# Danderson123/Amira

Measured on AMD Instinct MI355X. Metric: gene-mers/s to corrected GeneMerGraph, higher is better.
Workload: dtype int32; 1 GPU; synthetic 1M reads x 60 genes, k=5, 20k-gene vocab: build + error-correction sweep (build, filter(3,1), correct, build, clip(5), correct, build); reads_per_gpu=1000000, genes_per_read=60, k=5, vocab=20000, gene_mers_per_gpu=56000000, final_nodes=472478, final_edges=1054844, multi_gpu=n/a

## Files before the change

amira_amd/_ffi.py:

```python
import ctypes as C
import os

import numpy as np

_HERE = os.path.dirname(os.path.abspath(__file__))
LIB_PATH = os.path.join(_HERE, "libamg.so")


class AmgError(RuntimeError):
    def __init__(self, code, msg):
        super().__init__(f"libamg error {code}: {msg}")
        self.code = code


E_ARG = -2
E_PALINDROME = -4
E_NOMEM = -6
MAX_K = 16


class Counts(C.Structure):
    _fields_ = [(n, C.c_int64) for n in (
        "n_reads", "n_tokens", "n_windows", "n_short_reads", "n_nodes", "n_edges", "n_pairs",
        "n_components", "n_live_nodes", "n_live_edges", "n_reads_to_correct",
        "node_table_slots", "edge_table_slots", "build_retries")] + [("k", C.c_int32), ("two_v", C.c_int32),
                                                                 ("exact_keys", C.c_int32), ("derived", C.c_int32)]

    def as_dict(self):
        return {n: getattr(self, n) for n, _ in self._fields_}


class Xfer(C.Structure):
    _fields_ = [("kind", C.c_int32), ("elem_bytes", C.c_int32), ("send", C.c_void_p), ("recv", C.c_void_p),
                ("send_counts", C.POINTER(C.c_int64)), ("recv_counts", C.POINTER(C.c_int64)), ("count", C.c_int64)]


XFER_ALL_TO_ALL, XFER_ALL_GATHER = 1, 2
UNIQUE_ID_BYTES = 128


def _load():
    if not os.path.exists(LIB_PATH):
        raise ImportError(
            f"{LIB_PATH} is missing: build it with `python -c 'import __graft_entry__ as g; g.build()'` "
            "(make -C amira_amd/csrc).  amira_amd has no CPU fallback."
        )
    try:
        import torch
    except Exception:
        pass
    lib = C.CDLL(LIB_PATH)
    P, I32, I64, U32 = C.c_void_p, C.c_int32, C.c_int64, C.c_uint32
    sig = {
        "amg_create": (C.c_int, [C.c_int, C.POINTER(P)]),
        "amg_destroy": (C.c_int, [P]),
        "amg_last_error": (C.c_char_p, []),
        "amg_sync": (C.c_int, [P]),
        "amg_stream": (P, [P]),
        "amg_set_reads": (C.c_int, [P, P, P, I64, I32, C.c_int]),
        "amg_set_positions": (C.c_int, [P, P, P, P, C.c_int]),
        "amg_set_positions32": (C.c_int, [P, P, P, P, C.c_int]),
        "amg_set_read_lengths": (C.c_int, [P, P, C.c_int]),
        "amg_build": (C.c_int, [P, I32]),
        "amg_build_filtered": (C.c_int, [P, C.c_int32, C.c_uint32, C.c_uint32]),
        "amg_counts": (C.c_int, [P, C.POINTER(Counts)]),
        "amg_build_multi": (C.c_int, [C.POINTER(P), C.POINTER(I32), I32]),
        "amg_finalize": (C.c_int, [P]),
        "amg_sizes": (C.c_int, [P, C.POINTER(I64), C.POINTER(I64)]),
        "amg_graph_sizes": (C.c_int, [P, C.POINTER(I64), C.POINTER(I64), C.POINTER(I32)]),
        "amg_get_nodes": (C.c_int, [P, P, P, P, P, P, P]),
        "amg_get_edges": (C.c_int, [P, P, P, P, P, P, P]),
        "amg_get_read_nodes": (C.c_int, [P, P, P]),
        "amg_get_read_nodes_rows": (C.c_int, [P, P, P, I64, P]),
        "amg_get_node_adj": (C.c_int, [P, P, P]),
        "amg_get_node_reads": (C.c_int, [P, P, P]),
        "amg_filter": (C.c_int, [P, U32, U32]),
        "amg_remove_nodes": (C.c_int, [P, P, I64]),
        "amg_remove_edges": (C.c_int, [P, P, I64]),
        "amg_remove_short_linear_paths": (C.c_int, [P, I32, P, C.POINTER(I64), P]),
        "amg_remove_low_coverage_components": (C.c_int, [P, U32]),
        "amg_get_reads_to_correct": (C.c_int, [P, P]),
        "amg_correct_reads": (C.c_int, [P, C.POINTER(I64), C.POINTER(I64)]),
        "amg_get_corrected": (C.c_int, [P, P, P, P, P, P, P]),
        "amg_get_corrected32": (C.c_int, [P, P, P, P, P, P, P, P, C.POINTER(I64)]),
        "amg_get_corrected_positions32": (C.c_int, [P, P, P]),
        "amg_adopt_corrected": (C.c_int, [P]),
        "amg_set_reads_from_corrected": (C.c_int, [P, P]),
        "amg_match_patterns": (C.c_int, [P, C.c_int, P, P, I64, P, P, P]),
        "amg_minhash": (C.c_int, [P, P, P, P, I64, I32, C.c_uint64, P, P, I64, C.POINTER(I64)]),
        "amg_junction_paths": (C.c_int, [P, I32, C.POINTER(I64)]),
        "amg_get_junction_paths": (C.c_int, [P, P, P, P, P, P, P]),
        "amg_seqs_create": (C.c_int, [I32, P, P, I64, C.POINTER(P)]),
        "amg_seqs_destroy": (C.c_int, [P]),
        "amg_path_sketch_overlaps": (C.c_int, [P, P, P, I32, C.c_uint64, I64, P, P, I64, P, P, P, P]),
        "amg_kcount_create": (C.c_int, [P, P, I32, I32, C.POINTER(P)]),
        "amg_kcount_sizes": (C.c_int, [P, P]),
        "amg_kcount_histo": (C.c_int, [P, P, I64, P]),
        "amg_kcount_query": (C.c_int, [P, P, P, P, I64, I64, P]),
        "amg_kcount_medians": (C.c_int, [P, P, P, P, P, I64, I64, P, P, P, I64]),
        "amg_kcount_destroy": (C.c_int, [P]),
        "amg_nw_align": (C.c_int, [P, I32, P, I32, P, C.POINTER(I32)]),
        "amg_pop_rewrite": (C.c_int, [P, I32, I32, I64, P, P, P, P, P, I64, P, P, P, I64, P, P, P, P, P, P, P,
                                      C.POINTER(I64)]),
        "amg_dist_unique_id": (C.c_int, [P, I32]),
        "amg_dist_init": (C.c_int, [P, P, I32, I32]),
        "amg_dist_merge": (C.c_int, [P, I32, U32, U32]),
        "amg_dist_finalize": (C.c_int, [P]),
        "amg_dist_init_external": (C.c_int, [P, I32, I32]),
        "amg_dist_merge_begin": (C.c_int, [P, I32, U32, U32]),
        "amg_dist_merge_next": (C.c_int, [P, C.POINTER(Xfer)]),
        "amg_dist_merge_local": (C.c_int, [C.POINTER(P), I32, I32, U32, U32]),
        "amg_copy_d2h": (C.c_int, [P, P, P, I64]),
        "amg_copy_h2d": (C.c_int, [P, P, P, I64]),
        "amg_dist_stats": (C.c_int, [P, C.POINTER(I64), I32]),
        "amg_dist_phase_ms": (C.c_int, [P, I32, C.POINTER(C.c_char_p), C.POINTER(C.c_double), I32]),
        "amg_calls_load_json": (C.c_int, [C.c_char_p, C.POINTER(P)]),
        "amg_calls_counts": (C.c_int, [P, C.POINTER(I64), C.POINTER(I64), C.POINTER(I64), C.POINTER(I64),
                                       C.POINTER(I64)]),
        "amg_calls_get": (C.c_int, [P, P, P, P, P, P]),
        "amg_calls_load_positions_json": (C.c_int, [P, C.c_char_p, P, P]),
        "amg_calls_write_json": (C.c_int, [C.c_char_p, P, P, I64, P, I64, P]),
        "amg_calls_write_positions_json": (C.c_int, [C.c_char_p, P, P, P, I64, P]),
        "amg_calls_write_positions_json32": (C.c_int, [C.c_char_p, P, P, P, I64, P]),
        "amg_calls_first_use": (C.c_int, [P, I64, I32, P, I64, P]),
        "amg_calls_has_blanks": (C.c_int, [P, C.POINTER(I32)]),
        "amg_calls_free": (C.c_int, [P]),
        "amg_calls_trim": (C.c_int, [C.POINTER(I64)]),
        "amg_cluster_full_blocks": (C.c_int, [P, P, I64, P, P, I32, P, I64, I64, C.POINTER(P)]),
        "amg_cluster_anchor_stats": (C.c_int, [P, P, I64, P, P, I32, I64, P]),
        "amg_cluster_blocks_sizes": (C.c_int, [P, C.POINTER(I64), C.POINTER(I64)]),
        "amg_cluster_blocks_get": (C.c_int, [P, P, P]),
        "amg_cluster_blocks_free": (C.c_int, [P]),
        "amg_py_tuple_hash": (I64, [P, I64]),
        "amg_pyset_script": (C.c_int, [P, I64, P, I32, P, P]),
        "amg_last_timings": (C.c_int, [P, C.POINTER(C.c_char_p), C.POINTER(C.c_float), C.c_int]),
        "amg_set_timing": (C.c_int, [P, C.c_int]),
        "amg_scan_probe": (C.c_int, [P, C.c_int, P, I64, P, P]),
        "amg_count_probe": (C.c_int, [P, C.c_int, C.c_int, P, I64, I64, P, I64, C.c_int, C.c_int, P, P]),
        "amg_nw_probe": (C.c_int, [P, I64, P, P, P, P, P, P, P, P, C.c_int, P, P, P, P]),
        "amg_correct_routes": (C.c_int, [P, P, I32]),
    }
    for name, (res, args) in sig.items():
        fn = getattr(lib, name)
        fn.restype, fn.argtypes = res, args
    return lib, sorted(sig)


lib, SYMBOLS = _load()


def check(rc):
    if rc != 0:
        raise AmgError(rc, lib.amg_last_error().decode(errors="replace"))


def ptr(a):
    if a is None:
        return None
    assert isinstance(a, np.ndarray) and a.flags["C_CONTIGUOUS"]
    return a.ctypes.data_as(C.c_void_p)
```

amira_amd/csrc/amg_correct.h:

```cpp
#pragma once
#include "amg_device.h"

enum { RC_SKIP = 0, RC_COPY = 1, RC_DROP = 2, RC_TRIM = 3, RC_GAPPED = 4, RC_KEEP_ORIG = 5 };

struct CorrArgs {
  const int* tokens;
  const long long* read_off;
  const int* tok_node;
  const signed char* tok_dir;
  const unsigned char* read_fix;
  const long long* p0s;
  const long long* p0e;
  const long long* p1s;
  const long long* p1e;
  long long n0;
  const long long* pos_off;
  const long long* read_len;
  long long n_reads;
  int k, flip, have_pos;
  unsigned int* gflag;
  unsigned long long* max_bound;
  unsigned long long* lmask;
  unsigned long long* n_runs;
  unsigned char* cls;
  unsigned char* cls_final;
  int* r_start;
  int* r_end;
  unsigned int* bound;
  const long long* tmp_off;
  unsigned int* new_len;
  int* tmp_tok;
};

__device__ __forceinline__ void pos_base(const CorrArgs& a, long long off, const long long*& gs, const long long*& ge) {
  if (off < a.n0) {
    gs = a.p0s + off;
    ge = a.p0e + off;
  } else {
    gs = a.p1s + (off - a.n0);
    ge = a.p1e + (off - a.n0);
  }
}

__device__ __forceinline__ long long bcast_i64(long long v, int lane) {
  const unsigned int lo = (unsigned int)__builtin_amdgcn_readlane((int)(unsigned int)v, lane);
  const unsigned int hi = (unsigned int)__builtin_amdgcn_readlane((int)(unsigned int)((unsigned long long)v >> 32), lane);
  return (long long)(((unsigned long long)hi << 32) | lo);
}

__device__ __forceinline__ void wave_sync() {
  __builtin_amdgcn_fence(__ATOMIC_ACQ_REL, "wavefront");
  __builtin_amdgcn_wave_barrier();
}

struct __attribute__((aligned(16))) GapRec {
  int r, L0, start, end;
  long long t0, dst;
  unsigned long long mask;
  long long pad;
};

__device__ __forceinline__ unsigned long long gap_run_ends(unsigned long long lv, int start, int end) {
  const unsigned long long inside =
      (end >= 63 ? ~0ull : ((1ull << (end + 1)) - 1ull)) & ~((1ull << (start & 63)) - 1ull);
  return ~lv & inside & (lv >> 1);
}
__device__ __forceinline__ void gap_run_terminals(unsigned long long lv, int i, int& ps, int& pe) {
  ps = 63 - __clzll((long long)(lv & ((1ull << i) - 1ull)));
  pe = i + 1;
}

struct GapArgs {
  CorrArgs a;
  GView g;
  const GapRec* rec;
  const int* gapped_reads;
  long long n_gapped;
  int* pool;
  unsigned long long pool_cap;
  unsigned long long* pool_used;
  unsigned long long* status;
  int* cand;
  unsigned int cand_stride;
  unsigned char* final_cls;
  unsigned char* need_slow;
  const int* gq;
  const int4* qres;
  const int* qpool;
};

#define GF_MAXW 128
#define GF_MAXGAP 16
#define GF_POOL 384
#define GF_CAND 136
#define GF_MAXCOMBO 256
#define GM_INLINE 64
#define LEAN_CHUNK 32
#define CLS_READS 64
#define PACK_READS 64
enum {
  GS_NOT_TRIED = 1,
  GS_WINDOWS = 2,
  GS_RUNS = 3,
  GS_MEMO_UNFIT = 4,
  GS_RECORDS = 5,
  GS_COMBOS = 6,
  GS_CAND = 7,
  GS_CODES = 8
};
enum {
  GL_NO_SLOTS = 1,
  GL_ANSWERS = 2,
  GL_LONG = 3,
  GL_OTHER = 4,
  GL_CODES = 5
};

#define NWF_MAX_M 64
#define NWF_MAX_N 128
__device__ __forceinline__ bool nw_fast_ok(long long N, long long M) {
  return N <= NWF_MAX_N && M <= NWF_MAX_M && N > 0 && M > 0;
}

struct __attribute__((aligned(16))) NwRec {
  int r, M, N, pad;
  long long t0, dst;
  long long pdst;
  long long poff;
};

struct NwArgs {
  CorrArgs a;
  const NwRec* rec;
  long long* o_gs;
  long long* o_ge;
  const int* gapped_reads;
  long long n_gapped;
  const unsigned char* final_cls;
  const long long* big_off;
  unsigned char* big_buf;
  int allow_fast;
  int shortcuts;
  unsigned char* route;
};
enum { NW_ROUTE_NONE = 0, NW_ROUTE_EQUAL = 1, NW_ROUTE_CERT = 2, NW_ROUTE_FILL = 3, NW_ROUTE_LDS = 4, NW_ROUTE_GLOBAL = 5 };

struct PackArgs {
  CorrArgs a;
  const long long* new_idx;
  const long long* new_off;
  const unsigned char* final_cls;
  int* o_tok;
  long long* o_off;
  int* o_orig;
  unsigned char* o_changed;
  long long* o_src;
  const long long* pos_new;
  long long* o_posoff;
  long long* o_rl;
  long long out_reads, out_tokens;
  unsigned long long* dead_kept;
};

struct CorrSwitches {
  bool gap_memo;
  bool fast_gapped;
  bool lean_gapped;
  int fast_nw;
  int nw_shortcuts;
  const char* node_bound;
  bool routes;
  const char* gap_pool;
  const char* memo_spill;
};

struct CorrScratch {
  size_t per_read = 0;
  unsigned char *cls = nullptr, *final_cls = nullptr;
  int *r_start = nullptr, *r_end = nullptr;
  long long *nw_size = nullptr, *nw_off = nullptr;
  unsigned int *bound = nullptr, *new_len = nullptr, *flag = nullptr;
  long long *tmp_off = nullptr, *new_idx = nullptr, *new_off = nullptr;
  int* tmp_tok = nullptr;
  long long *plen = nullptr, *poffs = nullptr, *pos_new = nullptr;
  unsigned long long *max_bound = nullptr, *n_general = nullptr;
  unsigned long long* n_runs = nullptr;
  unsigned long long* dead_kept = nullptr;
  bool count_alive = false;
  DevBuf* glist = nullptr;
  DevBuf* cand = nullptr;
  DevBuf* pool = nullptr;
  DevBuf* need_slow = nullptr;
};

struct CorrCounts {
  long long tmp_total = 0, n_gapped = 0, total_runs = 0;
  unsigned long long max_bound = 0;
  bool carry = false;
  long long out_reads = 0, out_tokens = 0, big_total = 0, pos_total = 0;
  unsigned long long n_general = 0;
  long long n_queries = 0;
  int pool_retries = 0;
  bool lean_ran = false, fast_ran = false, memo = false;
};

static void fill_pos_args(amg_ctx* c, CorrArgs& a) {
  a.p0s = c->have_pos ? c->gene_start.as<long long>() : nullptr;
  a.p0e = c->have_pos ? c->gene_end.as<long long>() : nullptr;
  a.p1s = c->pos1_s.as<long long>();
  a.p1e = c->pos1_e.as<long long>();
  a.n0 = c->pos_n0;
  a.pos_off = (c->have_pos && !c->pos_identity) ? c->pos_off.as<long long>() : nullptr;
}

void corr_classify_launch(amg_ctx* c, const CorrArgs& a);
int corr_gapped(amg_ctx* c, const CorrSwitches& sw, const CorrScratch& S, const CorrArgs& a, CorrCounts& n);
int corr_nw_sizes(amg_ctx* c, const CorrSwitches& sw, const CorrScratch& S, const CorrArgs& a, long long n_gapped,
                  FetchList& shape);
int corr_grow_pos_pools(amg_ctx* c, const CorrCounts& n);
int corr_positions(amg_ctx* c, const CorrSwitches& sw, const CorrScratch& S, const CorrArgs& a, const CorrCounts& n,
                   unsigned char* route = nullptr);

int routes_begin(amg_ctx* c);
int routes_gapped(amg_ctx* c, const CorrScratch& S, const CorrCounts& n, const unsigned char* need_slow, const int* gq);
int routes_nw(amg_ctx* c, const CorrScratch& S, const CorrCounts& n);
int routes_end(amg_ctx* c, const CorrCounts& n);
```

amira_amd/csrc/amg_correct.hip:

```cpp
#include "amg_correct.h"

__global__ __launch_bounds__(256) void k_count_alive(const unsigned char* __restrict__ alive, long long n,
                                                     unsigned long long* out) {
  __shared__ unsigned int s_part[4];
  unsigned int c = 0;
  for (long long i = ((long long)blockIdx.x * blockDim.x + threadIdx.x) * 4; i < n; i += (long long)gridDim.x * blockDim.x * 4) {
    if (i + 4 <= n) {
      const unsigned int w = *reinterpret_cast<const unsigned int*>(alive + i);
      c += __popc(w & 0x01010101u);
    } else {
      for (long long j = i; j < n; ++j) c += alive[j] ? 1u : 0u;
    }
  }
  for (int d = 32; d > 0; d >>= 1) c += (unsigned int)__shfl_xor((int)c, d, 64);
  if ((threadIdx.x & 63) == 0) s_part[threadIdx.x >> 6] = c;
  __syncthreads();
  if (threadIdx.x == 0 && (s_part[0] | s_part[1] | s_part[2] | s_part[3]))
    atomicAdd(out, (unsigned long long)s_part[0] + s_part[1] + s_part[2] + s_part[3]);
}

__global__ __launch_bounds__(256) void k_corr_pack(PackArgs A) {
  const CorrArgs& a = A.a;
  const int lane = threadIdx.x & 63;
  const long long r = ((long long)blockIdx.x * 4 + (threadIdx.x >> 6)) * PACK_READS + lane;
  if (blockIdx.x == 0 && threadIdx.x == 0) A.o_off[A.out_reads] = A.out_tokens;
  long long dst = 0, src = 0;
  int n = 0;
  unsigned int dead = 0;
  if (r < a.n_reads && a.new_len[r] > 0) {
    dst = A.new_off[r];
    n = (int)a.new_len[r];
    const unsigned char fc = A.final_cls[r];
    if (fc == RC_KEEP_ORIG) {
      const long long nw = a.read_off[r + 1] - a.read_off[r] - a.k + 1;
      dead = nw <= 64 ? (unsigned int)(nw - __popcll(a.lmask[r])) : (unsigned int)nw;
    }
    long long poff = 0;
    if (fc == RC_GAPPED) {
      src = a.tmp_off[r] | (1ll << 62);
      if (a.have_pos) poff = A.pos_new[r];
    } else {
      const long long cut = fc == RC_TRIM ? a.r_start[r] : 0;
      src = a.read_off[r] + cut;
      if (a.have_pos) poff = (a.pos_off ? a.pos_off[r] : a.read_off[r]) + cut;
    }
    const long long q = A.new_idx[r];
    A.o_off[q] = dst;
    A.o_orig[q] = (int)r;
    A.o_changed[q] = (fc == RC_TRIM || fc == RC_GAPPED) ? 1 : 0;
    A.o_src[q] = fc == RC_GAPPED ? -1ll : src;
    if (a.have_pos) A.o_posoff[q] = poff;
    if (a.read_len) A.o_rl[q] = a.read_len[r];
  }
  if (__ballot(dead != 0u) != 0ull) {
    for (int d = 32; d > 0; d >>= 1) dead += (unsigned int)__shfl_xor((int)dead, d, 64);
    if (lane == 0) atomicAdd(A.dead_kept + 16 * (blockIdx.x & 15), (unsigned long long)dead);
  }
  if (__ballot(n > 0) == 0ull) return;
  for (int j0 = 0; j0 < PACK_READS; j0 += 4) {
    const int* sp[4];
    long long d[4];
    int nn[4], vt[4];
#pragma unroll
    for (int j = 0; j < 4; ++j) {
      nn[j] = __builtin_amdgcn_readlane(n, j0 + j);
      const long long sj = bcast_i64(src, j0 + j);
      d[j] = bcast_i64(dst, j0 + j);
      sp[j] = ((sj >> 62) & 1 ? a.tmp_tok : a.tokens) + (sj & ~(1ll << 62));
    }
#pragma unroll
    for (int j = 0; j < 4; ++j)
      if (lane < nn[j]) vt[j] = sp[j][lane];
#pragma unroll
    for (int j = 0; j < 4; ++j)
      if (lane < nn[j]) A.o_tok[d[j] + lane] = vt[j];
#pragma unroll
    for (int j = 0; j < 4; ++j)
      for (int i = 64 + lane; i < nn[j]; i += 64)
        A.o_tok[d[j] + i] = sp[j][i];
  }
}

static CorrSwitches read_switches() {
  auto is_one = [](const char* name) {
    const char* v = getenv(name);
    return v && v[0] == '1';
  };
  CorrSwitches sw;
  sw.gap_memo = !is_one("AMG_NO_GAP_MEMO");
  sw.fast_gapped = !is_one("AMG_NO_FAST_GAPPED");
  sw.lean_gapped = !is_one("AMG_NO_LEAN_GAPPED");
  sw.fast_nw = !is_one("AMG_NO_FAST_NW");
  sw.nw_shortcuts = !is_one("AMG_NW_NO_SHORTCUT");
  sw.node_bound = getenv("AMG_TEST_NODE_BOUND");
  sw.routes = is_one("AMG_CORR_ROUTES");
  sw.gap_pool = getenv("AMG_TEST_GAP_POOL");
  sw.memo_spill = getenv("AMG_TEST_MEMO_SPILL");
  return sw;
}

static int plan_per_read(amg_ctx* c, CorrScratch& S) {
  const size_t per_read = (size_t)(c->n_reads + 2);
  AMGCHK(c->s0.ensure(per_read * (1 + 1) + 64));
  AMGCHK(c->s1.ensure(per_read * sizeof(int) * 2 + per_read * sizeof(long long) * 2 + 64));
  AMGCHK(c->s2.ensure(per_read * sizeof(unsigned int) * 3));
  AMGCHK(c->s3.ensure(per_read * sizeof(long long) * 3));
  AMGCHK(c->gm_mask.ensure(per_read * sizeof(unsigned long long)));
  AMGCHK(c->gm_ctr.ensure((16 + 256 + 256 + 16) * sizeof(unsigned long long)));
  S.per_read = per_read;
  S.cls = c->s0.as<unsigned char>();
  S.final_cls = S.cls + per_read;
  S.r_start = c->s1.as<int>();
  S.r_end = S.r_start + per_read;
  S.nw_size = reinterpret_cast<long long*>(((uintptr_t)(S.r_end + per_read) + 15) & ~(uintptr_t)15);
  S.nw_off = S.nw_size + per_read;
  S.bound = c->s2.as<unsigned int>();
  S.new_len = S.bound + per_read;
  S.flag = S.new_len + per_read;
  S.tmp_off = c->s3.as<long long>();
  S.new_idx = S.tmp_off + per_read;
  S.new_off = S.new_idx + per_read;
  S.max_bound = S.n_general = c->status.as<unsigned long long>() + ST_MISC;
  S.n_runs = c->gm_ctr.as<unsigned long long>() + 16;
  S.dead_kept = S.n_runs + 256;
  S.count_alive = c->n_nodes >= (1ll << 20);
  S.glist = &c->c_orig;
  S.cand = &c->c_gstart;
  S.pool = &c->c_gend;
  S.need_slow = &c->c_changed;
  return AMG_OK;
}

static int plan_staging(amg_ctx* c, CorrScratch& S, long long tmp_total) {
  AMGCHK(c->c_tokens_buf.ensure((size_t)(tmp_total + 4) * sizeof(int)));
  AMGCHK(c->s4.ensure((size_t)(tmp_total + 4) * sizeof(int)));
  S.tmp_tok = c->s4.as<int>();
  return AMG_OK;
}

static int plan_positions(amg_ctx* c, CorrScratch& S, long long n_gapped) {
  AMGCHK(c->s5.ensure((size_t)(2 * (n_gapped + 2) + c->n_reads + 2) * sizeof(long long)));
  S.plen = c->s5.as<long long>();
  S.poffs = S.plen + (n_gapped + 2);
  S.pos_new = S.poffs + (n_gapped + 2);
  return AMG_OK;
}

static void corr_args(amg_ctx* c, const CorrScratch& S, CorrArgs& a) {
  a.tokens = c->tokens.as<int>();
  a.read_off = c->read_off.as<long long>();
  a.tok_node = c->tok_node.as<int>();
  a.tok_dir = c->tok_dir.as<signed char>();
  a.read_fix = c->read_fix.as<unsigned char>();
  fill_pos_args(c, a);
  a.read_len = c->have_read_len ? c->read_len.as<long long>() : nullptr;
  a.n_reads = c->n_reads;
  a.k = c->k;
  a.flip = c->two_v - 1;
  a.have_pos = c->have_pos ? 1 : 0;
  a.gflag = S.flag;
  a.max_bound = S.max_bound;
  a.lmask = c->gm_mask.as<unsigned long long>();
  a.n_runs = S.n_runs;
  a.cls = S.cls;
  a.cls_final = S.final_cls;
  a.r_start = S.r_start;
  a.r_end = S.r_end;
  a.bound = S.bound;
  a.tmp_off = S.tmp_off;
  a.new_len = S.new_len;
  a.tmp_tok = S.tmp_tok;
}

static int corr_classify(amg_ctx* c, const CorrScratch& S, const CorrArgs& a, CorrCounts& n) {
  hipStream_t st = c->stream;
  const long long R = c->n_reads;
  {
    ClearList cl;
    cl.add(S.bound, S.per_read * sizeof(unsigned int) * 3);
    cl.add(S.max_bound, sizeof(unsigned long long));
    cl.add(S.n_runs, (256 + 256 + 16) * sizeof(unsigned long long));
    AMGCHK(clear_many(c, cl));
  }
  if (R > 0) corr_classify_launch(c, a);
  if (S.count_alive)
    hipLaunchKernelGGL(k_count_alive, dim3(128), dim3(256), 0, st, c->node_alive.as<unsigned char>(), c->n_nodes,
                       S.dead_kept + 256);
  AMGCHK(prim_exscan_u32_pair(c, S.bound, S.tmp_off, S.flag, S.new_idx, (size_t)R));
  FetchList l;
  l.add(S.tmp_off + R);
  l.add(S.max_bound);
  l.add(S.new_idx + R);
  for (int i = 0; i < 16; ++i) l.add(S.n_runs + 16 * i);
  unsigned long long v[3 + 16];
  AMGCHK(fetch(c, l, v));
  n.tmp_total = (long long)v[0];
  n.max_bound = v[1];
  n.n_gapped = (long long)v[2];
  for (int i = 0; i < 16; ++i) n.total_runs += (long long)v[3 + i];
  n.carry = n.n_gapped > 0 && c->have_pos;
  return AMG_OK;
}

static int corr_shape(amg_ctx* c, const CorrSwitches& sw, CorrScratch& S, const CorrArgs& a, CorrCounts& n) {
  const long long R = c->n_reads;
  AMGCHK(prim_exscan_keep_and_len(c, S.new_len, S.new_idx, S.new_off, (size_t)R));
  FetchList shape;
  shape.add(S.new_idx + R);
  shape.add(S.new_off + R);
  if (n.carry) {
    AMGCHK(plan_positions(c, S, n.n_gapped));
    AMGCHK(corr_nw_sizes(c, sw, S, a, n.n_gapped, shape));
  }
  unsigned long long v[5] = {0, 0, 0, 0, 0};
  AMGCHK(fetch(c, shape, v));
  n.out_reads = (long long)v[0];
  n.out_tokens = (long long)v[1];
  n.big_total = (long long)v[2];
  n.pos_total = (long long)v[3];
  n.n_general = v[4];
  return AMG_OK;
}

static int ensure_outputs(amg_ctx* c, const CorrCounts& n) {
  AMGCHK(c->c_tokens_buf.ensure((size_t)(n.out_tokens + 64) * sizeof(int)));
  AMGCHK(c->c_read_off.ensure((size_t)(n.out_reads + 2) * sizeof(long long)));
  AMGCHK(c->c_orig.ensure((size_t)(n.out_reads + 2) * sizeof(int)));
  AMGCHK(c->c_changed.ensure((size_t)(n.out_reads + 2)));
  AMGCHK(c->c_src.ensure((size_t)(n.out_reads + 2) * sizeof(long long)));
  if (c->have_pos) AMGCHK(c->c_pos_off.ensure((size_t)(n.out_reads + 2) * sizeof(long long)));
  if (c->have_read_len) AMGCHK(c->c_read_len.ensure((size_t)(n.out_reads + 2) * sizeof(long long)));
  return AMG_OK;
}

static int corr_pack(amg_ctx* c, const CorrScratch& S, const CorrArgs& a, const CorrCounts& n) {
  PackArgs Pk;
  Pk.a = a;
  Pk.new_idx = S.new_idx;
  Pk.new_off = S.new_off;
  Pk.final_cls = S.final_cls;
  Pk.o_tok = c->c_tokens_buf.as<int>();
  Pk.o_off = c->c_read_off.as<long long>();
  Pk.o_orig = c->c_orig.as<int>();
  Pk.o_changed = c->c_changed.as<unsigned char>();
  Pk.o_src = c->c_src.as<long long>();
  Pk.pos_new = S.pos_new;
  Pk.o_posoff = c->have_pos ? c->c_pos_off.as<long long>() : nullptr;
  Pk.o_rl = c->have_read_len ? c->c_read_len.as<long long>() : nullptr;
  Pk.out_reads = n.out_reads;
  Pk.out_tokens = n.out_tokens;
  Pk.dead_kept = S.dead_kept;
  if (c->n_reads > 0)
    hipLaunchKernelGGL(k_corr_pack, dim3(nblk(c->n_reads, 4 * PACK_READS)), dim3(256), 0, c->stream, Pk);
  else
    HIPCHK(hipMemcpyAsync(c->c_read_off.as<long long>() + n.out_reads, &n.out_tokens, sizeof(long long),
                          hipMemcpyHostToDevice, c->stream));
  return AMG_OK;
}

static int corr_node_bound(amg_ctx* c, const CorrSwitches& sw, const CorrScratch& S, const CorrCounts& n) {
  FetchList l;
  for (int i = 0; i < 16; ++i) l.add(S.dead_kept + 16 * i);
  l.add(S.dead_kept + 256);
  unsigned long long v[17];
  AMGCHK(fetch(c, l, v));
  unsigned long long bound = S.count_alive ? v[16] : (unsigned long long)c->n_nodes;
  unsigned long long dead_kept = 0;
  for (int i = 0; i < 16; ++i) dead_kept += v[i];
  bound += dead_kept;
  c->c_derivable = n.n_gapped == 0 && dead_kept == 0 && !c->edge_own_deaths;
  c->c_node_bound = (int64_t)bound;
  if (sw.node_bound) c->c_node_bound = atoll(sw.node_bound);
  c->c_node_bound_k = c->k;
  return AMG_OK;
}

extern "C" int amg_correct_reads(amg_ctx* c, int64_t* n_out_reads, int64_t* n_out_tokens) {
  NEED_BUILT(c);
  const CorrSwitches sw = read_switches();
  stages_reset(c);
  c->have_corrected = false;
  CorrScratch S;
  CorrCounts n;
  CorrArgs a;
  AMGCHK(plan_per_read(c, S));
  corr_args(c, S, a);
  c->have_routes = false;
  if (sw.routes) AMGCHK(routes_begin(c));

  stage_begin(c, "correct_classify");
  AMGCHK(corr_classify(c, S, a, n));
  stage_end(c);
  AMGCHK(plan_staging(c, S, n.tmp_total));
  corr_args(c, S, a);

  if (n.n_gapped > 0) {
    stage_begin(c, "live_adjacency");
    AMGCHK(ensure_live_adj(c));
    stage_end(c);
    stage_begin(c, "correct_gapped");
    AMGCHK(corr_gapped(c, sw, S, a, n));
    stage_end(c);
  }

  stage_begin(c, "correct_pack");
  AMGCHK(corr_shape(c, sw, S, a, n));
  stage_end(c);
  AMGCHK(ensure_outputs(c, n));

  if (n.carry) {
    stage_begin(c, "correct_positions");
    AMGCHK(corr_grow_pos_pools(c, n));
    corr_args(c, S, a);
    AMGCHK(corr_positions(c, sw, S, a, n));
    if (sw.routes) AMGCHK(routes_nw(c, S, n));
    stage_end(c);
  }

  stage_begin(c, "correct_pack");
  AMGCHK(corr_pack(c, S, a, n));
  AMGCHK(corr_node_bound(c, sw, S, n));
  stage_end(c);
  if (sw.routes) AMGCHK(routes_end(c, n));
  c->c_reads = n.out_reads;
  c->c_tokens = n.out_tokens;
  c->c_pos1_used = c->pos1_used + (n.carry ? n.pos_total : 0);
  c->have_corrected = true;
  if (n_out_reads) *n_out_reads = n.out_reads;
  if (n_out_tokens) *n_out_tokens = n.out_tokens;
  return AMG_OK;
}
```

amira_amd/csrc/amg_correct_gapped.hip:

```cpp
#include "amg_correct.h"
#include "amg_wave_dfs.h"

__global__ __launch_bounds__(256) void k_corr_classify(CorrArgs a) {
  const long long rbase = ((long long)blockIdx.x * 4 + (threadIdx.x >> 6)) * CLS_READS;
  if (rbase >= a.n_reads) return;
  const int lane = threadIdx.x & 63;
  const long long r = rbase + lane;
  const bool have = r < a.n_reads;
  const long long t0 = have ? a.read_off[r] : 0;
  const long long n = have ? (a.read_off[r + 1] - t0) - a.k + 1 : 0;
  const bool look = have && n > 0 && a.read_fix[r] != 0;
  unsigned long long lv = 0;
  unsigned long long todo = __ballot(look && n <= 64);
  while (todo) {
    int who[4];
    long long tj[4];
    int nj[4], v[4];
#pragma unroll
    for (int q = 0; q < 4; ++q) {
      who[q] = todo ? __ffsll((long long)todo) - 1 : -1;
      if (todo) todo &= todo - 1ull;
      tj[q] = who[q] >= 0 ? bcast_i64(t0, who[q]) : 0;
      nj[q] = who[q] >= 0 ? __builtin_amdgcn_readlane((int)n, who[q]) : 0;
    }
// ... 562 lines not shown

__device__ __forceinline__ void gf_stage(const CorrArgs& a, const GapRec& rec, int nwin, int lane, GfLds& S) {
  for (int i = lane; i < nwin; i += 64) {
    S.node[i] = a.tok_node[rec.t0 + i];
    S.dir[i] = a.tok_dir[rec.t0 + i];
  }
  for (int i = lane; i < rec.L0; i += 64) S.tok[i] = a.tokens[rec.t0 + i];
  if (lane == 0) S.used = 0;
  wave_sync();
}

__device__ __forceinline__ int gf_list_runs(int start, int end, int lane, GfLds& S) {
  int n_gaps = 0;
  for (int c0 = start; c0 <= end; c0 += 64) {
    const int i = c0 + lane;
    const bool is_end = i <= end && S.node[i] < 0 && S.node[i + 1] >= 0;
    const unsigned long long m = __ballot(is_end);
    if (is_end) {
      int q = n_gaps + __popcll(m & ((1ull << lane) - 1ull));
      if (q < GF_MAXGAP) {
        int ps = i - 1;
        while (S.node[ps] < 0) --ps;
        S.gap[3 * q] = ps;
        S.gap[3 * q + 1] = i + 1;
        S.gap[3 * q + 2] = 0;
      }
    }
    n_gaps += __popcll(m);
  }
  return n_gaps;
}

__device__ __forceinline__ int gf_paths_from_memo(const GapArgs& A, int myslot, int n_gaps, int lane, GfLds& S) {
  int4 res = make_int4(0, 0, 0, 0);
  if (lane < n_gaps) res = A.qres[myslot];
  const int len = res.y > 0 ? res.y : 0;
  int at = len;
#pragma unroll
  for (int d = 1; d < GF_MAXGAP; d <<= 1) {
    const int o = __shfl_up(at, d, 64);
    if (lane >= d) at += o;
  }
  const int total = __shfl(at, n_gaps - 1, 64);
  at -= len;
  if (__any(res.y < 0)) return GS_MEMO_UNFIT;
  if (total > GF_POOL) return GS_RECORDS;
  for (int q = 0; q < n_gaps; ++q) {
    const int src = __shfl(res.x, q, 64), ln = __shfl(len, q, 64), dst0 = __shfl(at, q, 64);
    for (int i = lane; i < ln; i += 64) S.pool[dst0 + i] = A.qpool[src + i];
  }
  wave_sync();
  if (lane < n_gaps) {
    for (int o = at; o < at + len; o += 2 + 2 * S.pool[o + 1]) S.pool[o] = lane;
    S.gap[3 * lane + 2] = res.z;
  }
  if (lane == 0) S.used = total;
  wave_sync();
  return 0;
}

__device__ __forceinline__ int gf_paths_by_search(const GView& g, int n_gaps, int lane, GfLds& S) {
  for (int q = 0; q < n_gaps; ++q) {
    const int ps = S.gap[3 * q], pe = S.gap[3 * q + 1];
    const int np = dfs_paths_wave(g, S.node[ps], S.dir[ps], S.node[pe], 2 * g.k, q, S.pool, &S.used, lane);
    if (lane == 0) S.gap[3 * q + 2] = np < 0 ? 0 : np;
    if (np < 0) return GS_RECORDS;
  }
  return 0;
}

__device__ __forceinline__ unsigned long long gf_count_combos(const GfLds& S, int n_gaps, bool& dead_end) {
  unsigned long long n_combo = 1;
  dead_end = false;
  for (int q = 0; q < n_gaps; ++q) {
    const int np = S.gap[3 * q + 2];
    dead_end = dead_end || np == 0;
    n_combo *= (unsigned long long)np;
    if (n_combo > GF_MAXCOMBO) break;
  }
  return n_combo;
}

__device__ __forceinline__ void gf_copy_windows(GfLds& S, int n, int i, int cnt, int lane) {
  for (int j = lane; j < cnt; j += 64) {
    S.cnode[n + j] = S.node[i + j];
    S.cdir[n + j] = S.dir[i + j];
  }
}

__device__ __forceinline__ int gf_build_candidate(GfLds& S, int start, int end, int n_gaps, int used,
                                                  unsigned long long combo, int lane) {
  int n = 0, i = start, prev_pe = -1;
  for (int q = 0; q < n_gaps; ++q) {
    const int ps = S.gap[3 * q], pe = S.gap[3 * q + 1], np = S.gap[3 * q + 2];
    const int cnt = ps - i;
    if (cnt > 0) {
      if (n + cnt > GF_CAND) return -1;
      gf_copy_windows(S, n, i, cnt, lane);
      n += cnt;
    }
    unsigned long long div = 1;
    for (int j = q + 1; j < n_gaps; ++j) div *= (unsigned long long)S.gap[3 * j + 2];
    int pick = (int)((combo / div) % (unsigned long long)np);
    int off = 0;
    while (off < used) {
      if (S.pool[off] == q) {
        if (pick == 0) break;
        --pick;
      }
      off += 2 + 2 * S.pool[off + 1];
    }
    const int L = S.pool[off + 1];
    if (prev_pe == ps && n > 0) --n;
    if (n + L > GF_CAND) return -1;
    for (int j = lane; j < L; j += 64) {
      S.cnode[n + j] = S.pool[off + 2 + j];
      S.cdir[n + j] = (signed char)S.pool[off + 2 + L + j];
    }
    n += L;
    prev_pe = pe;
    i = (q + 1 < n_gaps && S.gap[3 * (q + 1)] == pe) ? pe : pe + 1;
  }
  const int cnt = end - i + 1;
  if (cnt > 0) {
    if (n + cnt > GF_CAND) return -1;
    gf_copy_windows(S, n, i, cnt, lane);
    n += cnt;
  }
  return n;
}

__device__ __forceinline__ void gf_spell_and_score(const GView& g, GfLds& S, int n, int L0, bool rank, int lane,
                                                   int& shared, unsigned long long& csum) {
  const int ng = n + g.k - 1;
  shared = 0;
  csum = 0;
  for (int q = lane; q < ng; q += 64) {
    const int idx = q < g.k - 1 ? 0 : q - (g.k - 1);
    const int j = q < g.k - 1 ? q : g.k - 1;
    S.gene[q] = oriented_tok(g, S.cnode[idx], S.cdir[idx], j);
  }
  if (rank) {
    for (int q = lane; q < n; q += 64) csum += g.n_cov[S.cnode[q]];
    for (int d = 32; d > 0; d >>= 1) csum += __shfl_xor(csum, d, 64);
  }
  wave_sync();
  if (rank) {
    for (int q = lane; q < ng; q += 64) {
      const int tk = S.gene[q];
      bool dup = false;
      for (int w = 0; w < q && !dup; ++w) dup = (S.gene[w] == tk);
      bool hit = false;
      if (!dup)
        for (int w = 0; w < L0 && !hit; ++w) hit = (S.tok[w] == tk);
      shared += hit ? 1 : 0;
    }
    for (int d = 32; d > 0; d >>= 1) shared += __shfl_xor(shared, d, 64);
  }
}

__device__ __forceinline__ void gf_hand_down(const GapArgs& A, long long gi, int lane, int why) {
  if (lane == 0) A.need_slow[gi] = (unsigned char)why;
}

__device__ __forceinline__ void gapped_fast_read(const GapArgs& A, long long gi, int lane, GfLds& S) {
  const CorrArgs& a = A.a;
  const GView& g = A.g;
  const GapRec rec = A.rec[gi];
  const int nwin = rec.L0 - g.k + 1;
  if (nwin > GF_MAXW) return gf_hand_down(A, gi, lane, GS_WINDOWS);
  const int myslot = (A.gq && lane < GF_MAXGAP) ? A.gq[gi * GF_MAXGAP + lane] : -1;
  gf_stage(a, rec, nwin, lane, S);
  const int n_gaps = gf_list_runs(rec.start, rec.end, lane, S);
  if (n_gaps > GF_MAXGAP) return gf_hand_down(A, gi, lane, GS_RUNS);
  wave_sync();
  const int unfit = __builtin_amdgcn_readfirstlane(myslot) >= 0 ? gf_paths_from_memo(A, myslot, n_gaps, lane, S)
                                                                : gf_paths_by_search(g, n_gaps, lane, S);
  if (unfit) return gf_hand_down(A, gi, lane, unfit);
  wave_sync();
  bool dead_end;
  const unsigned long long n_combo = gf_count_combos(S, n_gaps, dead_end);
  if (dead_end) {
    if (lane == 0) {
      a.new_len[rec.r] = (unsigned int)rec.L0;
      A.final_cls[rec.r] = RC_KEEP_ORIG;
    }
    return;
  }
  if (n_combo > GF_MAXCOMBO) return gf_hand_down(A, gi, lane, GS_COMBOS);
  const int used = S.used;
  int best_shared = 0, best_ng = -1;
  unsigned long long best_sum = 0, best_len = 1;
  for (unsigned long long combo = 0; combo < n_combo; ++combo) {
    const int n = gf_build_candidate(S, rec.start, rec.end, n_gaps, used, combo, lane);
    wave_sync();
    if (n < 0) return gf_hand_down(A, gi, lane, GS_CAND);
    int shared;
    unsigned long long csum;
    gf_spell_and_score(g, S, n, rec.L0, n_combo > 1, lane, shared, csum);
    if (n_combo == 1 || cand_better(shared, csum, n, best_shared, best_sum, best_len)) {
      best_shared = shared;
      best_sum = csum;
      best_len = (unsigned long long)n;
      best_ng = n + g.k - 1;
      for (int q = lane; q < best_ng; q += 64) S.best[q] = S.gene[q];
    }
    wave_sync();
  }
  for (int q = lane; q < best_ng; q += 64) a.tmp_tok[rec.dst + q] = S.best[q];
  if (lane == 0) a.new_len[rec.r] = (unsigned int)best_ng;
}

__global__ __launch_bounds__(64 * GF_WPB, 8) void k_corr_gapped_fast(GapArgs A, const unsigned char* __restrict__ left) {
  __shared__ GfLds s_lds;
  const int lane = (int)threadIdx.x;
  if (!left) {
    if ((long long)blockIdx.x < A.n_gapped) gapped_fast_read(A, (long long)blockIdx.x, lane, s_lds);
    return;
  }
  const long long base = (long long)blockIdx.x * LEAN_CHUNK;
  const bool mine = lane < LEAN_CHUNK && base + lane < A.n_gapped && left[base + lane] != 0;
  unsigned long long todo = __ballot(mine);
  while (todo) {
    const int b = __ffsll((long long)todo) - 1;
    todo &= todo - 1ull;
    gapped_fast_read(A, base + b, lane, s_lds);
    wave_sync();
  }
}

__global__ void k_scatter_gapped(const unsigned int* __restrict__ flag, const long long* __restrict__ pos,
                                 long long n_reads, int* __restrict__ out, const long long* __restrict__ read_off,
                                 const int* __restrict__ r_start, const int* __restrict__ r_end,
                                 const long long* __restrict__ tmp_off, const unsigned long long* __restrict__ lmask,
                                 GapRec* __restrict__ rec) {
  long long r = (long long)blockIdx.x * blockDim.x + threadIdx.x;
  if (r >= n_reads || !flag[r]) return;
  const long long gi = pos[r];
  out[gi] = (int)r;
  GapRec q;
  q.r = (int)r;
  q.t0 = read_off[r];
  const long long len = read_off[r + 1] - q.t0;
  q.L0 = (int)(len > 0x7fffffff ? 0x7fffffff : len);
  q.start = r_start[r];
  q.end = r_end[r];
  q.dst = tmp_off[r];
  q.mask = lmask[r];
  q.pad = 0;
  rec[gi] = q;
}

static int gap_memo(amg_ctx* c, const CorrSwitches& sw, const CorrArgs& a, CorrCounts& n, const int** gq) {
  hipStream_t st = c->stream;
  const long long n_gapped = n.n_gapped, total_runs = n.total_runs;
  *gq = nullptr;
  const uint64_t qslots = pow2_at_least((uint64_t)total_runs * 2 + 16);
  AMGCHK(c->gm_tab.ensure((size_t)qslots * sizeof(unsigned long long)));
  AMGCHK(c->gm_res.ensure((size_t)qslots * sizeof(int4)));
  AMGCHK(c->gm_list.ensure((size_t)(total_runs + 1) * sizeof(int)));
  AMGCHK(c->gm_q.ensure((size_t)(n_gapped + 1) * GF_MAXGAP * sizeof(int)));
  {
    ClearList cl;
    cl.add(c->gm_tab.p, (size_t)qslots * sizeof(unsigned long long));
    cl.add(c->gm_ctr.p, 16 * sizeof(unsigned long long));
    cl.add(c->status.as<unsigned long long>() + ST_OVERFLOW, sizeof(unsigned long long));
    AMGCHK(clear_many(c, cl));
  }
  hipLaunchKernelGGL(k_gap_queries, dim3(nblk(n_gapped, 256)), dim3(256), 0, st, c->gap_rec.as<GapRec>(), n_gapped,
                     c->k, a.tok_node, a.tok_dir, c->gm_tab.as<unsigned long long>(), (unsigned int)(qslots - 1),
                     c->gm_ctr.as<unsigned long long>(), c->gm_list.as<int>(), c->gm_q.as<int>(),
                     c->status.as<unsigned long long>());
  unsigned long long v[2] = {0, 0};
  {
    FetchList l;
    l.add(c->gm_ctr.p);
    l.add(c->status.as<unsigned long long>() + ST_OVERFLOW);
    AMGCHK(fetch(c, l, v));
  }
  if (v[1]) return amg_fail(AMG_E_HIP, "correct_reads: path memo table full");
  const long long n_queries = (long long)v[0];
  unsigned long long qcap = (unsigned long long)n_queries * (GM_INLINE + 32ull) + 4096ull;
  if (sw.memo_spill) {
    const unsigned long long lo = (unsigned long long)n_queries * GM_INLINE + strtoull(sw.memo_spill, nullptr, 10);
    qcap = lo < qcap ? lo : qcap;
  }
  if (qcap > 0x7fffffffull) return AMG_OK;
  AMGCHK(c->gm_pool.ensure((size_t)qcap * sizeof(int)));
  AMGCHK(c->gm_gene.ensure((size_t)qcap * sizeof(int)));
  if (n_queries > 0)
    hipLaunchKernelGGL(k_gap_dfs, dim3((unsigned int)n_queries), dim3(64), 0, st, make_view(c), c->gm_list.as<int>(),
                       n_queries, c->gm_tab.as<unsigned long long>(), c->gm_ctr.as<unsigned long long>() + 1, qcap,
                       c->gm_pool.as<int>(), c->gm_res.as<int4>(), c->gm_gene.as<int>());
  *gq = c->gm_q.as<int>();
  n.n_queries = n_queries;
  return AMG_OK;
}

int corr_gapped(amg_ctx* c, const CorrSwitches& sw, const CorrScratch& S, const CorrArgs& a, CorrCounts& n) {
  hipStream_t st = c->stream;
  const long long R = c->n_reads, n_gapped = n.n_gapped;
  AMGCHK(S.glist->ensure((size_t)(n_gapped + 1) * sizeof(int)));
  AMGCHK(c->gap_rec.ensure((size_t)(n_gapped + 1) * sizeof(GapRec)));
  hipLaunchKernelGGL(k_scatter_gapped, dim3(nblk(R, 256)), dim3(256), 0, st, S.flag, S.new_idx, R,
                     S.glist->as<int>(), a.read_off, S.r_start, S.r_end, S.tmp_off, a.lmask, c->gap_rec.as<GapRec>());
  const int* gq = nullptr;
  if (n.total_runs > 0 && sw.gap_memo) AMGCHK(gap_memo(c, sw, a, n, &gq));
  const unsigned int threads_total = 64u * 2048u;
  unsigned int cand_stride = (unsigned int)(2 * n.max_bound + (n.max_bound + 3) / 4 + c->k + 16);
  AMGCHK(S.cand->ensure((size_t)threads_total * cand_stride * sizeof(int)));
  unsigned long long pool_cap = 1ull << 22;
  if (sw.gap_pool) {
    const unsigned long long lo = strtoull(sw.gap_pool, nullptr, 10);
    pool_cap = lo < pool_cap ? lo : pool_cap;
  }
  AMGCHK(S.need_slow->ensure((size_t)n_gapped + 64));
  unsigned char* need_slow = S.need_slow->as<unsigned char>();
  for (int attempt = 0;; ++attempt) {
    AMGCHK(S.pool->ensure((size_t)pool_cap * sizeof(int)));
    unsigned long long* used = c->status.as<unsigned long long>() + ST_COMPACT_A;
    ClearList gcl;
    gcl.add(c->status.p, ST_WORDS * sizeof(unsigned long long));
    GapArgs G;
    G.a = a;
    G.g = make_view(c);
    G.rec = c->gap_rec.as<GapRec>();
    G.gapped_reads = S.glist->as<int>();
    G.n_gapped = n_gapped;
    G.pool = S.pool->as<int>();
    G.pool_cap = pool_cap;
    G.pool_used = used;
    G.status = c->status.as<unsigned long long>();
    G.cand = S.cand->as<int>();
    G.cand_stride = cand_stride;
    G.final_cls = S.final_cls;
    G.need_slow = need_slow;
    G.gq = gq;
    G.qres = c->gm_res.as<int4>();
    G.qpool = c->gm_pool.as<int>();
    if (attempt == 0) {
      gcl.add(need_slow, ((size_t)n_gapped + 4) & ~(size_t)3, sw.fast_gapped ? 0u : 0x01010101u);
      AMGCHK(clear_many(c, gcl));
      if (sw.fast_gapped && gq && sw.lean_gapped) {
        n.lean_ran = true;
        AMGCHK(c->gm_fail.ensure((size_t)n_gapped + 64));
        hipLaunchKernelGGL(k_corr_gapped_lean, dim3(nblk(n_gapped, GL_THREADS / GL_GROUP)), dim3(GL_THREADS), 0, st, G,
                           c->gm_gene.as<int>(), c->gm_fail.as<unsigned char>());
        hipLaunchKernelGGL(k_corr_gapped_fast, dim3(nblk(n_gapped, LEAN_CHUNK)), dim3(64 * GF_WPB), 0, st, G,
                           c->gm_fail.as<unsigned char>());
      } else if (sw.fast_gapped) {
        hipLaunchKernelGGL(k_corr_gapped_fast, dim3((unsigned int)n_gapped), dim3(64 * GF_WPB), 0, st, G,
                           (const unsigned char*)nullptr);
      }
    } else {
      AMGCHK(clear_many(c, gcl));
    }
    unsigned int blocks = (unsigned int)((n_gapped + 63) / 64);
    if (blocks > 2048u) blocks = 2048u;
    hipLaunchKernelGGL(k_corr_gapped, dim3(blocks), dim3(64), 0, st, G);
    unsigned long long hs[ST_WORDS];
    AMGCHK(fetch_status(c, hs));
    if (!hs[ST_OVERFLOW]) break;
    if (attempt >= 8) return amg_fail(AMG_E_OVERFLOW, "correct_reads: path pool overflow");
    pool_cap = hs[ST_COMPACT_A] * 2 + (1ull << 20);
    n.pool_retries = attempt + 1;
  }
  if (sw.routes) AMGCHK(routes_gapped(c, S, n, need_slow, gq));
  return AMG_OK;
}
```

amira_amd/csrc/amg_corrected.hip:

```cpp
#include "amg_correct.h"

__global__ __launch_bounds__(256) void k_gather_positions(CorrArgs a, const long long* __restrict__ c_off,
                                                          const long long* __restrict__ c_posoff, long long c_reads,
                                                          long long* __restrict__ o_gs, long long* __restrict__ o_ge) {
  const long long q = (long long)blockIdx.x * 4 + (threadIdx.x >> 6);
  if (q >= c_reads) return;
  const int lane = threadIdx.x & 63;
  const long long a0 = c_off[q], n = c_off[q + 1] - a0;
  const long long *gs, *ge;
  pos_base(a, c_posoff[q], gs, ge);
  for (long long i = lane; i < n; i += 64) {
    o_gs[a0 + i] = gs[i];
    o_ge[a0 + i] = ge[i];
  }
}

static CorrArgs pool_args(amg_ctx* c) {
  CorrArgs a;
  memset(&a, 0, sizeof(a));
  fill_pos_args(c, a);
  return a;
}

static int to_host(amg_ctx* c, void* dst, const DevBuf& src, size_t bytes) {
  if (!dst || !bytes) return AMG_OK;
  HIPCHK(hipMemcpyAsync(dst, src.p, bytes, hipMemcpyDeviceToHost, c->stream));
  return AMG_OK;
}

extern "C" int amg_get_corrected(amg_ctx* c, int32_t* tokens, int64_t* read_offsets, int32_t* orig_read,
                                 uint8_t* changed, int64_t* gene_start, int64_t* gene_end) {
  if (!c) return amg_fail(AMG_E_ARG, "null ctx");
  if (!c->have_corrected) return amg_fail(AMG_E_STATE, "amg_correct_reads first");
  HIPCHK(hipSetDevice(c->device));
  hipStream_t st = c->stream;
  AMGCHK(to_host(c, tokens, c->c_tokens_buf, (size_t)c->c_tokens * sizeof(int32_t)));
  AMGCHK(to_host(c, read_offsets, c->c_read_off, (size_t)(c->c_reads + 1) * sizeof(int64_t)));
  AMGCHK(to_host(c, orig_read, c->c_orig, (size_t)c->c_reads * sizeof(int32_t)));
  AMGCHK(to_host(c, changed, c->c_changed, (size_t)c->c_reads));
  if (c->have_pos && (gene_start || gene_end) && c->c_tokens > 0) {
    AMGCHK(c->c_gstart.ensure((size_t)(c->c_tokens + 64) * sizeof(long long)));
    AMGCHK(c->c_gend.ensure((size_t)(c->c_tokens + 64) * sizeof(long long)));
    const CorrArgs a = pool_args(c);
    hipLaunchKernelGGL(k_gather_positions, dim3(nblk(c->c_reads, 4)), dim3(256), 0, st, a,
                       c->c_read_off.as<long long>(), c->c_pos_off.as<long long>(), (long long)c->c_reads,
                       c->c_gstart.as<long long>(), c->c_gend.as<long long>());
    AMGCHK(to_host(c, gene_start, c->c_gstart, (size_t)c->c_tokens * sizeof(int64_t)));
    AMGCHK(to_host(c, gene_end, c->c_gend, (size_t)c->c_tokens * sizeof(int64_t)));
  }
  HIPCHK(hipStreamSynchronize(st));
  return AMG_OK;
}

__global__ void k_widen_pos(const int* __restrict__ s32, const int* __restrict__ e32, long long n,
                            long long* __restrict__ s64, long long* __restrict__ e64) {
  for (long long i = (long long)blockIdx.x * blockDim.x + threadIdx.x; i < n; i += (long long)gridDim.x * blockDim.x) {
    s64[i] = (long long)s32[i];
    e64[i] = (long long)e32[i];
  }
}

extern "C" int amg_set_positions32(amg_ctx* c, const int32_t* gene_start, const int32_t* gene_end,
                                   const int64_t* read_len, int on_device) {
  if (!c) return amg_fail(AMG_E_ARG, "null ctx");
  if (c->two_v <= 0) return amg_fail(AMG_E_STATE, "amg_set_reads first");
  if (!gene_start || !gene_end) return amg_fail(AMG_E_ARG, "null positions");
  if (on_device != 0 && on_device != 1) return amg_fail(AMG_E_ARG, "amg_set_positions32: on_device is 0 or 1 (the arrays are widened, never borrowed)");
  HIPCHK(hipSetDevice(c->device));
  hipStream_t st = c->stream;
  const long long T = c->n_tokens;
  const int* d_s = gene_start;
  const int* d_e = gene_end;
  if (!on_device) {
    AMGCHK(c->c_gstart.ensure((size_t)(T + 64) * sizeof(long long)));
    AMGCHK(c->c_gend.ensure((size_t)(T + 64) * sizeof(long long)));
    if (T > 0) {
      HIPCHK(hipMemcpyAsync(c->c_gstart.p, gene_start, (size_t)T * sizeof(int), hipMemcpyHostToDevice, st));
      HIPCHK(hipMemcpyAsync(c->c_gend.p, gene_end, (size_t)T * sizeof(int), hipMemcpyHostToDevice, st));
    }
    d_s = c->c_gstart.as<int>();
    d_e = c->c_gend.as<int>();
  }
  c->gene_start.unborrow();
  c->gene_end.unborrow();
  AMGCHK(c->gene_start.ensure((size_t)(T + 64) * sizeof(long long)));
  AMGCHK(c->gene_end.ensure((size_t)(T + 64) * sizeof(long long)));
  if (T > 0)
    hipLaunchKernelGGL(k_widen_pos, dim3(nblk(T, 1024) < 4096u ? nblk(T, 1024) : 4096u), dim3(256), 0, st, d_s, d_e, T,
                       c->gene_start.as<long long>(), c->gene_end.as<long long>());
  c->have_pos = true;
  c->pos_identity = true;
  c->pos0_own = false;
  c->pos_n0 = T;
  c->pos1_used = c->c_pos1_used = 0;
  c->have_corrected = false;
  c->have_read_len = false;
  if (read_len) {
    c->read_len.unborrow();
    AMGCHK(c->read_len.ensure((size_t)c->n_reads * sizeof(int64_t) + 64));
    if (c->n_reads > 0)
      HIPCHK(hipMemcpyAsync(c->read_len.p, read_len, (size_t)c->n_reads * sizeof(int64_t),
                            on_device ? hipMemcpyDeviceToDevice : hipMemcpyHostToDevice, st));
    c->have_read_len = true;
  }
  HIPCHK(hipStreamSynchronize(st));
  return AMG_OK;
}

__global__ void k_new_pos_len(const long long* __restrict__ c_off, const long long* __restrict__ c_posoff, long long own,
                              long long c_reads, long long* __restrict__ len) {
  const long long q = (long long)blockIdx.x * blockDim.x + threadIdx.x;
  if (q < c_reads) len[q] = c_posoff[q] >= own ? c_off[q + 1] - c_off[q] : 0;
}

__global__ __launch_bounds__(256) void k_gather_new_positions32(CorrArgs a, const long long* __restrict__ c_off,
                                                                const long long* __restrict__ c_posoff, long long c_reads,
                                                                const long long* __restrict__ new_off,
                                                                long long* __restrict__ pos_src, int* __restrict__ o_gs,
                                                                int* __restrict__ o_ge, unsigned long long* too_wide,
                                                                long long own) {
  const long long q = (long long)blockIdx.x * 4 + (threadIdx.x >> 6);
  if (q >= c_reads) return;
  const int lane = threadIdx.x & 63;
  const long long off = c_posoff[q];
  if (off < own) {
    if (lane == 0) pos_src[q] = off;
    return;
  }
  const long long n = c_off[q + 1] - c_off[q], at = new_off[q];
  if (lane == 0) pos_src[q] = -1 - at;
  const long long *gs, *ge;
  pos_base(a, off, gs, ge);
  bool wide = false;
  for (long long i = lane; i < n; i += 64) {
    const long long s = gs[i], e = ge[i];
    wide = wide || s != (long long)(int)s || e != (long long)(int)e;
    o_gs[at + i] = (int)s;
    o_ge[at + i] = (int)e;
  }
  if (wide) *too_wide = 1ull;
}

extern "C" int amg_get_corrected32(amg_ctx* c, int32_t* tokens, int64_t* read_offsets, int32_t* orig_read,
                                   uint8_t* changed, int64_t* pos_src, int32_t* new_start, int32_t* new_end,
                                   int64_t* n_new) {
  if (!c) return amg_fail(AMG_E_ARG, "null ctx");
  if (!c->have_corrected) return amg_fail(AMG_E_STATE, "amg_correct_reads first");
  if (!pos_src || !n_new) return amg_fail(AMG_E_ARG, "amg_get_corrected32: pos_src and n_new are required");
  HIPCHK(hipSetDevice(c->device));
  hipStream_t st = c->stream;
  const long long R = c->c_reads;
  *n_new = 0;
  AMGCHK(to_host(c, tokens, c->c_tokens_buf, (size_t)c->c_tokens * sizeof(int32_t)));
  AMGCHK(to_host(c, read_offsets, c->c_read_off, (size_t)(R + 1) * sizeof(int64_t)));
  AMGCHK(to_host(c, orig_read, c->c_orig, (size_t)R * sizeof(int32_t)));
  AMGCHK(to_host(c, changed, c->c_changed, (size_t)R));
  if (!c->have_pos || R == 0) {
    HIPCHK(hipStreamSynchronize(st));
    return c->have_pos ? AMG_OK : amg_fail(AMG_E_STATE, "amg_get_corrected32: no positions were set");
  }
  AMGCHK(c->s1.ensure((size_t)(2 * R + 4) * sizeof(long long)));
  AMGCHK(c->s2.ensure((size_t)(R + 2) * sizeof(long long)));
  AMGCHK(c->c_gstart.ensure((size_t)(c->c_tokens + 64) * sizeof(long long)));
  AMGCHK(c->c_gend.ensure((size_t)(c->c_tokens + 64) * sizeof(long long)));
  long long* len = c->s1.as<long long>();
  long long* off = len + (R + 2);
  const CorrArgs a = pool_args(c);
  unsigned long long* flag = c->status.as<unsigned long long>() + ST_MISC;
  HIPCHK(hipMemsetAsync(flag, 0, sizeof(unsigned long long), st));
  HIPCHK(hipMemsetAsync(len + R, 0, sizeof(long long), st));
  const long long own = c->pos0_own ? 0 : a.n0;
  hipLaunchKernelGGL(k_new_pos_len, dim3(nblk(R, 256)), dim3(256), 0, st, c->c_read_off.as<long long>(),
                     c->c_pos_off.as<long long>(), own, R, len);
  AMGCHK(prim_exscan_i64(c, len, off, (size_t)R + 1));
  hipLaunchKernelGGL(k_gather_new_positions32, dim3(nblk(R, 4)), dim3(256), 0, st, a, c->c_read_off.as<long long>(),
                     c->c_pos_off.as<long long>(), R, off, c->s2.as<long long>(), c->c_gstart.as<int>(),
                     c->c_gend.as<int>(), flag, own);
  unsigned long long h[2] = {0, 0};
  {
    FetchList l;
    l.add(off + R);
    l.add(flag);
    AMGCHK(fetch(c, l, h));
  }
  if (h[1]) return amg_fail(AMG_E_ARG, "amg_get_corrected32: a position does not fit 32 bits (amg_get_corrected returns 64-bit positions)");
  *n_new = (int64_t)h[0];
  AMGCHK(to_host(c, pos_src, c->s2, (size_t)R * sizeof(int64_t)));
  AMGCHK(to_host(c, new_start, c->c_gstart, (size_t)h[0] * sizeof(int32_t)));
  AMGCHK(to_host(c, new_end, c->c_gend, (size_t)h[0] * sizeof(int32_t)));
  HIPCHK(hipStreamSynchronize(st));
  return AMG_OK;
}

__global__ __launch_bounds__(256) void k_gather_positions32(CorrArgs a, const long long* __restrict__ c_off,
                                                            const long long* __restrict__ c_posoff, long long c_reads,
                                                            int* __restrict__ o_gs, int* __restrict__ o_ge,
                                                            unsigned long long* too_wide) {
  const long long q = (long long)blockIdx.x * 4 + (threadIdx.x >> 6);
  if (q >= c_reads) return;
  const int lane = threadIdx.x & 63;
  const long long a0 = c_off[q], n = c_off[q + 1] - a0;
  const long long *gs, *ge;
  pos_base(a, c_posoff[q], gs, ge);
  bool wide = false;
  for (long long i = lane; i < n; i += 64) {
    const long long s = gs[i], e = ge[i];
    wide = wide || s != (long long)(int)s || e != (long long)(int)e;
    o_gs[a0 + i] = (int)s;
    o_ge[a0 + i] = (int)e;
  }
  if (wide) *too_wide = 1ull;
}

extern "C" int amg_get_corrected_positions32(amg_ctx* c, int32_t* gene_start, int32_t* gene_end) {
  if (!c || !gene_start || !gene_end) return amg_fail(AMG_E_ARG, "null argument");
  if (!c->have_corrected) return amg_fail(AMG_E_STATE, "amg_correct_reads first");
  if (!c->have_pos) return amg_fail(AMG_E_STATE, "no gene positions were set");
  HIPCHK(hipSetDevice(c->device));
  hipStream_t st = c->stream;
  const long long R = c->c_reads, T = c->c_tokens;
  if (T == 0) return AMG_OK;
  AMGCHK(c->c_gstart.ensure((size_t)(T + 64) * sizeof(long long)));
  AMGCHK(c->c_gend.ensure((size_t)(T + 64) * sizeof(long long)));
  unsigned long long* flag = c->status.as<unsigned long long>() + ST_MISC;
  HIPCHK(hipMemsetAsync(flag, 0, sizeof(unsigned long long), st));
  const CorrArgs a = pool_args(c);
  hipLaunchKernelGGL(k_gather_positions32, dim3(nblk(R, 4)), dim3(256), 0, st, a, c->c_read_off.as<long long>(),
                     c->c_pos_off.as<long long>(), R, c->c_gstart.as<int>(), c->c_gend.as<int>(), flag);
  unsigned long long wide = 0;
  {
    FetchList l;
    l.add(flag);
    AMGCHK(fetch(c, l, &wide));
  }
  if (wide) return amg_fail(AMG_E_ARG, "amg_get_corrected_positions32: a position does not fit 32 bits (amg_get_corrected returns 64-bit positions)");
  HIPCHK(hipMemcpyAsync(gene_start, c->c_gstart.p, (size_t)T * sizeof(int32_t), hipMemcpyDeviceToHost, st));
  HIPCHK(hipMemcpyAsync(gene_end, c->c_gend.p, (size_t)T * sizeof(int32_t), hipMemcpyDeviceToHost, st));
  HIPCHK(hipStreamSynchronize(st));
  return AMG_OK;
}

extern "C" int amg_adopt_corrected(amg_ctx* c) {
  if (!c) return amg_fail(AMG_E_ARG, "null ctx");
  if (!c->have_corrected) return amg_fail(AMG_E_STATE, "amg_correct_reads first");
  bool compacted = false;
  if (c->have_pos && c->c_tokens > 0) {
    long long slack = 1ll << 20;
    if (const char* e = getenv("AMG_POS_COMPACT_MIN")) slack = atoll(e);
    if (c->c_pos1_used > 2 * c->c_tokens + slack) {
      HIPCHK(hipSetDevice(c->device));
      AMGCHK(c->c_gstart.ensure((size_t)(c->c_tokens + 64) * sizeof(long long)));
      AMGCHK(c->c_gend.ensure((size_t)(c->c_tokens + 64) * sizeof(long long)));
      const CorrArgs a = pool_args(c);
      hipLaunchKernelGGL(k_gather_positions, dim3(nblk(c->c_reads, 4)), dim3(256), 0, c->stream, a,
                         c->c_read_off.as<long long>(), c->c_pos_off.as<long long>(), (long long)c->c_reads,
                         c->c_gstart.as<long long>(), c->c_gend.as<long long>());
      HIPCHK(hipStreamSynchronize(c->stream));
      c->gene_start.unborrow();
      c->gene_end.unborrow();
      std::swap(c->gene_start, c->c_gstart);
      std::swap(c->gene_end, c->c_gend);
      compacted = true;
      c->pos0_own = true;
    }
  }
  for (DevBuf* b : {&c->tokens, &c->read_off, &c->read_len}) b->unborrow();
  std::swap(c->tokens, c->c_tokens_buf);
  std::swap(c->read_off, c->c_read_off);
  std::swap(c->rd_src, c->c_src);
  c->derive_ready = c->c_derivable;
  c->dist_candidate = c->dist_mode;
  c->c_derivable = false;
  if (c->have_pos && compacted) {
    c->pos_identity = true;
    c->pos_n0 = c->c_tokens;
    c->pos1_used = c->c_pos1_used = 0;
  } else if (c->have_pos) {
    std::swap(c->pos_off, c->c_pos_off);
    c->pos_identity = false;
    c->pos1_used = c->c_pos1_used;
  }
  if (c->have_read_len) std::swap(c->read_len, c->c_read_len);
  c->n_reads = c->c_reads;
  c->n_tokens = c->c_tokens;
  c->have_corrected = false;
  c->built = false;
  c->match_valid = false;
  if (c->c_node_bound > 0 && c->c_node_bound_k == c->k && (c->node_hint == 0 || c->c_node_bound < c->node_hint))
    c->node_hint = c->c_node_bound > 256 ? c->c_node_bound : 256;
  c->c_node_bound = 0;
  return AMG_OK;
}

extern "C" int amg_set_reads_from_corrected(amg_ctx* dst, amg_ctx* src) {
  if (!dst || !src) return amg_fail(AMG_E_ARG, "null ctx");
  if (!src->have_corrected) return amg_fail(AMG_E_STATE, "amg_correct_reads on the source ctx first");
  if (dst == src) return amg_adopt_corrected(src);
  if (dst->device != src->device) return amg_fail(AMG_E_ARG, "amg_set_reads_from_corrected: one device");
  HIPCHK(hipSetDevice(dst->device));
  HIPCHK(hipStreamSynchronize(src->stream));
  hipStream_t st = dst->stream;
  const long long R = src->c_reads, T = src->c_tokens;
  AMGCHK(dst->tokens.ensure((size_t)T * sizeof(int32_t) + 64));
  AMGCHK(dst->read_off.ensure((size_t)(R + 1) * sizeof(int64_t) + 64));
  if (T > 0) HIPCHK(hipMemcpyAsync(dst->tokens.p, src->c_tokens_buf.p, (size_t)T * sizeof(int32_t), hipMemcpyDeviceToDevice, st));
  HIPCHK(hipMemcpyAsync(dst->read_off.p, src->c_read_off.p, (size_t)(R + 1) * sizeof(int64_t), hipMemcpyDeviceToDevice, st));
  dst->n_reads = R;
  dst->n_tokens = T;
  dst->two_v = src->two_v;
  dst->have_pos = dst->have_read_len = false;
  if (src->have_pos) {
    AMGCHK(dst->gene_start.ensure((size_t)(T + 64) * sizeof(long long)));
    AMGCHK(dst->gene_end.ensure((size_t)(T + 64) * sizeof(long long)));
    if (R > 0 && T > 0) {
      const CorrArgs a = pool_args(src);
      hipLaunchKernelGGL(k_gather_positions, dim3(nblk(R, 4)), dim3(256), 0, st, a, src->c_read_off.as<long long>(),
                         src->c_pos_off.as<long long>(), R, dst->gene_start.as<long long>(),
                         dst->gene_end.as<long long>());
    }
    dst->have_pos = true;
    dst->pos0_own = true;
    dst->pos_identity = true;
    dst->pos_n0 = T;
    dst->pos1_used = dst->c_pos1_used = 0;
  }
  if (src->have_read_len) {
    AMGCHK(dst->read_len.ensure((size_t)(R + 1) * sizeof(long long) + 64));
    if (R > 0)
      HIPCHK(hipMemcpyAsync(dst->read_len.p, src->c_read_len.p, (size_t)R * sizeof(long long), hipMemcpyDeviceToDevice, st));
    dst->have_read_len = true;
  }
  HIPCHK(hipStreamSynchronize(st));
  dst->built = false;
  dst->derive_ready = false;
  dst->have_corrected = false;
  dst->match_valid = false;
  dst->node_hint = 0;
  dst->hint_bound = src->c_node_bound;
  dst->hint_bound_k = src->c_node_bound_k;
  dst->cnt_hint_reset = true;
  return AMG_OK;
}
```

amira_amd/csrc/amg_derive.hip:

```cpp
#include "amg_device.h"

__device__ __forceinline__ long long dv_new_token(long long t, const long long* __restrict__ src,
                                                  const long long* __restrict__ read_off, long long n_reads, int k,
                                                  bool* ok) {
  long long lo = 0, hi = n_reads;
  while (lo < hi) {
    const long long mid = (lo + hi) >> 1;
    if (src[mid] <= t) lo = mid + 1; else hi = mid;
  }
  const long long i = lo - 1;
  if (i < 0) {
    *ok = false;
    return 0;
  }
  const long long q = t - src[i], len = read_off[i + 1] - read_off[i];
  if (q + k > len) *ok = false;
  return read_off[i] + q;
}

#define DV_READS 64
__device__ __forceinline__ long long dv_bcast(long long v, int lane) {
  const unsigned int lo = (unsigned int)__builtin_amdgcn_readlane((int)(unsigned int)(unsigned long long)v, lane);
  const unsigned int hi = (unsigned int)__builtin_amdgcn_readlane((int)(unsigned int)((unsigned long long)v >> 32), lane);
  return (long long)(((unsigned long long)hi << 32) | lo);
}
__global__ __launch_bounds__(256) void k_dv_windows(const long long* __restrict__ read_off, const long long* __restrict__ src,
                                                    long long n_reads, int k, const int* __restrict__ old_node,
                                                    const signed char* __restrict__ old_dir,
                                                    const long long* __restrict__ new_id, int* __restrict__ tok_node,
                                                    signed char* __restrict__ tok_dir, unsigned long long* bad) {
  const int lane = threadIdx.x & 63;
  const long long r0 = ((long long)blockIdx.x * 4 + (threadIdx.x >> 6)) * DV_READS;
  if (r0 >= n_reads) return;
  long long o = 0, s = 0;
  int n = 0;
  if (r0 + lane < n_reads) {
    o = read_off[r0 + lane];
    n = (int)(read_off[r0 + lane + 1] - o);
    s = src[r0 + lane];
  }
  for (int j0 = 0; j0 < DV_READS; j0 += 4) {
    long long oo[4], ss[4];
    int nn[4], most = 0;
#pragma unroll
    for (int j = 0; j < 4; ++j) {
      nn[j] = __builtin_amdgcn_readlane(n, j0 + j);
      oo[j] = dv_bcast(o, j0 + j);
      ss[j] = dv_bcast(s, j0 + j);
      most = nn[j] > most ? nn[j] : most;
    }
    for (int q = lane; q < most; q += 64) {
      int old[4];
      signed char d[4];
#pragma unroll
      for (int j = 0; j < 4; ++j) {
        old[j] = -1;
        d[j] = 0;
        if (q + k <= nn[j]) {
          old[j] = old_node[ss[j] + q];
          d[j] = old_dir[ss[j] + q];
        }
      }
#pragma unroll
      for (int j = 0; j < 4; ++j) {
        if (q >= nn[j]) continue;
        int v = -1;
        if (q + k <= nn[j]) {
          if (old[j] >= 0) v = (int)new_id[old[j]];
          else *bad = 1ull;
        }
        tok_node[oo[j] + q] = v;
        tok_dir[oo[j] + q] = v >= 0 ? d[j] : (signed char)0;
      }
    }
  }
}

__global__ void k_dv_nodes(const unsigned char* __restrict__ alive, const long long* __restrict__ new_id, long long n_old, int k,
                           const int* __restrict__ tok_in, const unsigned int* __restrict__ cov_in,
                           const long long* __restrict__ first_in, const long long* __restrict__ src,
                           const long long* __restrict__ read_off, long long n_reads, long long own_lo, long long own_hi,
                           int* __restrict__ tok_out, unsigned int* __restrict__ cov_out, long long* __restrict__ first_out,
                           unsigned char* __restrict__ alive_out, unsigned long long* bad) {
  long long n = (long long)blockIdx.x * blockDim.x + threadIdx.x;
  if (n >= n_old || !alive[n]) return;
  const long long i = new_id[n];
  for (int x = 0; x < k; ++x) tok_out[i * k + x] = tok_in[n * k + x];
  cov_out[i] = cov_in[n];
  alive_out[i] = 1;
  const long long f = first_in[n], tg = f >> 1;
  if (tg < own_lo || tg >= own_hi) {
    first_out[i] = 0;
    return;
  }
  bool ok = true;
  const long long t = dv_new_token(tg - own_lo, src, read_off, n_reads, k, &ok);
  if (!ok) *bad = 2ull;
  first_out[i] = (t << 1) | (f & 1ll);
}

__global__ void k_dv_pair_keep(const unsigned long long* __restrict__ pkey, long long n_pairs,
                               const unsigned char* __restrict__ alive, unsigned int* __restrict__ keep) {
  long long p = (long long)blockIdx.x * blockDim.x + threadIdx.x;
  if (p >= n_pairs) return;
  const unsigned long long key = pkey[p];
  const unsigned int lo = (unsigned int)((key >> 32) & 0x7fffffffull), hi = (unsigned int)(key & 0xffffffffull) - 1u;
  keep[p] = (alive[lo] && alive[hi]) ? 1u : 0u;
}

__global__ void k_dv_pairs(const unsigned long long* __restrict__ pkey, const unsigned long long* __restrict__ pfirst,
                           const unsigned int* __restrict__ pcnt, long long n_pairs, const unsigned int* __restrict__ keep,
                           const long long* __restrict__ pos, const long long* __restrict__ new_id,
                           const long long* __restrict__ src, const long long* __restrict__ read_off, long long n_reads, int k,
                           long long own_lo, long long own_hi,
                           unsigned long long* __restrict__ okey, unsigned long long* __restrict__ ofirst,
                           unsigned int* __restrict__ ocnt, unsigned long long* bad) {
  long long p = (long long)blockIdx.x * blockDim.x + threadIdx.x;
  if (p >= n_pairs || !keep[p]) return;
  const unsigned long long key = pkey[p], f = pfirst[p];
  const unsigned int lo = (unsigned int)((key >> 32) & 0x7fffffffull), hi = (unsigned int)(key & 0xffffffffull) - 1u;
  const unsigned long long nlo = (unsigned long long)new_id[lo], nhi = (unsigned long long)new_id[hi];
  const long long q = pos[p];
  okey[q] = (key & (1ull << 63)) | (nlo << 32) | (nhi + 1ull);
  ocnt[q] = pcnt[p];
  const long long tg = (long long)(f >> 3);
  if (tg < own_lo || tg >= own_hi) {
    ofirst[q] = 0ull;
    return;
  }
  bool ok = true;
  const long long t = dv_new_token(tg - own_lo, src, read_off, n_reads, k, &ok);
  if (!ok) *bad = 3ull;
  ofirst[q] = ((unsigned long long)t << 3) | (f & 7ull);
}

__global__ void k_dv_bounds(const long long* __restrict__ base, int world, const long long* __restrict__ node_first,
                            long long n_nodes, const long long* __restrict__ new_id, const unsigned long long* __restrict__ pfirst,
                            long long n_pairs, const long long* __restrict__ ppos, long long* __restrict__ bounds) {
  const int r = blockIdx.x * blockDim.x + threadIdx.x;
  if (r > world) return;
  {
    long long lo = 0, hi = n_nodes;
    const long long want = r == world ? 0x7fffffffffffffffll : (base[r] << 1);
    while (lo < hi) {
      const long long mid = (lo + hi) >> 1;
      if (node_first[mid] < want) lo = mid + 1; else hi = mid;
    }
    bounds[r] = new_id[lo];
  }
  {
    long long lo = 0, hi = n_pairs;
    const unsigned long long want = r == world ? ~0ull : ((unsigned long long)base[r] << 3);
    while (lo < hi) {
      const long long mid = (lo + hi) >> 1;
      if (pfirst[mid] < want) lo = mid + 1; else hi = mid;
    }
    bounds[world + 1 + r] = ppos[lo];
  }
}

int derive_local(amg_ctx* c, int k, long long own_lo, long long own_tokens, const long long* d_bases, int world,
                 long long* bounds_host, long long* D2_out, long long* P2_out, bool* ok) {
  *ok = false;
  hipStream_t st = c->stream;
  const long long D = c->n_nodes, P = c->n_pairs, R = c->n_reads, T = c->n_tokens;
  stage_begin(c, "derive");
  unsigned long long* bad = c->status.as<unsigned long long>() + ST_MISC;
  AMGCHK(c->s2.ensure((size_t)(D + 2) * sizeof(long long)));
  AMGCHK(c->s3.ensure((size_t)(P + 2) * sizeof(unsigned int)));
  AMGCHK(c->s4.ensure((size_t)(P + 2) * sizeof(long long)));
  long long* new_id = c->s2.as<long long>();
  unsigned int* keep = c->s3.as<unsigned int>();
  long long* ppos = c->s4.as<long long>();
  {
    ClearList cl;
    cl.add(c->status.p, ST_WORDS * sizeof(unsigned long long));
    cl.add(keep + P, sizeof(unsigned int));
    AMGCHK(clear_many(c, cl));
  }
  AMGCHK(prim_exscan_bytes_set(c, c->node_alive.as<unsigned char>(), new_id, (size_t)D));
  if (P > 0)
    hipLaunchKernelGGL(k_dv_pair_keep, dim3(nblk(P, 256)), dim3(256), 0, st, c->pair_key.as<unsigned long long>(), P,
                       c->node_alive.as<unsigned char>(), keep);
  AMGCHK(prim_exscan_u32_to_i64(c, keep, ppos, (size_t)P + 1));
  AMGCHK(c->alt_tok_node.ensure((size_t)(T + 8) * sizeof(int)));
  AMGCHK(c->alt_tok_dir.ensure((size_t)(T + 8)));
  if (R > 0)
    hipLaunchKernelGGL(k_dv_windows, dim3(nblk(R, 4 * DV_READS)), dim3(256), 0, st, c->read_off.as<long long>(),
                       c->rd_src.as<long long>(), R, k, c->tok_node.as<int>(), c->tok_dir.as<signed char>(), new_id,
                       c->alt_tok_node.as<int>(), c->alt_tok_dir.as<signed char>(), bad);
  long long* d_bounds = nullptr;
  if (d_bases) {
    AMGCHK(c->s1.ensure((size_t)(2 * (world + 1)) * sizeof(long long)));
    d_bounds = c->s1.as<long long>();
    hipLaunchKernelGGL(k_dv_bounds, dim3(nblk(world + 1, 64)), dim3(64), 0, st, d_bases, world, c->node_first.as<long long>(), D,
                       new_id, c->pair_first.as<unsigned long long>(), P, ppos, d_bounds);
  }
  unsigned long long v[2 + FETCH_MAX - 2];
  {
    FetchList l;
    l.add(new_id + D);
    l.add(ppos + P);
    if (d_bounds) l.add_words(d_bounds, 2 * (world + 1));
    if (l.overflow) return amg_fail(AMG_E_ARG, "derive: world too large");
    AMGCHK(fetch(c, l, v));
  }
  const long long D2 = (long long)v[0], P2 = (long long)v[1];
  if (bounds_host)
    for (int i = 0; i < 2 * (world + 1); ++i) bounds_host[i] = (long long)v[2 + i];
  AMGCHK(c->alt_ntok.ensure((size_t)(D2 * k + 1) * sizeof(int)));
  AMGCHK(c->alt_ncov.ensure((size_t)(D2 + 1) * sizeof(unsigned int)));
  AMGCHK(c->alt_nfirst.ensure((size_t)(D2 + 1) * sizeof(long long)));
  AMGCHK(c->alt_nalive.ensure((size_t)(D2 + 1)));
  AMGCHK(c->alt_pkey.ensure((size_t)(P2 + 2) * sizeof(unsigned long long)));
  AMGCHK(c->alt_pfirst.ensure((size_t)(P2 + 2) * sizeof(unsigned long long)));
  AMGCHK(c->alt_pcnt.ensure((size_t)(P2 + 2) * sizeof(unsigned int)));
  if (D > 0)
    hipLaunchKernelGGL(k_dv_nodes, dim3(nblk(D, 256)), dim3(256), 0, st, c->node_alive.as<unsigned char>(), new_id, D, k,
                       c->node_tokens.as<int>(), c->node_cov.as<unsigned int>(), c->node_first.as<long long>(),
                       c->rd_src.as<long long>(), c->read_off.as<long long>(), R, own_lo, own_lo + own_tokens,
                       c->alt_ntok.as<int>(), c->alt_ncov.as<unsigned int>(), c->alt_nfirst.as<long long>(),
                       c->alt_nalive.as<unsigned char>(), bad);
  if (P > 0)
    hipLaunchKernelGGL(k_dv_pairs, dim3(nblk(P, 256)), dim3(256), 0, st, c->pair_key.as<unsigned long long>(),
                       c->pair_first.as<unsigned long long>(), c->pair_cnt.as<unsigned int>(), P, keep, ppos, new_id,
                       c->rd_src.as<long long>(), c->read_off.as<long long>(), R, k, own_lo, own_lo + own_tokens,
                       c->alt_pkey.as<unsigned long long>(), c->alt_pfirst.as<unsigned long long>(),
                       c->alt_pcnt.as<unsigned int>(), bad);
  stage_end(c);
  AMGCHK(bs_read_stats(c, k));
  unsigned long long hs[ST_WORDS];
  AMGCHK(fetch_status(c, hs));
  if (hs[ST_MISC] || hs[ST_BADINPUT]) return AMG_OK;
  c->n_windows = (int64_t)hs[ST_N_WINDOWS];
  c->n_short = (int64_t)hs[ST_N_SHORT];
  *D2_out = D2;
  *P2_out = P2;
  *ok = true;
  return AMG_OK;
}

int derive_commit(amg_ctx* c, long long D2, long long P2) {
  std::swap(c->tok_node, c->alt_tok_node);
  std::swap(c->tok_dir, c->alt_tok_dir);
  std::swap(c->node_tokens, c->alt_ntok);
  std::swap(c->node_cov, c->alt_ncov);
  std::swap(c->node_first, c->alt_nfirst);
  std::swap(c->node_alive, c->alt_nalive);
  std::swap(c->pair_key, c->alt_pkey);
  std::swap(c->pair_first, c->alt_pfirst);
  std::swap(c->pair_cnt, c->alt_pcnt);
  AMGCHK(c->node_comp.ensure((size_t)(D2 + 1) * sizeof(int)));
  c->n_nodes = c->n_local_nodes = D2;
  c->n_pairs = c->n_local_pairs = P2;
  c->comp_from_claims = false;
  c->filtered_build = false;
  AMGCHK(bs_finish_from_pairs(c));
  c->built = true;
  c->derived = true;
  c->node_hint = D2 > 256 ? D2 : 256;
  return AMG_OK;
}

int derive_from_previous(amg_ctx* c, int k, bool* done) {
  *done = false;
  if (c->n_nodes <= 0 || c->n_reads <= 0 || c->n_tokens <= 0) return AMG_OK;
  long long D2 = 0, P2 = 0;
  bool ok = false;
  AMGCHK(derive_local(c, k, 0, 0x3fffffffffffffffll, nullptr, 1, nullptr, &D2, &P2, &ok));
  if (!ok) return AMG_OK;
  AMGCHK(derive_commit(c, D2, P2));
  *done = true;
  return AMG_OK;
}
```

amira_amd/csrc/amg_device.h:

```cpp
#pragma once
#include "amg_internal.h"

#define AMG_WAVE 64
#define AMG_LAST_FLAG 0x80000000u
#define AMG_MADE_FLAG 0x40000000u
#define AMG_FLAG_MASK (AMG_LAST_FLAG | AMG_MADE_FLAG)
#define AMG_SINGLE_BIT 0x20000000u

__device__ __forceinline__ unsigned long long ld_u64(const unsigned long long* p) {
  return __hip_atomic_load(p, __ATOMIC_RELAXED, __HIP_MEMORY_SCOPE_AGENT);
}
__device__ __forceinline__ int ld_i32(const int* p) {
  return __hip_atomic_load(p, __ATOMIC_RELAXED, __HIP_MEMORY_SCOPE_AGENT);
}

__device__ __forceinline__ unsigned long long mix64(unsigned long long x) {
  x ^= x >> 32;
  x *= 0xD6E8FEB86659FD93ull;
  x ^= x >> 32;
  x *= 0xD6E8FEB86659FD93ull;
  x ^= x >> 32;
  return x;
}

template <class View>
__device__ __forceinline__ int canon_dir(const View& w, int k, int flip) {
  for (int j = 0; j < k; ++j) {
    int a = w[j];
    int b = flip - w[k - 1 - j];
    if (a != b) return a < b ? 1 : -1;
  }
  return 0;
}

template <class View>
__device__ __forceinline__ int canon_tok(const View& w, int k, int flip, int dir, int j) {
  return dir > 0 ? w[j] : flip - w[k - 1 - j];
}

template <class View>
__device__ __forceinline__ unsigned long long canon_fingerprint(const View& w, int k, int flip,
                                                                int dir, unsigned long long seed) {
  unsigned long long h = seed;
  for (int j = 0; j < k; ++j) {
    unsigned long long c = (unsigned long long)(unsigned int)canon_tok(w, k, flip, dir, j);
    h = (h ^ c) * 0x9E3779B97F4A7C15ull;
    h ^= h >> 29;
  }
  h = mix64(h);
  return h ? h : 1ull;
}

__device__ __forceinline__ long long table_upsert(Slot* tab, unsigned long long mask,
                                                  unsigned long long key,
                                                  unsigned long long start,
                                                  unsigned long long first, unsigned int limit,
                                                  bool count_inline = true,
                                                  const unsigned long long* abort_flag = nullptr) {
  unsigned long long idx = start & mask;
  for (unsigned int probes = 0;; ++probes) {
    if (abort_flag && (probes & 63u) == 63u && *reinterpret_cast<const volatile unsigned long long*>(abort_flag))
      return -1;
    Slot* s = tab + idx;
    unsigned long long cur = ld_u64(&s->key);
    if (cur == 0ull) {
      cur = atomicCAS(&s->key, 0ull, key);
      if (cur == 0ull) cur = key;
    }
    if (cur == key) {
      if (count_inline) atomicAdd(&s->count, 1u);
      unsigned long long fi = ~first;
      if (ld_u64(&s->first_inv) < fi) atomicMax(&s->first_inv, fi);
      return (long long)idx;
    }
    if (probes >= limit) return -1;
    idx = (idx + 1) & mask;
  }
}

#define AMG_PACK_MAX_K 14
__device__ __forceinline__ void slot_pack(Slot* s, int id, const int* tok, int k) {
  unsigned int w[8] = {0, 0, 0, 0, 0, 0, 0, 0};
  for (int j = 0; j < k; ++j) {
    const int word = j < 10 ? (j >> 1) : 6 + ((j - 10) >> 1);
    w[word] |= ((unsigned int)tok[j] & 0xffffu) << ((j & 1) * 16);
  }
  w[5] = (unsigned int)id;
  uint4* p = reinterpret_cast<uint4*>(s);
  p[0] = make_uint4(w[0], w[1], w[2], w[3]);
  p[1] = make_uint4(w[4], w[5], w[6], w[7]);
}
__device__ __forceinline__ unsigned int packed_tok(const uint4& lo, const uint4& hi, int j) {
  const int word = j < 10 ? (j >> 1) : 6 + ((j - 10) >> 1);
  unsigned int w = word == 0 ? lo.x : word == 1 ? lo.y : word == 2 ? lo.z : word == 3 ? lo.w
                 : word == 4 ? hi.x : word == 6 ? hi.z : hi.w;
  return (w >> ((j & 1) * 16)) & 0xffffu;
}

template <int WAVES>
__device__ __forceinline__ unsigned int block_exscan(unsigned int v, unsigned int* total,
                                                     unsigned int* s_wave ) {
  unsigned int lane = threadIdx.x & 63, wave = threadIdx.x >> 6;
  unsigned int x = v;
#pragma unroll
  for (int d = 1; d < 64; d <<= 1) {
    unsigned int y = __shfl_up(x, d, 64);
    if (lane >= (unsigned)d) x += y;
  }
  if (lane == 63) s_wave[wave] = x;
  __syncthreads();
  unsigned int base = 0, tot = 0;
#pragma unroll
  for (int w = 0; w < WAVES; ++w) {
    unsigned int c = s_wave[w];
    if ((unsigned)w < wave) base += c;
    tot += c;
  }
  __syncthreads();
  *total = tot;
  return base + x - v;
}
__device__ __forceinline__ unsigned int block_exscan_256(unsigned int v, unsigned int* total,
                                                         unsigned int* s_wave ) {
  return block_exscan<4>(v, total, s_wave);
}


struct ClearArgs {
  void* p[CLEAR_MAX];
  unsigned long long words[CLEAR_MAX];
  unsigned int fill[CLEAR_MAX];
  int n;
};
static inline ClearArgs clear_args(const ClearList& l) {
  ClearArgs a;
  a.n = l.n;
  for (int i = 0; i < l.n; ++i) {
    a.p[i] = l.p[i];
    a.words[i] = l.bytes[i] >> 2;
    a.fill[i] = l.fill[i];
  }
  return a;
}
__device__ __forceinline__ void clear_args_part(const ClearArgs& a, unsigned long long part, unsigned long long parts) {
  const unsigned long long bd = blockDim.x, stride = parts * bd;
  for (int r = 0; r < a.n; ++r) {
    unsigned int* p = reinterpret_cast<unsigned int*>(a.p[r]);
    const unsigned long long w = a.words[r];
    const unsigned int f = a.fill[r];
    const unsigned long long head = ((16u - ((unsigned long long)(uintptr_t)p & 15u)) & 15u) >> 2;
    const unsigned long long h = head < w ? head : w;
    const unsigned long long quads = (w - h) >> 2;
    uint4* q = reinterpret_cast<uint4*>(p + h);
    for (unsigned long long i = part * bd + threadIdx.x; i < quads; i += stride) q[i] = make_uint4(f, f, f, f);
    if (part == 0) {
      for (unsigned long long i = threadIdx.x; i < h; i += bd) p[i] = f;
      for (unsigned long long i = h + quads * 4 + threadIdx.x; i < w; i += bd) p[i] = f;
    }
  }
}

__device__ __forceinline__ int uf_ld(const int* p) {
  return __hip_atomic_load(p, __ATOMIC_RELAXED, __HIP_MEMORY_SCOPE_WAVEFRONT);
}
__device__ __forceinline__ int uf_find(int* parent, int x) {
  int p = uf_ld(parent + x);
  while (p != x) {
    const int g = uf_ld(parent + p);
    if (g != p) __hip_atomic_store(parent + x, g, __ATOMIC_RELAXED, __HIP_MEMORY_SCOPE_WAVEFRONT);
    x = p;
    p = g;
  }
  return x;
}
```

amira_amd/csrc/amg_filter.hip:

```cpp
#include "amg_rows.h"

__global__ void k_filter_nodes(const unsigned int* __restrict__ cov, unsigned char* __restrict__ alive,
                               long long n, unsigned int min_cov) {
  long long i = (long long)blockIdx.x * blockDim.x + threadIdx.x;
  if (i < n && alive[i] && cov[i] < min_cov) alive[i] = 0;
}

__global__ void k_filter_edges(const int* __restrict__ src, const int* __restrict__ tgt,
                               const unsigned int* __restrict__ cov,
                               const unsigned char* __restrict__ node_alive,
                               unsigned char* __restrict__ alive, long long n, unsigned int min_cov) {
  long long e = (long long)blockIdx.x * blockDim.x + threadIdx.x;
  if (e >= n || !alive[e]) return;
  if ((min_cov > 1 && cov[e] < min_cov) || !node_alive[src[e]] || !node_alive[tgt[e]]) alive[e] = 0;
}

#define READS_PER_WAVE 8
__global__ __launch_bounds__(256) void k_mask_reads(int* __restrict__ tok_node,
                                                    const long long* __restrict__ read_off,
                                                    long long n_reads,
                                                    const unsigned char* __restrict__ node_alive,
                                                    unsigned char* __restrict__ read_fix) {
  const long long rbase = ((long long)blockIdx.x * 4 + (threadIdx.x >> 6)) * READS_PER_WAVE;
  if (rbase >= n_reads) return;
  const int lane = threadIdx.x & 63;
  const long long off_l = (lane <= READS_PER_WAVE && rbase + lane <= n_reads) ? read_off[rbase + lane] : 0;
  long long a[READS_PER_WAVE], b[READS_PER_WAVE];
  int v[READS_PER_WAVE];
#pragma unroll
  for (int j = 0; j < READS_PER_WAVE; ++j) {
    a[j] = __shfl(off_l, j, 64);
    b[j] = rbase + j < n_reads ? __shfl(off_l, j + 1, 64) : a[j];
  }
#pragma unroll
  for (int j = 0; j < READS_PER_WAVE; ++j) v[j] = a[j] + lane < b[j] ? tok_node[a[j] + lane] : -1;
  bool dead[READS_PER_WAVE];
#pragma unroll
  for (int j = 0; j < READS_PER_WAVE; ++j) dead[j] = v[j] >= 0 && !node_alive[v[j]];
#pragma unroll
  for (int j = 0; j < READS_PER_WAVE; ++j) {
    if (dead[j]) tok_node[a[j] + lane] = -2;
    bool hit = dead[j];
    for (long long t = a[j] + 64 + lane; t < b[j]; t += 64) {
      const int n = tok_node[t];
      if (n >= 0 && !node_alive[n]) {
        tok_node[t] = -2;
        hit = true;
      }
    }
    if (__any(hit) && lane == 0) read_fix[rbase + j] = 1;
  }
}

static int apply_removals(amg_ctx* c, unsigned int min_edge_cov) {
  hipStream_t st = c->stream;
  if (min_edge_cov > 1) live_lists_after_edge_deaths(c);
  else live_lists_after_node_deaths(c);
  if (c->n_edges > 0)
    hipLaunchKernelGGL(k_filter_edges, dim3(nblk(c->n_edges, 256)), dim3(256), 0, st,
                       c->edge_src.as<int>(), c->edge_tgt.as<int>(), c->edge_cov.as<unsigned int>(),
                       c->node_alive.as<unsigned char>(), c->edge_alive.as<unsigned char>(),
                       c->n_edges, min_edge_cov);
  if (c->n_reads > 0)
    hipLaunchKernelGGL(k_mask_reads, dim3(nblk(c->n_reads, 4 * READS_PER_WAVE)), dim3(256), 0, st,
                       c->tok_node.as<int>(), c->read_off.as<long long>(), c->n_reads,
                       c->node_alive.as<unsigned char>(), c->read_fix.as<unsigned char>());
  return AMG_OK;
}

extern "C" int amg_filter(amg_ctx* c, uint32_t min_node_cov, uint32_t min_edge_cov) {
  NEED_BUILT(c);
  stages_reset(c);
  stage_begin(c, "filter");
  if (c->n_nodes > 0)
    hipLaunchKernelGGL(k_filter_nodes, dim3(nblk(c->n_nodes, 256)), dim3(256), 0, c->stream,
                       c->node_cov.as<unsigned int>(), c->node_alive.as<unsigned char>(),
                       c->n_nodes, min_node_cov);
  AMGCHK(apply_removals(c, min_edge_cov));
  stage_end(c);
  c->have_corrected = false;
  return AMG_OK;
}

__global__ void k_kill_listed(const int* __restrict__ ids, long long n, long long n_nodes,
                              unsigned char* __restrict__ alive) {
  long long i = (long long)blockIdx.x * blockDim.x + threadIdx.x;
  if (i >= n) return;
  int v = ids[i];
  if (v >= 0 && v < n_nodes) alive[v] = 0;
}

extern "C" int amg_remove_nodes(amg_ctx* c, const int32_t* node_ids, int64_t n) {
  NEED_BUILT(c);
  if (n < 0 || (n > 0 && !node_ids)) return amg_fail(AMG_E_ARG, "bad node list");
  if (n == 0) return AMG_OK;
  AMGCHK(c->s0.ensure((size_t)n * sizeof(int)));
  HIPCHK(hipMemcpyAsync(c->s0.p, node_ids, (size_t)n * sizeof(int), hipMemcpyHostToDevice, c->stream));
  hipLaunchKernelGGL(k_kill_listed, dim3(nblk(n, 256)), dim3(256), 0, c->stream, c->s0.as<int>(),
                     (long long)n, c->n_nodes, c->node_alive.as<unsigned char>());
  AMGCHK(apply_removals(c, 0));
  HIPCHK(hipStreamSynchronize(c->stream));
  c->have_corrected = false;
  return AMG_OK;
}

extern "C" int amg_remove_edges(amg_ctx* c, const int32_t* edge_ids, int64_t n) {
  NEED_BUILT(c);
  if (n < 0 || (n > 0 && !edge_ids)) return amg_fail(AMG_E_ARG, "bad edge list");
  if (n == 0) return AMG_OK;
  AMGCHK(c->s0.ensure((size_t)n * sizeof(int)));
  HIPCHK(hipMemcpyAsync(c->s0.p, edge_ids, (size_t)n * sizeof(int), hipMemcpyHostToDevice, c->stream));
  hipLaunchKernelGGL(k_kill_listed, dim3(nblk(n, 256)), dim3(256), 0, c->stream, c->s0.as<int>(), (long long)n,
                     c->n_edges, c->edge_alive.as<unsigned char>());
  live_lists_after_edge_deaths(c);
  HIPCHK(hipStreamSynchronize(c->stream));
  c->have_corrected = false;
  return AMG_OK;
}

#define CLIP_MAX 64
template <class View>
__global__ void k_clip_mark(View g, long long n_nodes, int min_length, const unsigned long long* __restrict__ acc,
                            const unsigned int* __restrict__ comp_live,
                            const unsigned char* __restrict__ protect,
                            unsigned char* __restrict__ kill) {
  long long i = (long long)blockIdx.x * blockDim.x + threadIdx.x;
  if (i >= n_nodes || !g.n_alive[i]) return;
  int n = (int)i;
  if (node_degree(g, n) != 1) return;
  int d0 = (g.n_first[n] & 1ll) ? -1 : 1;
  int path[CLIP_MAX];
  int len = 0;
  path[len++] = n;
  int tgt = -1, td = 0;
  int r = lin_step(g, n, d0 == -1, &tgt, &td);
  while (r == 2 && tgt != n) {
    if (len >= min_length) return;
    path[len++] = tgt;
    r = lin_step(g, tgt, td == 1, &tgt, &td);
  }
  r = lin_step(g, n, d0 == 1, &tgt, &td);
  while (r == 2 && tgt != n) {
    if (len >= min_length) return;
    path[len++] = tgt;
    r = lin_step(g, tgt, td == 1, &tgt, &td);
  }
  if (!(len > 0 && len < min_length)) return;
  const double thr = ((double)acc[0] / (double)acc[1]) * 1.5;
  bool all_high = true;
  for (int j = 0; j < len; ++j) all_high = all_high && ((double)g.n_cov[path[j]] > thr);
  if (all_high) return;
  if (comp_live) {
    int distinct = 0;
    for (int j = 0; j < len; ++j) {
      bool dup = false;
      for (int q = 0; q < j; ++q) dup = dup || (path[q] == path[j]);
      distinct += dup ? 0 : 1;
    }
    if ((unsigned int)distinct == comp_live[g.n_comp[n]]) return;
  } else {
    bool closed = true;
    for (int j = 0; j < len && closed; ++j)
      for (int side = 0; side < 2 && closed; ++side) {
        const long long row = 2ll * path[j] + side;
        const int cnt = row_count(g, row);
        for (int q = 0; q < cnt && closed; ++q) {
          const int t = row_target(g, row, q);
          bool in = false;
          for (int m = 0; m < len; ++m) in = in || (path[m] == t);
          closed = in;
        }
      }
    if (closed) return;
  }
  for (int j = 0; j < len; ++j)
    if (!protect || !protect[path[j]]) kill[path[j]] = 1;
}

__device__ __forceinline__ void block_add_cov(unsigned long long sum, unsigned long long n, unsigned long long* __restrict__ acc) {
  __shared__ unsigned long long s_part[2][4];
  for (int d = 32; d > 0; d >>= 1) {
    sum += __shfl_xor(sum, d, 64);
    n += __shfl_xor(n, d, 64);
  }
  if ((threadIdx.x & 63) == 0) {
    s_part[0][threadIdx.x >> 6] = sum;
    s_part[1][threadIdx.x >> 6] = n;
  }
  __syncthreads();
  if (threadIdx.x == 0) {
    const unsigned long long n_all = s_part[1][0] + s_part[1][1] + s_part[1][2] + s_part[1][3];
    if (n_all) {
      atomicAdd(&acc[0], s_part[0][0] + s_part[0][1] + s_part[0][2] + s_part[0][3]);
      atomicAdd(&acc[1], n_all);
    }
  }
}

__global__ void k_comp_hist(const int* __restrict__ comp, const unsigned char* __restrict__ alive,
                            const unsigned int* __restrict__ cov, long long n, unsigned int min_cov,
                            unsigned int* __restrict__ live_cnt, unsigned int* __restrict__ high_cnt,
                            unsigned long long* __restrict__ acc ) {
  int cid = -1;
  unsigned int n_live = 0, n_high = 0;
  unsigned long long s_cov = 0, s_n = 0;
  for (long long i = (long long)blockIdx.x * blockDim.x + threadIdx.x; i < n; i += (long long)gridDim.x * blockDim.x) {
    if (!alive[i]) continue;
    if (acc) {
      s_cov += cov[i];
      s_n += 1;
    }
    const int id = comp[i];
    if (id != cid) {
      if (cid >= 0) {
        atomicAdd(&live_cnt[cid], n_live);
        if (high_cnt && n_high) atomicAdd(&high_cnt[cid], n_high);
      }
      cid = id;
      n_live = n_high = 0;
    }
    ++n_live;
    n_high += (high_cnt && cov[i] >= min_cov) ? 1u : 0u;
  }
  const int lane = threadIdx.x & 63;
  if (acc) block_add_cov(s_cov, s_n, acc);
  bool active = cid >= 0;
  unsigned long long todo = __ballot(active);
  while (todo) {
    const int leader = __ffsll((long long)todo) - 1;
    const int lc = __shfl(cid, leader, 64);
    const bool same = active && cid == lc;
    const unsigned long long m = __ballot(same);
    unsigned int sl = same ? n_live : 0u, sh = same ? n_high : 0u;
    for (int d = 32; d > 0; d >>= 1) {
      sl += __shfl_xor(sl, d, 64);
      sh += __shfl_xor(sh, d, 64);
    }
    if (lane == leader) {
      atomicAdd(&live_cnt[lc], sl);
      if (high_cnt && sh) atomicAdd(&high_cnt[lc], sh);
    }
    active = active && !same;
    todo &= ~m;
  }
}

__global__ __launch_bounds__(256) void k_cov_acc(const unsigned char* __restrict__ alive, const unsigned int* __restrict__ cov,
                                                 long long n, unsigned long long* __restrict__ acc) {
  unsigned long long s_cov = 0, s_n = 0;
  for (long long i = (long long)blockIdx.x * blockDim.x + threadIdx.x; i < n; i += (long long)gridDim.x * blockDim.x)
    if (alive[i]) {
      s_cov += cov[i];
      s_n += 1;
    }
  block_add_cov(s_cov, s_n, acc);
}

__global__ void k_scatter_ids(const unsigned char* __restrict__ killed, const long long* __restrict__ pos,
                              long long n, int* __restrict__ out) {
  long long i = (long long)blockIdx.x * blockDim.x + threadIdx.x;
  if (i < n && killed[i]) out[pos[i]] = (int)i;
}

static int finish_kill(amg_ctx* c, int64_t* n_removed, int32_t* removed_ids) {
  hipStream_t st = c->stream;
  const long long D = c->n_nodes;
  AMGCHK(c->s2.ensure((size_t)(D + 2) * sizeof(long long)));
  AMGCHK(prim_exscan_apply_kill(c, c->s0.as<unsigned char>(), c->node_alive.as<unsigned char>(), c->s2.as<long long>(),
                                (size_t)D));
  long long total = 0;
  {
    FetchList l;
    l.add(c->s2.as<long long>() + D);
    AMGCHK(fetch(c, l, reinterpret_cast<unsigned long long*>(&total)));
  }
  if (n_removed) *n_removed = total;
  if (removed_ids && total > 0) {
    AMGCHK(c->s3.ensure((size_t)total * sizeof(int)));
    hipLaunchKernelGGL(k_scatter_ids, dim3(nblk(D, 256)), dim3(256), 0, st, c->s0.as<unsigned char>(),
                       c->s2.as<long long>(), D, c->s3.as<int>());
    HIPCHK(hipMemcpyAsync(removed_ids, c->s3.p, (size_t)total * sizeof(int), hipMemcpyDeviceToHost, st));
  }
  if (total > 0) AMGCHK(apply_removals(c, 0));
  if (removed_ids && total > 0) HIPCHK(hipStreamSynchronize(st));
  return AMG_OK;
}

extern "C" int amg_remove_short_linear_paths(amg_ctx* c, int32_t min_length, const uint8_t* protect,
                                             int64_t* n_removed, int32_t* removed_ids) {
  NEED_BUILT(c);
  if (min_length < 1 || min_length > CLIP_MAX)
    return amg_fail(AMG_E_ARG, "min_length must be in [1, %d]", CLIP_MAX);
  hipStream_t st = c->stream;
  const long long D = c->n_nodes;
  if (n_removed) *n_removed = 0;
  if (D == 0) return AMG_OK;
  stages_reset(c);
  const bool by_labels = !c->pristine || getenv("AMG_CLIP_COMPONENTS");
  if (by_labels) AMGCHK(ensure_components(c));
  const bool light = c->live_lists == LiveLists::Absent && !getenv("AMG_CLIP_LISTS");
  stage_begin(c, "clip");
  unsigned long long* acc = c->status.as<unsigned long long>() + ST_COV_SUM;
  AMGCHK(c->s0.ensure((size_t)D + 8));
  if (by_labels) AMGCHK(c->s4.ensure((size_t)(c->n_components + 2) * sizeof(unsigned int)));
  {
    ClearList cl;
    cl.add(acc, 2 * sizeof(unsigned long long));
    cl.add(c->s0.p, (size_t)D + 8);
    if (by_labels) cl.add(c->s4.p, (size_t)(c->n_components + 2) * sizeof(unsigned int));
    if (light) AMGCHK(row_summary_reserve(c, &cl));
    AMGCHK(clear_many(c, cl));
  }
  RView summary;
  if (light) summary = row_summary(c);
  if (by_labels)
    hipLaunchKernelGGL(k_comp_hist, dim3(nblk(D, 256) < 256u ? nblk(D, 256) : 256u), dim3(256), 0, st, c->node_comp.as<int>(),
                       c->node_alive.as<unsigned char>(), c->node_cov.as<unsigned int>(), D, 0u,
                       c->s4.as<unsigned int>(), (unsigned int*)nullptr, acc);
  else
    hipLaunchKernelGGL(k_cov_acc, dim3(nblk(D, 2048) < 256u ? nblk(D, 2048) : 256u), dim3(256), 0, st,
                       c->node_alive.as<unsigned char>(), c->node_cov.as<unsigned int>(), D, acc);
  unsigned char* d_protect = nullptr;
  if (protect) {
    AMGCHK(c->s5.ensure((size_t)D + 8));
    HIPCHK(hipMemcpyAsync(c->s5.p, protect, (size_t)D, hipMemcpyHostToDevice, st));
    d_protect = c->s5.as<unsigned char>();
  }
  const unsigned int* comp_live = by_labels ? c->s4.as<unsigned int>() : nullptr;
  if (light) {
    hipLaunchKernelGGL(k_clip_mark<RView>, dim3(nblk(D, 128)), dim3(128), 0, st, summary, D, (int)min_length, acc, comp_live,
                       d_protect, c->s0.as<unsigned char>());
  } else {
    AMGCHK(ensure_live_adj(c));
    hipLaunchKernelGGL(k_clip_mark<GView>, dim3(nblk(D, 128)), dim3(128), 0, st, make_view(c), D, (int)min_length, acc,
                       comp_live, d_protect, c->s0.as<unsigned char>());
  }
  int r = finish_kill(c, n_removed, removed_ids);
  stage_end(c);
  c->have_corrected = false;
  return r;
}

__global__ void k_kill_low_components(const int* __restrict__ comp, const unsigned char* __restrict__ alive,
                                      const unsigned int* __restrict__ high_cnt, long long n,
                                      unsigned char* __restrict__ kill) {
  long long i = (long long)blockIdx.x * blockDim.x + threadIdx.x;
  if (i < n && alive[i] && high_cnt[comp[i]] == 0) kill[i] = 1;
}

extern "C" int amg_remove_low_coverage_components(amg_ctx* c, uint32_t min_cov) {
  NEED_BUILT(c);
  hipStream_t st = c->stream;
  const long long D = c->n_nodes;
  if (D == 0) return AMG_OK;
  AMGCHK(ensure_components(c));
  size_t nc = (size_t)(c->n_components + 2);
  AMGCHK(c->s0.ensure((size_t)D + 8));
  AMGCHK(c->s4.ensure(2 * nc * sizeof(unsigned int)));
  {
    ClearList cl;
    cl.add(c->s0.p, (size_t)D + 8);
    cl.add(c->s4.p, 2 * nc * sizeof(unsigned int));
    AMGCHK(clear_many(c, cl));
  }
  unsigned int* live = c->s4.as<unsigned int>();
  unsigned int* high = live + nc;
  hipLaunchKernelGGL(k_comp_hist, dim3(nblk(D, 256) < 256u ? nblk(D, 256) : 256u), dim3(256), 0, st, c->node_comp.as<int>(),
                     c->node_alive.as<unsigned char>(), c->node_cov.as<unsigned int>(), D, min_cov, live, high,
                     (unsigned long long*)nullptr);
  hipLaunchKernelGGL(k_kill_low_components, dim3(nblk(D, 256)), dim3(256), 0, st, c->node_comp.as<int>(),
                     c->node_alive.as<unsigned char>(), high, D, c->s0.as<unsigned char>());
  c->have_corrected = false;
  return finish_kill(c, nullptr, nullptr);
}
```

amira_amd/csrc/amg_internal.h:

```cpp
#pragma once
#include <cstdint>
#include <cstdio>
#include <cstring>
#include <string>
#include <vector>

#include <hip/hip_runtime.h>

#include "../../include/amg.h"

extern thread_local std::string g_amg_err;
int amg_fail(int code, const char* fmt, ...);

#define HIPCHK(call)                                                                   \
  do {                                                                                 \
    hipError_t e_ = (call);                                                            \
    if (e_ != hipSuccess)                                                              \
      return amg_fail(AMG_E_HIP, "%s:%d %s -> %s", __FILE__, __LINE__, #call,          \
                      hipGetErrorString(e_));                                          \
  } while (0)
#define AMGCHK(call)                 \
  do {                               \
    int r_ = (call);                 \
    if (r_ != AMG_OK) return r_;     \
  } while (0)

struct DevBuf {
  void* p = nullptr;
  size_t cap = 0;
  void* own_p = nullptr;
  size_t own_cap = 0;
  bool borrowed = false;
  void borrow(const void* ptr, size_t bytes) {
    if (!borrowed) {
      own_p = p;
      own_cap = cap;
    }
    p = const_cast<void*>(ptr);
    cap = bytes;
    borrowed = true;
  }
  void unborrow() {
    if (!borrowed) return;
    p = own_p;
    cap = own_cap;
    own_p = nullptr;
    own_cap = 0;
    borrowed = false;
  }
  int ensure(size_t bytes) {
    unborrow();
    if (bytes <= cap) return AMG_OK;
    if (p) (void)hipFree(p);
    p = nullptr;
    cap = 0;
    size_t want = bytes + bytes / 8 + 256;
    hipError_t e = hipMalloc(&p, want);
    if (e != hipSuccess) {
      p = nullptr;
      return amg_fail(AMG_E_NOMEM, "hipMalloc(%zu) failed: %s", want, hipGetErrorString(e));
    }
    cap = want;
    return AMG_OK;
  }
  void release() {
    unborrow();
    if (p) (void)hipFree(p);
    p = nullptr;
    cap = 0;
  }
  template <class T>
  T* as() const {
    return reinterpret_cast<T*>(p);
  }
};

struct __attribute__((aligned(32))) Slot {
  unsigned long long key;
  unsigned long long first_inv;
  unsigned int count;
  int id;
  unsigned long long pad;
};
static_assert(sizeof(Slot) == 32, "slot must be one 32-byte sector");

enum {
  ST_NODE_INSERTS = 0,
  ST_PAIR_INSERTS = 1,
  ST_OVERFLOW = 2,
  ST_PALINDROME = 3,
  ST_COLLISION = 4,
  ST_N_WINDOWS = 5,
  ST_N_SHORT = 6,
  ST_COMPACT_A = 7,
  ST_COMPACT_B = 8,
  ST_MISC = 9,
  ST_BADINPUT = 10,
  ST_COV_SUM = 11,
  ST_WORDS = 16
};

struct StageTime {
  const char* name;
  hipEvent_t a, b;
  float ms;
};

static const uint64_t kAmgSeed0 = 0x9E3779B97F4A7C15ull;
static const unsigned int kProbeLimit = 1024;

struct BuildSwitches {
  bool head_tiles_set = false;
  long long head_tiles = 0;
  int claim_shards = -1;
  bool tight_bits = false;
  bool key_fp = false;
  bool node_buckets = true;
  bool generic_k = false;
  bool rank_sort = false;
  int edge_lone = -1;
  bool edge_home = true;
  bool no_derive = false;
  int weak_fp = 0;
  bool count_inline = false;
  int count_list_seg = 1 << 30;
  bool count_debug = false;
};
BuildSwitches read_build_switches();

enum Overflow { OV_NONE = 0, OV_NODE_TABLE = 1, OV_EDGE_TABLE = 2, OV_COLLISION = 3 };
static inline int overflowed(Overflow* which, Overflow cause) { return *which = cause, AMG_E_OVERFLOW; }

struct DistState;
struct BubbleState;
struct SketchState;
struct PopState;

enum class LiveLists {
  Absent,
  Current,
  BehindNodes,
};

struct amg_ctx {
  int device = 0;
  hipStream_t stream = nullptr;

  DevBuf tokens;
  DevBuf read_off;
  DevBuf gene_start;
  DevBuf gene_end;
  DevBuf read_len;
  bool have_pos = false, have_read_len = false;
  DevBuf pos_off, c_pos_off;
  DevBuf pos1_s, pos1_e;
  bool pos_identity = true;
  int64_t pos_n0 = 0, pos1_used = 0, c_pos1_used = 0;
  int64_t n_reads = 0, n_tokens = 0;
  int32_t two_v = 0;

  bool built = false;
  int32_t k = 0;
  uint64_t seed = kAmgSeed0;
  int64_t n_windows = 0, n_short = 0;
  int64_t n_nodes = 0, n_pairs = 0, n_edges = 0, n_components = 0;
  int64_t node_slots = 0, edge_slots = 0, retries = 0;
  int64_t node_hint = 0;
  int64_t c_node_bound = 0;
  int c_node_bound_k = 0;
  int64_t hint_bound = 0;
  int hint_bound_k = 0;
  bool filtered_build = false;
  int64_t n_local_nodes = 0, n_local_pairs = 0;
  int64_t tok_base = 0;
  int64_t tok_total = 0;

  DevBuf node_tab;
  DevBuf edge_tab;
  DevBuf tok_slot;
  DevBuf tok_node;
  DevBuf tok_dir;
  DevBuf tok_pair;
  bool packed_nodes = false;
  int weak_fp_builds = 0;
  bool dist_mode = false;
  bool count_inline = false;
  DevBuf node_tokens;
  DevBuf node_cov;
  DevBuf node_first;
  DevBuf node_comp;
  DevBuf node_alive;
  DevBuf edge_src, edge_tgt;
  DevBuf edge_sdir, edge_tdir;
  DevBuf edge_cov;
  DevBuf edge_alive;
  DevBuf pair_key, pair_first;
  DevBuf pair_cnt;
  DevBuf adj_off;
  DevBuf adj_edge;
  DevBuf ladj;
  DevBuf ladj_rows;
  DevBuf ladj_pos, ladj_keys;
  DevBuf hub_bits;
  LiveLists live_lists = LiveLists::Absent;
  bool comp_valid = false, adj_valid = false;
  bool pristine = false;
  DevBuf read_fix;

  bool have_corrected = false;
  bool pos0_own = false;
  int64_t c_reads = 0, c_tokens = 0;
  DevBuf c_tokens_buf, c_read_off, c_orig, c_changed, c_gstart, c_gend, c_read_len;

  DevBuf c_src, rd_src;
  bool c_derivable = false;
  bool derive_ready = false;
  bool derived = false;
  bool dist_candidate = false;
  bool edge_own_deaths = false;
  DevBuf alt_tok_node, alt_tok_dir, alt_ntok, alt_ncov, alt_nfirst, alt_nalive, alt_pkey, alt_pfirst, alt_pcnt;

  bool exact_keys = false;
  int x_bits = 0;
  bool x_fp = false;
  bool x_two = false;
  int x_kbits = 0;
  int64_t x_nspace = 0, x_espace = 0;
  int64_t x_max_claims = 0, x_max_eclaims = 0;
  bool dist_x = false;
  DevBuf x_first, x_slot;
  DevBuf x_final;
  DevBuf x_efirst, x_eslot;
  DevBuf x_ecnt;
  DevBuf x_ncnt;
  int64_t rank_flags_clean = 0;
  DevBuf x_ftag;
  DevBuf f_ctrs;
  DevBuf x_efinal;
  DevBuf x_first_all;
  bool comp_from_claims = false;

  int world = 1;
  uint32_t dist_min_node = 1, dist_min_edge = 1;
  DistState* dist = nullptr;
  BubbleState* bub = nullptr;
  SketchState* sk = nullptr;
  PopState* pop = nullptr;

  bool match_valid = false;
  int64_t match_total = 0, match_npat = 0;
  DevBuf match_read, match_pos, match_off, match_wave;

  DevBuf status;
  unsigned long long* mail_host = nullptr;
  unsigned long long* mail_dev = nullptr;
  unsigned long long mail_ticket = 0;
  DevBuf sort_tmp;
  DevBuf scan_state;
  unsigned long long scan_tickets = 0;
  unsigned int scan_epoch = 0;
  DevBuf s0, s1, s2, s3, s4, s5;
  DevBuf nw_big;
  DevBuf gap_rec;
  DevBuf gm_mask;
  DevBuf gm_tab;
  DevBuf gm_res;
  DevBuf gm_list;
  DevBuf gm_q;
  DevBuf gm_pool;
  DevBuf gm_gene;
  DevBuf gm_fail;
  DevBuf gm_ctr;
  DevBuf nw_rec;
  DevBuf routes_dev;
  bool have_routes = false;
  int64_t routes[AMG_ROUTE_WORDS] = {0};
  DevBuf bnd_bits;
  DevBuf cnt_state;
  bool cnt_hint_reset = false;
  DevBuf cnt_list;
  int cnt_sweeps[2] = {4, 4};
  int cnt_launched[2] = {0, 0};

  BuildSwitches sw;
  std::vector<StageTime> stages;
  bool timing = true;
};

struct amg_seqs {
  int device = 0;
  DevBuf bases, off;
  int64_t n = 0, total = 0;
};

int prim_sort_u64_u32(amg_ctx* c, const unsigned long long* kin, unsigned long long* kout,
                      const unsigned int* vin, unsigned int* vout, size_t n, int end_bit);
int prim_sort_u32_u32(amg_ctx* c, const unsigned int* kin, unsigned int* kout,
                      const unsigned int* vin, unsigned int* vout, size_t n, int end_bit);
struct ClearList;
int prim_exscan_i64(amg_ctx* c, const long long* in, long long* out, size_t n);
int prim_exscan_u32_to_i64(amg_ctx* c, const unsigned int* in, long long* out, size_t n);
int prim_exscan_u32_pair(amg_ctx* c, const unsigned int* in_a, long long* out_a, const unsigned int* in_b, long long* out_b,
                         size_t n);
int prim_exscan_i64_pair(amg_ctx* c, const long long* in_a, long long* out_a, const long long* in_b, long long* out_b,
                         size_t n);
int prim_exscan_bytes_set(amg_ctx* c, const unsigned char* in, long long* out, size_t n, const ClearList* side = nullptr);
int prim_exscan_apply_kill(amg_ctx* c, unsigned char* kill, unsigned char* alive, long long* out, size_t n);
int prim_exscan_keep_and_len(amg_ctx* c, const unsigned int* len, long long* out_keep, long long* out_off, size_t n);
int prim_exscan_flag_words(amg_ctx* c, const unsigned char* flags, unsigned int* bits, long long* out, size_t n_words);
int prim_exscan_bits_popc(amg_ctx* c, const unsigned int* bits, long long* out, size_t n_words);
int prim_exscan_pair_width(amg_ctx* c, const unsigned long long* pkey, long long* out, size_t n_pairs);
int prim_exscan_emit_edges(amg_ctx* c, const unsigned long long* pkey, const unsigned int* pcnt,
                           const unsigned long long* pfirst, size_t n_pairs, long long* total, int* e_src, int* e_tgt,
                           signed char* e_sdir, signed char* e_tdir, unsigned int* e_cov, unsigned char* e_alive,
                           const ClearList* side);

#define CLEAR_MAX 8
struct ClearList {
  void* p[CLEAR_MAX];
  unsigned long long bytes[CLEAR_MAX];
  int n = 0;
  bool overflow = false;
  unsigned int fill[CLEAR_MAX];
  void add(void* ptr, size_t b, unsigned int value = 0u) {
    if (b == 0) return;
    if (n >= CLEAR_MAX) {
      overflow = true;
      return;
    }
    p[n] = ptr;
    bytes[n] = (unsigned long long)((b + 3) & ~(size_t)3);
    fill[n] = value;
    ++n;
  }
};
int clear_many(amg_ctx* c, const ClearList& l);

#define FETCH_MAX 96
struct FetchList {
  const unsigned long long* p[FETCH_MAX];
  int n = 0;
  bool overflow = false;
  void add(const void* q) {
    if (n < FETCH_MAX)
      p[n++] = static_cast<const unsigned long long*>(q);
    else
      overflow = true;
  }
  void add_words(const void* q, int words) { for (int i = 0; i < words; ++i) add(static_cast<const unsigned long long*>(q) + i); }
};
int fetch(amg_ctx* c, const FetchList& l, unsigned long long* out, const ClearList* filler = nullptr);
static_assert(ST_WORDS <= FETCH_MAX, "fetch_status reads the status words in one list");
int fetch_status(amg_ctx* c, unsigned long long* out , const ClearList* filler = nullptr);
int stream_wait(amg_ctx* c);

void stage_begin(amg_ctx* c, const char* name);
void stage_end(amg_ctx* c);
void stages_reset(amg_ctx* c);

struct GView {
  const int2* lent;
  const int4* lrows;
  const unsigned char* n_alive;
  const unsigned int* n_cov;
  const int* n_tok;
  const long long* n_first;
  const int* n_comp;
  int k, flip;
};
int ensure_live_adj(amg_ctx* c);
GView make_view(amg_ctx* c);
void live_lists_after_node_deaths(amg_ctx* c);
void live_lists_after_edge_deaths(amg_ctx* c);
void live_lists_after_build(amg_ctx* c);
void bubbles_release(amg_ctx* c);
void sketch_release(amg_ctx* c);
void pop_release(amg_ctx* c);

void dist_release(amg_ctx* c);
int derive_from_previous(amg_ctx* c, int k, bool* done);
int derive_local(amg_ctx* c, int k, long long own_lo, long long own_tokens, const long long* d_bases, int world,
                 long long* bounds_host, long long* D2_out, long long* P2_out, bool* ok);
int derive_commit(amg_ctx* c, long long D2, long long P2);

uint64_t pow2_at_least(uint64_t x);
uint64_t slots_for(uint64_t n_keys);
void bs_size_tables(amg_ctx* c);
int grow_after_overflow(amg_ctx* c, Overflow cause);
int bs_read_stats(amg_ctx* c, int k, const ClearList* also = nullptr);
int bs_alloc_nodes(amg_ctx* c, long long D);
int bs_alloc_pairs(amg_ctx* c, long long P);
int bs_finish_from_pairs(amg_ctx* c);
int bs_nodes_pass(amg_ctx* c, int k, Overflow* which);
int bs_nodes_rank_local(amg_ctx* c);
int bs_edges_pass(amg_ctx* c, Overflow* which);
int bs_pairs_from_local(amg_ctx* c);
int ensure_components(amg_ctx* c);
int ensure_adjacency(amg_ctx* c);
enum CountKind { CountNodes = 0, CountEdgeClasses = 1 };
enum CountIds {
  IdsPlain,
  IdsClaimsMarked,
};
int count_ids(amg_ctx* c, CountKind what, CountIds form, int* ids, long long n, long long n_ids, unsigned int* out,
              const Slot* gather_tab = nullptr);
#define COUNT_LEARN_WORDS 8
bool count_learn_add(amg_ctx* c, FetchList* l);
void count_learn_take(amg_ctx* c, const unsigned long long* done );
bool bx_applicable(const amg_ctx* c, int k);
bool bx_fits(const amg_ctx* c, int k);
bool bx_tuple_fits(const amg_ctx* c, int k);
int bx_nodes(amg_ctx* c, int k, Overflow* which);
int bx_nodes_upsert(amg_ctx* c, int k, Overflow* which, bool sharded = false, bool rank_follows = true);
int bx_nodes_rank(amg_ctx* c);
int bx_edges(amg_ctx* c, Overflow* which, unsigned int min_edge_cov = 0);
int bx_nodes_filtered(amg_ctx* c, int k, unsigned int min_cov, Overflow* which);
int bx_flag_dead_reads(amg_ctx* c);
int bx_edges_upsert(amg_ctx* c, Overflow* which, bool lone = false, bool sharded = false, bool rank_follows = true);
int bx_edges_rank(amg_ctx* c, unsigned int min_edge_cov = 0, bool nodes_counted = false);
int bx_node_count(amg_ctx* c, bool tag);
int bx_bits(const amg_ctx* c, int k);
int bx_pairs_rank(amg_ctx* c, const int* final_of_claim, int* efinal);
int bx_components_from_claims(amg_ctx* c);
int bs_count_by_slot(amg_ctx* c, CountKind what, const int* slots, int* ids_scratch, long long n, Slot* tab,
                     const unsigned int* slot_sorted, long long n_ids, unsigned int* out);

#define NEED_BUILT(c)                                                     \
  do {                                                                    \
    if (!(c)) return amg_fail(AMG_E_ARG, "null ctx");                     \
    if (!(c)->built) return amg_fail(AMG_E_STATE, "amg_build first");     \
    HIPCHK(hipSetDevice((c)->device));                                    \
  } while (0)

static inline unsigned int nblk(long long n, int per) {
  long long b = (n + per - 1) / per;
  return (unsigned int)(b < 1 ? 1 : b);
}

static inline int ilog2_ceil(uint64_t x) {
  int b = 0;
  while ((1ull << b) < x && b < 63) ++b;
  return b;
}
```

amira_amd/csrc/amg_scan.hip:

```cpp
#include "amg_device.h"

#define SC_THREADS 512
#define SC_ROWS 16
#define SC_TILE (SC_THREADS * SC_ROWS)
#define SC_VAL_MASK ((1ull << 48) - 1ull)

__device__ __forceinline__ unsigned long long sc_word(unsigned int state, unsigned int epoch, unsigned long long v) {
  return ((unsigned long long)state << 62) | ((unsigned long long)(epoch & 0x3fffu) << 48) | (v & SC_VAL_MASK);
}

#define SC_NO_LIM 0x7fffffffffffffffll
template <class T>
struct LoadArr {
  const T* in;
  using Raw = T;
  __device__ __forceinline__ long long lim() const { return SC_NO_LIM; }
  __device__ __forceinline__ Raw raw(long long i) const { return in[i]; }
  __device__ __forceinline__ unsigned long long val(long long, Raw r) const { return (unsigned long long)r; }
};
template <class T>
struct LoadArrN {
  const T* in;
  long long n;
  using Raw = T;
  __device__ __forceinline__ long long lim() const { return n; }
  __device__ __forceinline__ Raw raw(long long i) const { return in[i]; }
  __device__ __forceinline__ unsigned long long val(long long, Raw r) const { return (unsigned long long)r; }
};
struct LoadNonzero {
  const unsigned int* in;
  long long n;
  using Raw = unsigned int;
  __device__ __forceinline__ long long lim() const { return n; }
  __device__ __forceinline__ Raw raw(long long i) const { return in[i]; }
  __device__ __forceinline__ unsigned long long val(long long, Raw r) const { return r != 0u ? 1ull : 0ull; }
};
struct LoadByteSet {
  const unsigned char* in;
  long long n;
  using Raw = unsigned char;
  __device__ __forceinline__ long long lim() const { return n; }
  __device__ __forceinline__ Raw raw(long long i) const { return in[i]; }
  __device__ __forceinline__ unsigned long long val(long long, Raw r) const { return r != 0 ? 1ull : 0ull; }
};
struct LoadApplyKill {
  unsigned char* kill;
  unsigned char* alive;
  long long n;
  struct Raw {
    unsigned int kill, alive;
  };
  __device__ __forceinline__ long long lim() const { return n; }
  __device__ __forceinline__ Raw raw(long long i) const { return Raw{kill[i], alive[i]}; }
  __device__ __forceinline__ unsigned long long val(long long i, Raw r) const {
    const bool f = r.kill != 0u && r.alive != 0u;
    if (f) alive[i] = 0;
    kill[i] = f ? 1 : 0;
    return f ? 1ull : 0ull;
  }
};
struct LoadFlagWords {
  const unsigned char* flags;
  unsigned int* bits;
  long long n_words;
  struct Raw {
    uint4 a, b;
  };
  __device__ __forceinline__ long long lim() const { return n_words; }
  __device__ __forceinline__ Raw raw(long long i) const {
    const uint4* p = reinterpret_cast<const uint4*>(flags + 32 * i);
    return Raw{p[0], p[1]};
  }
  __device__ __forceinline__ unsigned long long val(long long i, const Raw& r) const {
    auto nib = [](unsigned int x) { return (x & 1u) | ((x >> 7) & 2u) | ((x >> 14) & 4u) | ((x >> 21) & 8u); };
    const uint4 a = r.a, b = r.b;
    const unsigned int w = nib(a.x) | (nib(a.y) << 4) | (nib(a.z) << 8) | (nib(a.w) << 12) | (nib(b.x) << 16) |
                           (nib(b.y) << 20) | (nib(b.z) << 24) | (nib(b.w) << 28);
    bits[i] = w;
    return (unsigned long long)__popc(w);
  }
};
struct LoadBitsPopc {
  const unsigned int* bits;
  long long n_words;
  using Raw = unsigned int;
  __device__ __forceinline__ long long lim() const { return n_words; }
  __device__ __forceinline__ Raw raw(long long i) const { return bits[i]; }
  __device__ __forceinline__ unsigned long long val(long long, Raw r) const { return (unsigned long long)__popc(r); }
};
struct LoadPairWidth {
  const unsigned long long* pkey;
  long long n_pairs;
  using Raw = unsigned long long;
  __device__ __forceinline__ long long lim() const { return n_pairs; }
  __device__ __forceinline__ Raw raw(long long i) const { return pkey[i]; }
  __device__ __forceinline__ unsigned long long val(long long, Raw key) const {
    const unsigned int lo = (unsigned int)((key >> 32) & 0x7fffffffull);
    const unsigned int hi = (unsigned int)(key & 0xffffffffull) - 1u;
    return lo == hi ? 1ull : 2ull;
  }
};

struct LoadNone {
  using Raw = unsigned char;
  __device__ __forceinline__ long long lim() const { return 0; }
  __device__ __forceinline__ Raw raw(long long) const { return 0; }
  __device__ __forceinline__ unsigned long long val(long long, Raw) const { return 0ull; }
};

template <class L>
__device__ __forceinline__ void load_rows(const L& ld, long long w0, long long n, int lane, unsigned long long* x) {
  const long long lim = n < ld.lim() ? n : ld.lim();
  if (w0 >= lim) {
#pragma unroll
    for (int r = 0; r < SC_ROWS; ++r) x[r] = 0ull;
    return;
  }
  typename L::Raw raw[SC_ROWS];
#pragma unroll
  for (int r = 0; r < SC_ROWS; ++r) {
    const long long i = w0 + r * 64 + lane;
    raw[r] = ld.raw(i < lim ? i : lim - 1);
  }
  asm volatile("" ::: "memory");
#pragma unroll
  for (int r = 0; r < SC_ROWS; ++r) {
    const long long i = w0 + r * 64 + lane;
    x[r] = i < lim ? ld.val(i, raw[r]) : 0ull;
  }
}

struct EmitOut {
  long long* out;
  struct Pre {};
  __device__ __forceinline__ Pre pre(long long) const { return Pre{}; }
  __device__ __forceinline__ void operator()(long long i, unsigned long long excl, const Pre&) const {
    out[i] = (long long)excl;
  }
};
struct EmitEdges {
  const unsigned long long* pkey;
  const unsigned int* pcnt;
  const unsigned long long* pfirst;
  long long n_pairs;
  long long* total;
  int* e_src;
  int* e_tgt;
  signed char* e_sdir;
  signed char* e_tdir;
  unsigned int* e_cov;
  unsigned char* e_alive;
  struct Pre {
    unsigned long long key, first;
    unsigned int cnt;
  };
  __device__ __forceinline__ Pre pre(long long i) const {
    const long long j = i < n_pairs ? i : 0;
    return Pre{pkey[j], pfirst[j], pcnt[j]};
  }
  __device__ __forceinline__ void operator()(long long i, unsigned long long excl, const Pre& p) const {
    if (i >= n_pairs) {
      total[0] = (long long)excl;
      return;
    }
    const unsigned long long key = p.key, first = p.first;
    const int lo = (int)((key >> 32) & 0x7fffffffull);
    const int hi = (int)((key & 0xffffffffull) - 1ull);
    const int X = (first & 1ull) ? lo : hi, Y = (first & 1ull) ? hi : lo;
    const signed char dX = (first & 2ull) ? 1 : -1, dY = (first & 4ull) ? 1 : -1;
    const long long e = (long long)excl;
    const unsigned int cnt = p.cnt;
    e_src[e] = X; e_tgt[e] = Y; e_sdir[e] = dX; e_tdir[e] = dY; e_alive[e] = 1;
    if (lo == hi) {
      e_cov[e] = cnt * 2u;
    } else {
      e_cov[e] = cnt;
      e_src[e + 1] = Y; e_tgt[e + 1] = X; e_sdir[e + 1] = (signed char)-dY;
      e_tdir[e + 1] = (signed char)-dX; e_cov[e + 1] = cnt; e_alive[e + 1] = 1;
    }
  }
};
template <class Load, class LoadB, class Emit>
__global__ __launch_bounds__(SC_THREADS) void k_exscan(Load load, Emit emit_a, long long n_a, LoadB load_b,
                                                        long long* __restrict__ out_b, long long n_b, long long tiles_a,
                                                        unsigned long long* counter, unsigned long long ticket_base,
                                                        unsigned long long* status, unsigned int epoch, ClearArgs side) {
  __shared__ unsigned long long s_wave[SC_THREADS / 64];
  __shared__ unsigned long long s_excl;
  __shared__ unsigned int s_tile;
  const int lane = threadIdx.x & 63, wave = threadIdx.x >> 6;
  if (threadIdx.x == 0) s_tile = (unsigned int)(atomicAdd(counter, 1ull) - ticket_base);
  __syncthreads();
  const long long tile = s_tile;
  const bool second = tile >= tiles_a;
  const long long seg0 = second ? tiles_a : 0;
  const long long n = second ? n_b : n_a;
  const long long w0 = (tile - seg0) * SC_TILE + (long long)wave * (64 * SC_ROWS);
  unsigned long long x[SC_ROWS], inc[SC_ROWS];
  if (second)
    load_rows(load_b, w0, n, lane, x);
  else
    load_rows(load, w0, n, lane, x);
  unsigned long long row_off = 0;
#pragma unroll
  for (int r = 0; r < SC_ROWS; ++r) {
    unsigned long long v = x[r];
#pragma unroll
    for (int d = 1; d < 64; d <<= 1) {
      const unsigned long long o = __shfl_up(v, d, 64);
      if (lane >= d) v += o;
    }
    inc[r] = v + row_off;
    row_off += __shfl(v, 63, 64);
  }
  if (lane == 0) s_wave[wave] = row_off;
  __syncthreads();
  unsigned long long wave_excl = 0, tile_sum = 0;
#pragma unroll
  for (int w = 0; w < SC_THREADS / 64; ++w) {
    const unsigned long long s = s_wave[w];
    wave_excl += w < wave ? s : 0ull;
    tile_sum += s;
  }
  typename Emit::Pre pre[SC_ROWS];
  if (!second) {
#pragma unroll
    for (int r = 0; r < SC_ROWS; ++r) {
      const long long i = w0 + r * 64 + lane;
      pre[r] = emit_a.pre(i < n ? i : n - 1);
    }
  }
  if (wave == 0) {
    unsigned long long excl = 0;
    if (tile == seg0) {
      if (lane == 0)
        __hip_atomic_store(status + tile, sc_word(2u, epoch, tile_sum), __ATOMIC_RELAXED, __HIP_MEMORY_SCOPE_AGENT);
    } else {
      if (lane == 0)
        __hip_atomic_store(status + tile, sc_word(1u, epoch, tile_sum), __ATOMIC_RELAXED, __HIP_MEMORY_SCOPE_AGENT);
      for (long long look = tile - 1;; look -= 64) {
        const long long idx = look - lane;
        unsigned int state = 2u;
        unsigned long long val = 0;
        if (idx >= seg0) {
          unsigned long long w;
          do {
            w = __hip_atomic_load(status + idx, __ATOMIC_RELAXED, __HIP_MEMORY_SCOPE_AGENT);
          } while ((unsigned int)((w >> 48) & 0x3fffu) != (epoch & 0x3fffu) || (w >> 62) == 0ull);
          state = (unsigned int)(w >> 62);
          val = w & SC_VAL_MASK;
        }
        const unsigned long long full = __ballot(state == 2u);
        const int stop = full ? __ffsll((long long)full) - 1 : 63;
        unsigned long long part = lane <= stop ? val : 0ull;
#pragma unroll
        for (int d = 32; d > 0; d >>= 1) part += __shfl_xor(part, d, 64);
        excl += part;
        if (full) break;
      }
      if (lane == 0)
        __hip_atomic_store(status + tile, sc_word(2u, epoch, excl + tile_sum), __ATOMIC_RELAXED, __HIP_MEMORY_SCOPE_AGENT);
    }
    if (lane == 0) s_excl = excl;
  }
  __syncthreads();
  const unsigned long long base = s_excl + wave_excl;
#pragma unroll
  for (int r = 0; r < SC_ROWS; ++r) {
    const long long i = w0 + r * 64 + lane;
    if (i < n) {
      if (second)
        out_b[i] = (long long)(base + inc[r] - x[r]);
      else
        emit_a(i, base + inc[r] - x[r], pre[r]);
    }
  }
  if (side.n) clear_args_part(side, blockIdx.x, gridDim.x);
}

template <class Load, class Emit, class LoadB = LoadNone>
static int exscan_emit(amg_ctx* c, Load load, Emit emit, size_t n, LoadB load_b = LoadNone{}, long long* out_b = nullptr,
                       size_t n_b = 0, const ClearList* side = nullptr) {
  if (side && side->overflow) return amg_fail(AMG_E_ARG, "exscan: more than %d ranges in one list", CLEAR_MAX);
  if (n == 0 && n_b == 0) return side ? clear_many(c, *side) : AMG_OK;
  const unsigned long long tiles_a = (n + SC_TILE - 1) / SC_TILE;
  const unsigned long long tiles = tiles_a + (n_b + SC_TILE - 1) / SC_TILE;
  const size_t need = (size_t)(tiles + 8) * sizeof(unsigned long long);
  if (need > c->scan_state.cap || c->scan_epoch >= 0x3fffu) {
    if (need > c->scan_state.cap) {
      AMGCHK(c->scan_state.ensure(need * 2));
      c->scan_tickets = 0;
      HIPCHK(hipMemsetAsync(c->scan_state.p, 0, c->scan_state.cap, c->stream));
    } else {
      HIPCHK(hipMemsetAsync(c->scan_state.as<unsigned long long>() + 8, 0,
                            c->scan_state.cap - 8 * sizeof(unsigned long long), c->stream));
    }
    c->scan_epoch = 0;
  }
  const unsigned int epoch = ++c->scan_epoch;
  unsigned long long* st = c->scan_state.as<unsigned long long>();
  ClearArgs sa;
  sa.n = 0;
  if (side) sa = clear_args(*side);
  hipLaunchKernelGGL((k_exscan<Load, LoadB, Emit>), dim3((unsigned int)tiles), dim3(SC_THREADS), 0, c->stream, load, emit,
                     (long long)n, load_b, out_b, (long long)n_b, (long long)tiles_a, st, c->scan_tickets, st + 8, epoch, sa);
  c->scan_tickets += tiles;
  return AMG_OK;
}

template <class Load, class LoadB = LoadNone>
static int exscan(amg_ctx* c, Load load, long long* out, size_t n, LoadB load_b = LoadNone{}, long long* out_b = nullptr,
                  size_t n_b = 0) {
  return exscan_emit(c, load, EmitOut{out}, n, load_b, out_b, n_b);
}

int prim_exscan_u32_to_i64(amg_ctx* c, const unsigned int* in, long long* out, size_t n) {
  return exscan(c, LoadArr<unsigned int>{in}, out, n);
}

int prim_exscan_i64(amg_ctx* c, const long long* in, long long* out, size_t n) {
  return exscan(c, LoadArr<long long>{in}, out, n);
}

int prim_exscan_u32_pair(amg_ctx* c, const unsigned int* in_a, long long* out_a, const unsigned int* in_b, long long* out_b,
                         size_t n) {
  return exscan(c, LoadArrN<unsigned int>{in_a, (long long)n}, out_a, n + 1, LoadArrN<unsigned int>{in_b, (long long)n}, out_b,
                n + 1);
}

int prim_exscan_i64_pair(amg_ctx* c, const long long* in_a, long long* out_a, const long long* in_b, long long* out_b,
                         size_t n) {
  return exscan(c, LoadArrN<long long>{in_a, (long long)n}, out_a, n + 1, LoadArrN<long long>{in_b, (long long)n}, out_b,
                n + 1);
}

int prim_exscan_bytes_set(amg_ctx* c, const unsigned char* in, long long* out, size_t n, const ClearList* side) {
  return exscan_emit(c, LoadByteSet{in, (long long)n}, EmitOut{out}, n + 1, LoadNone{}, nullptr, 0, side);
}

int prim_exscan_apply_kill(amg_ctx* c, unsigned char* kill, unsigned char* alive, long long* out, size_t n) {
  return exscan(c, LoadApplyKill{kill, alive, (long long)n}, out, n + 1);
}

int prim_exscan_keep_and_len(amg_ctx* c, const unsigned int* len, long long* out_keep, long long* out_off, size_t n) {
  return exscan(c, LoadNonzero{len, (long long)n}, out_keep, n + 1, LoadArrN<unsigned int>{len, (long long)n}, out_off, n + 1);
}

int prim_exscan_flag_words(amg_ctx* c, const unsigned char* flags, unsigned int* bits, long long* out, size_t n_words) {
  return exscan(c, LoadFlagWords{flags, bits, (long long)n_words}, out, n_words + 1);
}

int prim_exscan_bits_popc(amg_ctx* c, const unsigned int* bits, long long* out, size_t n_words) {
  return exscan(c, LoadBitsPopc{bits, (long long)n_words}, out, n_words + 1);
}

int prim_exscan_pair_width(amg_ctx* c, const unsigned long long* pkey, long long* out, size_t n_pairs) {
  return exscan(c, LoadPairWidth{pkey, (long long)n_pairs}, out, n_pairs + 1);
}

int prim_exscan_emit_edges(amg_ctx* c, const unsigned long long* pkey, const unsigned int* pcnt,
                           const unsigned long long* pfirst, size_t n_pairs, long long* total, int* e_src, int* e_tgt,
                           signed char* e_sdir, signed char* e_tdir, unsigned int* e_cov, unsigned char* e_alive,
                           const ClearList* side) {
  return exscan_emit(c, LoadPairWidth{pkey, (long long)n_pairs},
                     EmitEdges{pkey, pcnt, pfirst, (long long)n_pairs, total, e_src, e_tgt, e_sdir, e_tdir, e_cov, e_alive},
                     n_pairs + 1, LoadNone{}, nullptr, 0, side);
}

extern "C" int amg_scan_probe(amg_ctx* c, int kind, const void* in, int64_t n, int64_t* out, void* aux) {
  if (!c || n < 0 || (n > 0 && !in) || !out) return amg_fail(AMG_E_ARG, "scan_probe: bad arguments");
  size_t in_bytes = 0, out_words = (size_t)n + 1, aux_bytes = 0;
  switch (kind) {
    case 0: in_bytes = (size_t)n; aux_bytes = (size_t)n; break;
    case 1: in_bytes = 8 * (size_t)n; break;
    case 2: in_bytes = 32 * (size_t)n; aux_bytes = 4 * (size_t)n; break;
    case 3: in_bytes = 2 * (size_t)n; aux_bytes = 2 * (size_t)n; break;
    case 4: in_bytes = 4 * (size_t)n; out_words = 2 * ((size_t)n + 1); break;
    case 5: in_bytes = 20 * (size_t)n; out_words = 1; aux_bytes = 30 * (size_t)n; break;
    default: return amg_fail(AMG_E_ARG, "scan_probe: unknown kind %d", kind);
  }
  char* d = nullptr;
  const size_t in_cap = (in_bytes + 255) & ~(size_t)255, out_cap = (out_words * 8 + 255) & ~(size_t)255;
  const size_t aux_cap = (aux_bytes + 256) & ~(size_t)255;
  HIPCHK(hipMalloc(reinterpret_cast<void**>(&d), in_cap + out_cap + aux_cap));
  char* din = d;
  long long* dout = reinterpret_cast<long long*>(d + in_cap);
  char* daux = d + in_cap + out_cap;
  int rc = AMG_OK;
  do {
    if (in_bytes && hipMemcpy(din, in, in_bytes, hipMemcpyHostToDevice) != hipSuccess) { rc = amg_fail(AMG_E_HIP, "h2d"); break; }
    if (hipMemset(daux, 0xff, aux_cap) != hipSuccess || hipDeviceSynchronize() != hipSuccess) {
      rc = amg_fail(AMG_E_HIP, "memset");
      break;
    }
    switch (kind) {
      case 0: {
        ClearList side;
        side.add(daux, (size_t)n);
        rc = prim_exscan_bytes_set(c, reinterpret_cast<unsigned char*>(din), dout, (size_t)n, &side);
        break;
      }
      case 1: rc = prim_exscan_pair_width(c, reinterpret_cast<unsigned long long*>(din), dout, (size_t)n); break;
      case 2:
        rc = prim_exscan_flag_words(c, reinterpret_cast<unsigned char*>(din), reinterpret_cast<unsigned int*>(daux), dout,
                                    (size_t)n);
        break;
      case 3:
        if (n && (hipMemcpy(daux, din, 2 * (size_t)n, hipMemcpyDeviceToDevice) != hipSuccess ||
                  hipDeviceSynchronize() != hipSuccess)) {
          rc = amg_fail(AMG_E_HIP, "d2d");
          break;
        }
        rc = prim_exscan_apply_kill(c, reinterpret_cast<unsigned char*>(daux), reinterpret_cast<unsigned char*>(daux) + n,
                                    dout, (size_t)n);
        break;
      case 4:
        rc = prim_exscan_keep_and_len(c, reinterpret_cast<unsigned int*>(din), dout, dout + n + 1, (size_t)n);
        break;
      case 5: {
        const size_t E = 2 * (size_t)n;
        int* src = reinterpret_cast<int*>(daux);
        int* tgt = src + E;
        unsigned int* cov = reinterpret_cast<unsigned int*>(tgt + E);
        signed char* sdir = reinterpret_cast<signed char*>(cov + E);
        signed char* tdir = sdir + E;
        unsigned char* alive = reinterpret_cast<unsigned char*>(tdir + E);
        rc = prim_exscan_emit_edges(c, reinterpret_cast<unsigned long long*>(din),
                                    reinterpret_cast<unsigned int*>(din + 16 * (size_t)n),
                                    reinterpret_cast<unsigned long long*>(din + 8 * (size_t)n), (size_t)n, dout, src, tgt,
                                    sdir, tdir, cov, alive, nullptr);
        break;
      }
    }
    if (rc != AMG_OK) break;
    if (hipStreamSynchronize(c->stream) != hipSuccess) { rc = amg_fail(AMG_E_HIP, "scan_probe: stream"); break; }
    if (hipMemcpy(out, dout, out_words * 8, hipMemcpyDeviceToHost) != hipSuccess) { rc = amg_fail(AMG_E_HIP, "d2h"); break; }
    if (aux && aux_bytes && hipMemcpy(aux, daux, aux_bytes, hipMemcpyDeviceToHost) != hipSuccess) { rc = amg_fail(AMG_E_HIP, "d2h"); break; }
  } while (false);
  (void)hipFree(d);
  return rc;
}
```

amira_amd/engine.py:

```python
import ctypes as C
import weakref

import numpy as np

from . import _ffi
from ._ffi import check, ptr


class Engine:
    def __init__(self, device=0):
        self._h = C.c_void_p()
        check(_ffi.lib.amg_create(int(device), C.byref(self._h)))
        self.device = device
        self._leases = weakref.WeakSet()
        self._pool_when_free = False
        self.pop_rewrite_stats = {"calls": 0, "reads": 0, "rewritten": 0, "declined": 0}

    def close(self):
        if self._h:
            _ffi.lib.amg_destroy(self._h)
            self._h = C.c_void_p()

    def __del__(self):
        try:
            self.close()
        except Exception:
            pass

    def set_reads(self, tokens, read_offsets, two_v):
        tokens = np.ascontiguousarray(tokens, dtype=np.int32)
        read_offsets = np.ascontiguousarray(read_offsets, dtype=np.int64)
        check(_ffi.lib.amg_set_reads(self._h, ptr(tokens), ptr(read_offsets),
                                     len(read_offsets) - 1, int(two_v), 0))

    def set_reads_device(self, tokens_ptr, read_offsets_ptr, n_reads, two_v, borrow=False):
        check(_ffi.lib.amg_set_reads(self._h, C.c_void_p(tokens_ptr), C.c_void_p(read_offsets_ptr),
                                     int(n_reads), int(two_v), 2 if borrow else 1))

    def set_positions(self, gene_start, gene_end, read_len=None):
        rl = None if read_len is None else np.ascontiguousarray(read_len, dtype=np.int64)
        if getattr(gene_start, "dtype", None) == np.int32 and getattr(gene_end, "dtype", None) == np.int32:
            gs, ge = np.ascontiguousarray(gene_start), np.ascontiguousarray(gene_end)
            check(_ffi.lib.amg_set_positions32(self._h, ptr(gs), ptr(ge), ptr(rl), 0))
            return
        gs = np.ascontiguousarray(gene_start, dtype=np.int64)
        ge = np.ascontiguousarray(gene_end, dtype=np.int64)
        check(_ffi.lib.amg_set_positions(self._h, ptr(gs), ptr(ge), ptr(rl), 0))

    def set_positions32_device(self, gs_ptr, ge_ptr, rl_ptr):
        check(_ffi.lib.amg_set_positions32(self._h, C.c_void_p(gs_ptr), C.c_void_p(ge_ptr),
                                           C.c_void_p(rl_ptr) if rl_ptr else None, 1))

    def set_read_lengths(self, read_len):
        rl = np.ascontiguousarray(read_len, dtype=np.int64)
        check(_ffi.lib.amg_set_read_lengths(self._h, ptr(rl), 0))

    def set_positions_device(self, gs_ptr, ge_ptr, rl_ptr, borrow=False):
        check(_ffi.lib.amg_set_positions(self._h, C.c_void_p(gs_ptr), C.c_void_p(ge_ptr),
                                         C.c_void_p(rl_ptr) if rl_ptr else None, 2 if borrow else 1))

    def build(self, k):
        check(_ffi.lib.amg_build(self._h, int(k)))

    def build_filtered(self, k, min_node_cov, min_edge_cov):
        check(_ffi.lib.amg_build_filtered(self._h, int(k), max(int(min_node_cov), 0), max(int(min_edge_cov), 0)))

    @staticmethod
    def build_multi(engines, ks):
        n = len(engines)
        assert n == len(ks) and n >= 1
        handles = (C.c_void_p * n)(*[e._h for e in engines])
        arr = (C.c_int32 * n)(*[int(k) for k in ks])
        check(_ffi.lib.amg_build_multi(handles, arr, n))

    def finalize(self):
        check(_ffi.lib.amg_finalize(self._h))

    def sizes(self):
        nr, nt = C.c_int64(0), C.c_int64(0)
        check(_ffi.lib.amg_sizes(self._h, C.byref(nr), C.byref(nt)))
        return nr.value, nt.value

    def graph_sizes(self):
        nn, ne, k = C.c_int64(0), C.c_int64(0), C.c_int32(0)
        check(_ffi.lib.amg_graph_sizes(self._h, C.byref(nn), C.byref(ne), C.byref(k)))
        return nn.value, ne.value, k.value

    def counts(self):
        c = _ffi.Counts()
        check(_ffi.lib.amg_counts(self._h, C.byref(c)))
        return c.as_dict()

    def sync(self):
        check(_ffi.lib.amg_sync(self._h))

    def stream(self):
        return _ffi.lib.amg_stream(self._h)

    def set_timing(self, on):
        check(_ffi.lib.amg_set_timing(self._h, 1 if on else 0))

    def timings(self):
        names = (C.c_char_p * 64)()
        ms = (C.c_float * 64)()
        n = _ffi.lib.amg_last_timings(self._h, names, ms, 64)
        return [(names[i].decode(), float(ms[i])) for i in range(max(n, 0))]

    @staticmethod
    def _take(buf, key, shape, dtype):
        n = int(np.prod(shape))
        if buf is not None and key in buf:
            a = buf[key]
            assert a.dtype == dtype and a.size >= n and a.flags["C_CONTIGUOUS"], key
            return a.reshape(-1)[:n].reshape(shape)
        return np.empty(shape, dtype)

    def nodes(self, buf=None):
        D, _, k = self.graph_sizes()
        out = {
            "tokens": self._take(buf, "tokens", (D, k), np.int32), "coverage": self._take(buf, "coverage", (D,), np.uint32),
            "first_token": self._take(buf, "first_token", (D,), np.int64), "first_dir": self._take(buf, "first_dir", (D,), np.int8),
            "component": self._take(buf, "component", (D,), np.int32), "alive": self._take(buf, "alive", (D,), np.uint8),
        }
        check(_ffi.lib.amg_get_nodes(self._h, ptr(out["tokens"]), ptr(out["coverage"]),
                                     ptr(out["first_token"]), ptr(out["first_dir"]),
                                     ptr(out["component"]), ptr(out["alive"])))
        return out

    def edges(self, buf=None):
        E = self.graph_sizes()[1]
        out = {"src": self._take(buf, "src", (E,), np.int32), "tgt": self._take(buf, "tgt", (E,), np.int32),
               "sdir": self._take(buf, "sdir", (E,), np.int8), "tdir": self._take(buf, "tdir", (E,), np.int8),
               "coverage": self._take(buf, "ecoverage", (E,), np.uint32), "alive": self._take(buf, "ealive", (E,), np.uint8)}
        check(_ffi.lib.amg_get_edges(self._h, ptr(out["src"]), ptr(out["tgt"]), ptr(out["sdir"]),
                                     ptr(out["tdir"]), ptr(out["coverage"]), ptr(out["alive"])))
        return out

    def read_nodes(self, buf=None):
        T = self.sizes()[1]
        node, d = self._take(buf, "tok_node", (T,), np.int32), self._take(buf, "tok_dir", (T,), np.int8)
        check(_ffi.lib.amg_get_read_nodes(self._h, ptr(node), ptr(d)))
        return node, d

    def read_node_ids(self, buf=None):
        T = self.sizes()[1]
        node = self._take(buf, "tok_node", (T,), np.int32)
        check(_ffi.lib.amg_get_read_nodes(self._h, ptr(node), None))
        return node

    def read_node_ids_of(self, first_token, n_windows):
        first_token = np.ascontiguousarray(first_token, np.int64)
        starts = np.zeros(len(first_token) + 1, np.int64)
        np.cumsum(n_windows, out=starts[1:])
        out = np.empty(int(starts[-1]), np.int32)
        check(_ffi.lib.amg_get_read_nodes_rows(self._h, ptr(first_token), ptr(starts), len(first_token), ptr(out)))
        return out, starts

    def read_dirs(self, buf=None):
        T = self.sizes()[1]
        d = self._take(buf, "tok_dir", (T,), np.int8)
        check(_ffi.lib.amg_get_read_nodes(self._h, None, ptr(d)))
        return d

    def node_adj(self):
        D, E, _ = self.graph_sizes()
        off, ids = np.empty(2 * D + 1, np.int64), np.empty(E, np.int32)
        check(_ffi.lib.amg_get_node_adj(self._h, ptr(off), ptr(ids)))
        return off, ids

    def node_reads(self):
        D = self.graph_sizes()[0]
        off = np.empty(D + 1, np.int64)
        idx = np.empty(max(self.sizes()[1], 1), np.int32)
        check(_ffi.lib.amg_get_node_reads(self._h, ptr(off), ptr(idx)))
        return off, idx[:int(off[-1]) if D else 0]

    def reads_to_correct(self):
        f = np.empty(self.sizes()[0], np.uint8)
        check(_ffi.lib.amg_get_reads_to_correct(self._h, ptr(f)))
        return f

    def filter(self, min_node_cov, min_edge_cov):
        check(_ffi.lib.amg_filter(self._h, int(min_node_cov), int(min_edge_cov)))

    def remove_nodes(self, ids):
        ids = np.ascontiguousarray(ids, dtype=np.int32)
        check(_ffi.lib.amg_remove_nodes(self._h, ptr(ids), len(ids)))

    def remove_edges(self, ids):
        ids = np.ascontiguousarray(ids, dtype=np.int32)
        check(_ffi.lib.amg_remove_edges(self._h, ptr(ids), len(ids)))

    def remove_short_linear_paths(self, min_length, protect=None, want_ids=True):
        n = C.c_int64(0)
        pr = None if protect is None else np.ascontiguousarray(protect, dtype=np.uint8)
        if not want_ids:
            check(_ffi.lib.amg_remove_short_linear_paths(self._h, int(min_length), ptr(pr), C.byref(n), None))
            return n.value
        ids = np.empty(self.graph_sizes()[0], np.int32)
        check(_ffi.lib.amg_remove_short_linear_paths(self._h, int(min_length), ptr(pr),
                                                     C.byref(n), ptr(ids)))
        return ids[: n.value].copy()

    def remove_low_coverage_components(self, min_cov):
        check(_ffi.lib.amg_remove_low_coverage_components(self._h, int(min_cov)))

    def correct_reads(self):
        nr, nt = C.c_int64(0), C.c_int64(0)
        check(_ffi.lib.amg_correct_reads(self._h, C.byref(nr), C.byref(nt)))
        return nr.value, nt.value

    ROUTES = ("gapped", "by_lean", "by_fast", "by_general", "on_not_tried", "on_windows", "on_runs", "on_memo_unfit",
              "on_records", "on_combos", "on_cand", "lean_no_slots", "lean_answers", "lean_long", "lean_other",
              "no_memo_slots", "memo_questions", "memo_spilled", "memo_unfit", "pool_retries", "keep_orig",
              "nw_fast", "nw_lds", "nw_global")

    def correct_routes(self):
        out = np.zeros(len(self.ROUTES), np.int64)
        check(_ffi.lib.amg_correct_routes(self._h, _ffi.ptr(out), len(out)))
        return dict(zip(self.ROUTES, out.tolist()))

    NW_ROUTES = ("none", "equal_length", "certificate", "fill", "general_lds", "general_global")

    def nw_probe(self, x, y, pos, read_len=None, keep_orig=None, flags=0):
        (xt, xo), (yt, yo) = ((np.ascontiguousarray(t, np.int32), np.ascontiguousarray(o, np.int64)) for t, o in (x, y))
        ps, pe = (np.ascontiguousarray(p, np.int64) for p in pos)
        n = len(xo) - 1
        assert len(yo) == n + 1 and len(ps) == len(pe) == len(yt)
        rl = None if read_len is None else np.ascontiguousarray(read_len, np.int64)
        keep = None if keep_orig is None else np.ascontiguousarray(keep_orig, np.uint8)
        lens = np.diff(xo)
        total = int(lens.sum() if keep is None else lens[keep == 0].sum())
        gs, ge = np.zeros(max(total, 1), np.int64), np.zeros(max(total, 1), np.int64)
        route, state = np.zeros(max(n, 1), np.uint8), np.zeros(8, np.int64)
        check(_ffi.lib.amg_nw_probe(self._h, n, _ffi.ptr(xt) if xt.size else None, _ffi.ptr(xo), _ffi.ptr(yt),
                                    _ffi.ptr(yo), _ffi.ptr(ps), _ffi.ptr(pe), _ffi.ptr(rl), _ffi.ptr(keep), int(flags),
                                    _ffi.ptr(gs), _ffi.ptr(ge), _ffi.ptr(route), _ffi.ptr(state)))
        return gs[:total], ge[:total], route[:n], state

    def corrected(self, n_reads, n_tokens, with_positions, buf=None, pos32=False):
        out = {"tokens": self._take(buf, "c_tokens", (n_tokens,), np.int32),
               "read_offsets": self._take(buf, "c_read_offsets", (n_reads + 1,), np.int64),
               "orig_read": self._take(buf, "c_orig_read", (n_reads,), np.int32),
               "changed": self._take(buf, "c_changed", (n_reads,), np.uint8)}
        gs = ge = None
        if with_positions and pos32:
            gs = self._take(buf, "c_gene_start32", (n_tokens,), np.int32)
            ge = self._take(buf, "c_gene_end32", (n_tokens,), np.int32)
            check(_ffi.lib.amg_get_corrected(self._h, ptr(out["tokens"]), ptr(out["read_offsets"]),
                                             ptr(out["orig_read"]), ptr(out["changed"]), None, None))
            rc = _ffi.lib.amg_get_corrected_positions32(self._h, ptr(gs), ptr(ge))
            if rc == 0:
                out["gene_start"], out["gene_end"] = gs, ge
                return out
            if rc != -2:
                check(rc)
        if with_positions:
            gs = self._take(buf, "c_gene_start", (n_tokens,), np.int64)
            ge = self._take(buf, "c_gene_end", (n_tokens,), np.int64)
        check(_ffi.lib.amg_get_corrected(self._h, ptr(out["tokens"]), ptr(out["read_offsets"]),
                                         ptr(out["orig_read"]), ptr(out["changed"]), ptr(gs), ptr(ge)))
        out["gene_start"], out["gene_end"] = gs, ge
        return out

    def corrected32(self, n_reads, n_tokens, buf=None):
        out = {"tokens": self._take(buf, "c_tokens", (n_tokens,), np.int32),
               "read_offsets": self._take(buf, "c_read_offsets", (n_reads + 1,), np.int64),
               "orig_read": self._take(buf, "c_orig_read", (n_reads,), np.int32),
               "changed": self._take(buf, "c_changed", (n_reads,), np.uint8),
               "pos_src": self._take(buf, "c_pos_src", (n_reads,), np.int64)}
        ns = self._take(buf, "c_new_start", (n_tokens,), np.int32)
        ne = self._take(buf, "c_new_end", (n_tokens,), np.int32)
        n = C.c_int64(0)
        check(_ffi.lib.amg_get_corrected32(self._h, ptr(out["tokens"]), ptr(out["read_offsets"]), ptr(out["orig_read"]),
                                           ptr(out["changed"]), ptr(out["pos_src"]), ptr(ns), ptr(ne), C.byref(n)))
        out["new_start"], out["new_end"] = ns[: n.value], ne[: n.value]
        return out

    def corrected_index(self, n_reads):
        out = {"read_offsets": np.empty(n_reads + 1, np.int64), "orig_read": np.empty(n_reads, np.int32),
               "changed": np.empty(n_reads, np.uint8)}
        check(_ffi.lib.amg_get_corrected(self._h, None, ptr(out["read_offsets"]), ptr(out["orig_read"]),
                                         ptr(out["changed"]), None, None))
        return out

    def adopt_corrected(self):
        check(_ffi.lib.amg_adopt_corrected(self._h))

    def set_reads_from_corrected(self, src):
        check(_ffi.lib.amg_set_reads_from_corrected(self._h, src._h))

    def match_patterns(self, which, patterns):
        n = len(patterns)
        offs = np.zeros(n + 1, np.int64)
        np.cumsum([len(p) for p in patterns], out=offs[1:])
        flat = np.fromiter((x for p in patterns for x in p), dtype=np.int32, count=int(offs[-1]))
        hit_off = np.zeros(n + 1, np.int64)
        check(_ffi.lib.amg_match_patterns(self._h, int(which), ptr(flat) if len(flat) else None,
                                          ptr(offs), n, ptr(hit_off), None, None))
        total = int(hit_off[-1])
        hr, hp = np.empty(total, np.int32), np.empty(total, np.int32)
        if total:
            check(_ffi.lib.amg_match_patterns(self._h, int(which), ptr(flat) if len(flat) else None,
                                              ptr(offs), n, ptr(hit_off), ptr(hr), ptr(hp)))
        return hit_off, hr, hp

    def minhash(self, segments, set_ids, ksize, scaled):
        out = {int(s): set() for s in set_ids}
        if not segments:
            return out
        blobs = [s.encode() if isinstance(s, str) else bytes(s) for s in segments]
        offs = np.zeros(len(blobs) + 1, np.int64)
        np.cumsum([len(b) for b in blobs], out=offs[1:])
        bases = np.frombuffer(b"".join(blobs), dtype=np.uint8)
        if len(bases) == 0:
            return out
        sets = np.ascontiguousarray(set_ids, dtype=np.int32)
        n = C.c_int64(0)
        cap = len(bases) if int(scaled) <= 1 else min(len(bases), 4 * len(bases) // int(scaled) + 1024)
        while True:
            o_set, o_hash = np.empty(cap, np.int32), np.empty(cap, np.uint64)
            check(_ffi.lib.amg_minhash(self._h, ptr(bases), ptr(offs), ptr(sets), len(blobs), int(ksize), int(scaled),
                                       ptr(o_set), ptr(o_hash), cap, C.byref(n)))
            if n.value <= cap:
                break
            cap = n.value
        if n.value == 0:
            return out
        o_set, o_hash = o_set[: n.value], o_hash[: n.value]
        order = np.lexsort((o_hash, o_set))
        o_set, o_hash = o_set[order], o_hash[order]
        cuts = np.flatnonzero(np.diff(o_set)) + 1
        for ids, hs in zip(np.split(o_set, cuts), np.split(o_hash, cuts)):
            out[int(ids[0])] = set(np.unique(hs).tolist())
        return out

    def junction_paths(self, max_distance):
        sizes = (C.c_int64 * 4)()
        check(_ffi.lib.amg_junction_paths(self._h, int(max_distance), sizes))
        J, P, N, flags = (int(x) for x in sizes)
        out = {"junction_node": np.empty(J, np.int32), "junction_dir": np.empty(J, np.int8),
               "path_start": np.empty(P, np.int32), "path_off": np.zeros(P + 1, np.int64),
               "path_node": np.empty(N, np.int32), "path_dir": np.empty(N, np.int8), "flags": flags}
        check(_ffi.lib.amg_get_junction_paths(self._h, ptr(out["junction_node"]), ptr(out["junction_dir"]),
                                              ptr(out["path_start"]), ptr(out["path_off"]), ptr(out["path_node"]),
                                              ptr(out["path_dir"])))
        return out

    def path_sketch_overlaps(self, seqs, row_to_seq, ksize, scaled, path_off, path_node, pair_a, pair_b):
        path_off = np.ascontiguousarray(path_off, np.int64)
        path_node = np.ascontiguousarray(path_node, np.int32)
        pair_a, pair_b = np.ascontiguousarray(pair_a, np.int32), np.ascontiguousarray(pair_b, np.int32)
        rts = None if row_to_seq is None else np.ascontiguousarray(row_to_seq, np.int32)
        n_paths, n_pairs = len(path_off) - 1, len(pair_a)
        size, common = np.zeros(max(n_paths, 1), np.int64), np.zeros(max(n_pairs, 1), np.int64)
        check(_ffi.lib.amg_path_sketch_overlaps(self._h, seqs._h, ptr(rts), int(ksize), int(scaled), n_paths, ptr(path_off),
                                                ptr(path_node), n_pairs, ptr(pair_a), ptr(pair_b), ptr(size), ptr(common)))
        return size[:n_paths], common[:n_pairs]

    POP_MAX_LIST, POP_MAX_ITEMS, POP_MAX_READ = 128, 1 << 20, 1 << 24

    @classmethod
    def pop_rewrite_declines(cls, k, better, worse, reads):
        return (not 1 <= k <= 16 or not 1 <= len(better) <= cls.POP_MAX_ITEMS or not 1 <= len(reads) <= cls.POP_MAX_ITEMS
                or any(not k <= len(x) <= cls.POP_MAX_LIST for lists in (better, worse) for x in lists)
                or any(len(x) > cls.POP_MAX_READ for x in reads))

    def pop_rewrite(self, k, two_v, better_tok, better_off, worse_tok, worse_off, interest, read_tok, read_off, read_op):
        better_tok, worse_tok = np.ascontiguousarray(better_tok, np.int32), np.ascontiguousarray(worse_tok, np.int32)
        better_off, worse_off = np.ascontiguousarray(better_off, np.int64), np.ascontiguousarray(worse_off, np.int64)
        read_tok, read_off = np.ascontiguousarray(read_tok, np.int32), np.ascontiguousarray(read_off, np.int64)
        read_op = np.ascontiguousarray(read_op, np.int32)
        flags = None if interest is None else np.ascontiguousarray(interest, np.uint8)
        assert flags is None or len(flags) == two_v
        n_ops, n_reads = len(better_off) - 1, len(read_off) - 1
        assert len(worse_off) == n_ops + 1 and len(read_op) == n_reads
        cap = int(read_off[-1])
        if n_ops > 0 and n_reads > 0 and 0 <= int(read_op.min()) and int(read_op.max()) < n_ops:
            cap += int(np.diff(better_off)[read_op].sum())
        out = {"op_veto": np.zeros(max(n_ops, 1), np.uint8), "status": np.zeros(max(n_reads, 1), np.uint8),
               "first_shared": np.zeros(max(n_reads, 1), np.int32), "last_shared": np.zeros(max(n_reads, 1), np.int32),
               "out_off": np.zeros(max(n_reads, 0) + 1, np.int64), "out_tok": np.empty(max(cap, 1), np.int32),
               "out_src": np.empty(max(cap, 1), np.int32)}
        n_out = C.c_int64(0)
        check(_ffi.lib.amg_pop_rewrite(self._h, int(k), int(two_v), n_ops, ptr(better_tok), ptr(better_off), ptr(worse_tok),
                                       ptr(worse_off), ptr(flags), n_reads, ptr(read_tok), ptr(read_off), ptr(read_op), cap,
                                       ptr(out["op_veto"]), ptr(out["status"]), ptr(out["first_shared"]),
                                       ptr(out["last_shared"]), ptr(out["out_off"]), ptr(out["out_tok"]),
                                       ptr(out["out_src"]), C.byref(n_out)))
        for key, n in (("op_veto", n_ops), ("status", n_reads), ("first_shared", n_reads), ("last_shared", n_reads),
                       ("out_tok", n_out.value), ("out_src", n_out.value)):
            out[key] = out[key][:n]
        stats = self.pop_rewrite_stats
        stats["calls"] += 1
        stats["reads"] += n_reads
        stats["rewritten"] += int((out["status"] == 2).sum())
        return out

    @staticmethod
    def dist_unique_id():
        buf = C.create_string_buffer(_ffi.UNIQUE_ID_BYTES)
        check(_ffi.lib.amg_dist_unique_id(buf, _ffi.UNIQUE_ID_BYTES))
        return buf.raw

    def dist_init(self, unique_id, rank, world):
        assert len(unique_id) == _ffi.UNIQUE_ID_BYTES
        check(_ffi.lib.amg_dist_init(self._h, C.c_char_p(unique_id), int(rank), int(world)))

    def dist_init_external(self, rank, world):
        check(_ffi.lib.amg_dist_init_external(self._h, int(rank), int(world)))

    def dist_merge(self, k, min_node_cov=1, min_edge_cov=1):
        check(_ffi.lib.amg_dist_merge(self._h, int(k), max(int(min_node_cov), 1), max(int(min_edge_cov), 1)))

    def dist_merge_begin(self, k, min_node_cov=1, min_edge_cov=1):
        check(_ffi.lib.amg_dist_merge_begin(self._h, int(k), max(int(min_node_cov), 1), max(int(min_edge_cov), 1)))

    def dist_merge_next(self):
        x = _ffi.Xfer()
        rc = _ffi.lib.amg_dist_merge_next(self._h, C.byref(x))
        if rc < 0:
            check(rc)
        return x if rc == 1 else None

    @staticmethod
    def dist_merge_local(engines, k, min_node_cov=1, min_edge_cov=1):
        n = len(engines)
        handles = (C.c_void_p * n)(*[e._h for e in engines])
        check(_ffi.lib.amg_dist_merge_local(handles, n, int(k), max(int(min_node_cov), 1), max(int(min_edge_cov), 1)))

    def dist_finalize(self):
        check(_ffi.lib.amg_dist_finalize(self._h))

    def copy_d2h(self, dev_ptr, host_array):
        check(_ffi.lib.amg_copy_d2h(self._h, C.c_void_p(dev_ptr), ptr(host_array), host_array.nbytes))

    def copy_h2d(self, dev_ptr, host_array):
        check(_ffi.lib.amg_copy_h2d(self._h, C.c_void_p(dev_ptr), ptr(host_array), host_array.nbytes))

    def dist_stats(self, reset=True):
        out = (C.c_int64 * 8)()
        check(_ffi.lib.amg_dist_stats(self._h, out, 1 if reset else 0))
        return {"host_waits": out[0], "exchanges": out[1], "a2a_bytes_per_peer": out[2], "back_bytes_per_peer": out[3],
                "ag_bytes_contributed": out[4], "repeated_builds": out[5], "a2a_bytes_sent": out[6],
                "derived_builds": out[7]}

    def dist_phase_ms(self, on=True):
        names = (C.c_char_p * 32)()
        ms = (C.c_double * 32)()
        n = _ffi.lib.amg_dist_phase_ms(self._h, 1 if on else 0, names, ms, 32)
        return {names[i].decode(): float(ms[i]) for i in range(max(n, 0))}


_ENGINE_POOL = {}


def acquire_engine(device):
    free = _ENGINE_POOL.setdefault(device, [])
    while free:
        engine = free.pop()
        if engine._h:
            return engine
    return Engine(device)


def release_engine(engine):
    if engine is None or not engine._h:
        return
    if len(engine._leases) > 0:
        engine._pool_when_free = True
        return
    engine._pool_when_free = False
    _ENGINE_POOL.setdefault(engine.device, []).append(engine)


def lease_done(engine, lease):
    engine._leases.discard(lease)
    if engine._pool_when_free and len(engine._leases) == 0:
        release_engine(engine)


class Sequences:

    def __init__(self, sequences, device=0):
        n = len(sequences)
        ptrs = (C.c_void_p * max(n, 1))()
        lens = np.zeros(max(n, 1), np.int64)
        as_utf8 = C.pythonapi.PyUnicode_AsUTF8AndSize
        as_utf8.restype, as_utf8.argtypes = C.c_void_p, [C.py_object, C.POINTER(C.c_ssize_t)]
        size = C.c_ssize_t(0)
        keep = []
        for i, s in enumerate(sequences):
            if isinstance(s, str):
                ptrs[i] = as_utf8(s, C.byref(size))
                lens[i] = size.value
                if size.value != len(s):
                    raise TypeError("a read's sequence holds characters outside ASCII")
            else:
                b = bytes(s)
                keep.append(b)
                ptrs[i] = C.cast(C.c_char_p(b), C.c_void_p).value
                lens[i] = len(b)
        self._h = C.c_void_p()
        self.device, self.n = int(device), n
        check(_ffi.lib.amg_seqs_create(int(device), ptrs, ptr(lens), n, C.byref(self._h)))
        del keep

    def close(self):
# ... 79 lines not shown
```

include/amg.h:

```cpp
#ifndef AMG_H
#define AMG_H

#include <stdint.h>

#ifdef __cplusplus
extern "C" {
#endif

typedef struct amg_ctx amg_ctx;

enum {
  AMG_OK = 0,
  AMG_E_HIP = -1,
  AMG_E_ARG = -2,
  AMG_E_STATE = -3,
  AMG_E_PALINDROME = -4,
  AMG_E_OVERFLOW = -5,
  AMG_E_NOMEM = -6,
  AMG_E_DIST = -7,
  AMG_E_COLLISION = -8
};

#define AMG_MAX_K 16

typedef struct amg_counts_t {
  int64_t n_reads;
  int64_t n_tokens;
  int64_t n_windows;
  int64_t n_short_reads;
  int64_t n_nodes;
  int64_t n_edges;
  int64_t n_pairs;
  int64_t n_components;
  int64_t n_live_nodes;
  int64_t n_live_edges;
  int64_t n_reads_to_correct;
  int64_t node_table_slots;
  int64_t edge_table_slots;
  int64_t build_retries;
  int32_t k;
  int32_t two_v;
  int32_t exact_keys;
  int32_t derived;
} amg_counts_t;

int amg_create(int device, amg_ctx** out);
int amg_destroy(amg_ctx* ctx);
const char* amg_last_error(void);
int amg_sync(amg_ctx* ctx);
void* amg_stream(amg_ctx* ctx);

int amg_set_reads(amg_ctx* ctx, const int32_t* tokens, const int64_t* read_offsets,
                  int64_t n_reads, int32_t two_v, int on_device);
int amg_set_positions(amg_ctx* ctx, const int64_t* gene_start, const int64_t* gene_end,
                      const int64_t* read_len, int on_device);
int amg_set_positions32(amg_ctx* ctx, const int32_t* gene_start, const int32_t* gene_end,
                        const int64_t* read_len, int on_device);

int amg_set_read_lengths(amg_ctx* ctx, const int64_t* read_len, int on_device);

int amg_build(amg_ctx* ctx, int32_t k);
int amg_build_filtered(amg_ctx* ctx, int32_t k, uint32_t min_node_cov, uint32_t min_edge_cov);
int amg_build_multi(amg_ctx* const* ctxs, const int32_t* ks, int32_t n);
int amg_counts(amg_ctx* ctx, amg_counts_t* out);
int amg_finalize(amg_ctx* ctx);
int amg_sizes(amg_ctx* ctx, int64_t* n_reads, int64_t* n_tokens);
int amg_graph_sizes(amg_ctx* ctx, int64_t* n_nodes, int64_t* n_edges, int32_t* k);

int amg_get_nodes(amg_ctx* ctx, int32_t* canon_tokens, uint32_t* coverage,
                  int64_t* first_token, int8_t* first_dir, int32_t* component,
                  uint8_t* alive);
int amg_get_edges(amg_ctx* ctx, int32_t* src, int32_t* tgt, int8_t* sdir, int8_t* tdir,
                  uint32_t* coverage, uint8_t* alive);
int amg_get_read_nodes(amg_ctx* ctx, int32_t* tok_node, int8_t* tok_dir);
int amg_get_read_nodes_rows(amg_ctx* ctx, const int64_t* first_token, const int64_t* out_start, int64_t n_rows,
                            int32_t* node_ids);
int amg_get_node_adj(amg_ctx* ctx, int64_t* offsets, int32_t* edge_ids);
int amg_get_node_reads(amg_ctx* ctx, int64_t* offsets, int32_t* read_idx);

int amg_filter(amg_ctx* ctx, uint32_t min_node_cov, uint32_t min_edge_cov);
int amg_remove_nodes(amg_ctx* ctx, const int32_t* node_ids, int64_t n);
int amg_remove_edges(amg_ctx* ctx, const int32_t* edge_ids, int64_t n);
int amg_remove_short_linear_paths(amg_ctx* ctx, int32_t min_length, const uint8_t* protect,
                                  int64_t* n_removed, int32_t* removed_ids);
int amg_remove_low_coverage_components(amg_ctx* ctx, uint32_t min_component_coverage);
int amg_get_reads_to_correct(amg_ctx* ctx, uint8_t* flags);

int amg_correct_reads(amg_ctx* ctx, int64_t* n_out_reads, int64_t* n_out_tokens);
int amg_get_corrected(amg_ctx* ctx, int32_t* tokens, int64_t* read_offsets,
                      int32_t* orig_read, uint8_t* changed, int64_t* gene_start,
                      int64_t* gene_end);
int amg_get_corrected32(amg_ctx* ctx, int32_t* tokens, int64_t* read_offsets, int32_t* orig_read,
                        uint8_t* changed, int64_t* pos_src, int32_t* new_start, int32_t* new_end,
                        int64_t* n_new);
int amg_get_corrected_positions32(amg_ctx* ctx, int32_t* gene_start, int32_t* gene_end);
int amg_adopt_corrected(amg_ctx* ctx);
int amg_set_reads_from_corrected(amg_ctx* dst, amg_ctx* src);

int amg_match_patterns(amg_ctx* ctx, int which, const int32_t* pat, const int64_t* pat_offsets,
                       int64_t n_pat, int64_t* hit_offsets, int32_t* hit_read,
                       int32_t* hit_pos);

int amg_minhash(amg_ctx* ctx, const uint8_t* bases, const int64_t* seg_off, const int32_t* seg_set,
                int64_t n_seg, int32_t ksize, uint64_t scaled, int32_t* out_set, uint64_t* out_hash,
                int64_t cap, int64_t* n_out);

int amg_junction_paths(amg_ctx* ctx, int32_t max_distance, int64_t* sizes );
int amg_get_junction_paths(amg_ctx* ctx, int32_t* junction_node, int8_t* junction_dir, int32_t* path_start,
                           int64_t* path_off, int32_t* path_node, int8_t* path_dir);
typedef struct amg_seqs amg_seqs;
int amg_seqs_create(int32_t device, const char* const* seq, const int64_t* len, int64_t n, amg_seqs** out);
int amg_seqs_destroy(amg_seqs* seqs);
int amg_path_sketch_overlaps(amg_ctx* ctx, const amg_seqs* seqs, const int32_t* row_to_seq, int32_t ksize,
                             uint64_t scaled, int64_t n_paths, const int64_t* path_off, const int32_t* path_node,
                             int64_t n_pairs, const int32_t* pair_a, const int32_t* pair_b, int64_t* sketch_size,
                             int64_t* common);

typedef struct amg_kcount amg_kcount;
int amg_kcount_create(amg_ctx* ctx, const amg_seqs* seqs, int32_t k, int32_t slots_log2, amg_kcount** out);
int amg_kcount_sizes(const amg_kcount* counts, int64_t sizes[4]);
int amg_kcount_histo(amg_ctx* ctx, const amg_kcount* counts, int64_t min_count, int64_t histo[10002]);
int amg_kcount_query(amg_ctx* ctx, const amg_kcount* counts, const uint8_t* bases, const int64_t* seg_off,
                     int64_t n_seg, int64_t min_count, int64_t* out_count);
int amg_kcount_medians(amg_ctx* ctx, const amg_kcount* counts, const amg_seqs* seqs, const int64_t* set_off,
                       const int64_t* set_row, int64_t n_sets, int64_t min_count, int64_t* n, int64_t* mid_lo,
                       int64_t* mid_hi, int64_t max_pairs);
int amg_kcount_destroy(amg_kcount* counts);

int amg_nw_align(const int32_t* x, int32_t n, const int32_t* y, int32_t m, int8_t* ops, int32_t* n_ops);
int amg_pop_rewrite(amg_ctx* ctx, int32_t k, int32_t two_v, int64_t n_ops, const int32_t* better_tok,
                    const int64_t* better_off, const int32_t* worse_tok, const int64_t* worse_off, const uint8_t* interest,
                    int64_t n_reads, const int32_t* read_tok, const int64_t* read_off, const int32_t* read_op, int64_t cap,
                    uint8_t* op_veto, uint8_t* status, int32_t* first_shared, int32_t* last_shared, int64_t* out_off,
                    int32_t* out_tok, int32_t* out_src, int64_t* n_out);

int amg_dist_unique_id(void* out, int32_t bytes);
int amg_dist_init(amg_ctx* ctx, const void* unique_id, int32_t rank, int32_t world);
int amg_dist_merge(amg_ctx* ctx, int32_t k, uint32_t min_node_cov, uint32_t min_edge_cov);
int amg_dist_finalize(amg_ctx* ctx);

enum { AMG_XFER_ALL_TO_ALL = 1, AMG_XFER_ALL_GATHER = 2 };
typedef struct amg_xfer {
  int32_t kind;
  int32_t elem_bytes;
  const void* send;
  void* recv;
  const int64_t* send_counts;
  const int64_t* recv_counts;
  int64_t count;
} amg_xfer;
int amg_dist_init_external(amg_ctx* ctx, int32_t rank, int32_t world);
int amg_dist_merge_begin(amg_ctx* ctx, int32_t k, uint32_t min_node_cov, uint32_t min_edge_cov);
int amg_dist_merge_next(amg_ctx* ctx, amg_xfer* out);
int amg_dist_merge_local(amg_ctx* const* ctxs, int32_t world, int32_t k, uint32_t min_node_cov, uint32_t min_edge_cov);
int amg_copy_d2h(amg_ctx* ctx, const void* device_ptr, void* host_ptr, int64_t bytes);
int amg_copy_h2d(amg_ctx* ctx, void* device_ptr, const void* host_ptr, int64_t bytes);
int amg_dist_stats(amg_ctx* ctx, int64_t* out, int32_t reset);
int amg_dist_phase_ms(amg_ctx* ctx, int32_t on, const char** names, double* ms, int32_t cap);

typedef struct amg_calls amg_calls;
int amg_calls_load_json(const char* path, amg_calls** out);
int amg_calls_counts(amg_calls* calls, int64_t* n_reads, int64_t* n_tokens, int64_t* n_genes,
                     int64_t* names_bytes, int64_t* ids_bytes);
int amg_calls_get(amg_calls* calls, int32_t* tokens, int64_t* read_offsets, char* gene_names,
                  char* read_ids, uint8_t* gene_hashes);
int amg_calls_has_blanks(amg_calls* calls, int32_t* out);
int amg_calls_load_positions_json(amg_calls* calls, const char* path, int64_t* gene_start,
                                  int64_t* gene_end);
int amg_calls_write_json(const char* path, const int32_t* tokens, const int64_t* read_offsets,
                         int64_t n_reads, const char* gene_names, int64_t n_genes,
                         const char* read_ids);
int amg_calls_write_positions_json(const char* path, const int64_t* gene_start, const int64_t* gene_end,
                                   const int64_t* read_offsets, int64_t n_reads, const char* read_ids);
int amg_calls_write_positions_json32(const char* path, const int32_t* gene_start, const int32_t* gene_end,
                                     const int64_t* read_offsets, int64_t n_reads, const char* read_ids);
int amg_calls_first_use(const int32_t* tokens, int64_t n_tokens, int32_t two_v, const int32_t* wanted_ranks,
                        int64_t n_wanted, int64_t* first_index);
int amg_calls_free(amg_calls* calls);
int amg_calls_trim(int64_t* released_bytes);

typedef struct amg_blocks amg_blocks;
int amg_cluster_full_blocks(const int32_t* seq, const int64_t* seq_off, int64_t n_reads,
                            const int32_t* anchors, const int32_t* anchor_rank, int32_t n_anchors,
                            const int64_t* py_hash, int64_t n_nodes, int64_t none_hash, amg_blocks** out);
int amg_cluster_anchor_stats(const int32_t* seq, const int64_t* seq_off, int64_t n_reads, const int64_t* read_order,
                             const int32_t* amr_ids, int32_t n_amr, int64_t n_nodes, int32_t* out);
int amg_cluster_blocks_sizes(const amg_blocks* blocks, int64_t* n_blocks, int64_t* n_ids);
int amg_cluster_blocks_get(const amg_blocks* blocks, int64_t* block_off, int32_t* block_ids);
int amg_cluster_blocks_free(amg_blocks* blocks);
int64_t amg_py_tuple_hash(const int64_t* item_hashes, int64_t n);
int amg_pyset_script(const int32_t* ops, int64_t n_ops, const int64_t* key_hash, int32_t n_sets,
                     int32_t* out_keys, int64_t* out_off);

int amg_last_timings(amg_ctx* ctx, const char** names, float* ms, int cap);
int amg_set_timing(amg_ctx* ctx, int on);

int amg_scan_probe(amg_ctx* ctx, int kind, const void* in, int64_t n, int64_t* out, void* aux);

int amg_count_probe(amg_ctx* ctx, int kind, int form, int32_t* ids, int64_t n, int64_t n_ids, const int32_t* tab_ids,
                    int64_t n_slots, int misalign, int flags, uint32_t* counts, int64_t* state);

int amg_nw_probe(amg_ctx* ctx, int64_t n_pairs, const int32_t* x_tok, const int64_t* x_off, const int32_t* y_tok,
                 const int64_t* y_off, const int64_t* y_start, const int64_t* y_end, const int64_t* read_len,
                 const uint8_t* keep_orig, int flags, int64_t* out_start, int64_t* out_end, uint8_t* route,
                 int64_t* state);

enum {
  AMG_ROUTE_GAPPED = 0,
  AMG_ROUTE_BY_LEAN = 1,
  AMG_ROUTE_BY_FAST = 2,
  AMG_ROUTE_BY_GENERAL = 3,
  AMG_ROUTE_ON_NOT_TRIED = 4,
  AMG_ROUTE_ON_WINDOWS = 5,
  AMG_ROUTE_ON_RUNS = 6,
  AMG_ROUTE_ON_MEMO_UNFIT = 7,
  AMG_ROUTE_ON_RECORDS = 8,
  AMG_ROUTE_ON_COMBOS = 9,
  AMG_ROUTE_ON_CAND = 10,
  AMG_ROUTE_LEAN_NO_SLOTS = 11,
  AMG_ROUTE_LEAN_ANSWERS = 12,
  AMG_ROUTE_LEAN_LONG = 13,
  AMG_ROUTE_LEAN_OTHER = 14,
  AMG_ROUTE_NO_MEMO_SLOTS = 15,
  AMG_ROUTE_MEMO_QUESTIONS = 16,
  AMG_ROUTE_MEMO_SPILLED = 17,
  AMG_ROUTE_MEMO_UNFIT = 18,
  AMG_ROUTE_POOL_RETRIES = 19,
  AMG_ROUTE_KEEP_ORIG = 20,
  AMG_ROUTE_NW_FAST = 21,
  AMG_ROUTE_NW_LDS = 22,
  AMG_ROUTE_NW_GLOBAL = 23,
  AMG_ROUTE_WORDS = 24
};
int amg_correct_routes(amg_ctx* ctx, int64_t* out, int32_t cap);

#ifdef __cplusplus
}
#endif
#endif
```

Baseline: 10.22 billion gene-mers/s.

## Cut host round-trips in correction, derive and clip; rework read masking kernel

Result: no change. 10.30 billion gene-mers/s, median of 6 (+0.8%).

```diff
diff --git a/amira_amd/_ffi.py b/amira_amd/_ffi.py
--- a/amira_amd/_ffi.py
+++ b/amira_amd/_ffi.py
@@ -139,6 +139,7 @@
         "amg_count_probe": (C.c_int, [P, C.c_int, C.c_int, P, I64, I64, P, I64, C.c_int, C.c_int, P, P]),
         "amg_nw_probe": (C.c_int, [P, I64, P, P, P, P, P, P, P, P, C.c_int, P, P, P, P]),
         "amg_correct_routes": (C.c_int, [P, P, I32]),
+        "amg_cov_acc": (C.c_int, [P, P]),
     }
     for name, (res, args) in sig.items():
         fn = getattr(lib, name)
diff --git a/amira_amd/csrc/amg_correct.h b/amira_amd/csrc/amg_correct.h
--- a/amira_amd/csrc/amg_correct.h
+++ b/amira_amd/csrc/amg_correct.h
@@ -42,12 +42,6 @@
   }
 }
 
-__device__ __forceinline__ long long bcast_i64(long long v, int lane) {
-  const unsigned int lo = (unsigned int)__builtin_amdgcn_readlane((int)(unsigned int)v, lane);
-  const unsigned int hi = (unsigned int)__builtin_amdgcn_readlane((int)(unsigned int)((unsigned long long)v >> 32), lane);
-  return (long long)(((unsigned long long)hi << 32) | lo);
-}
-
 __device__ __forceinline__ void wave_sync() {
   __builtin_amdgcn_fence(__ATOMIC_ACQ_REL, "wavefront");
   __builtin_amdgcn_wave_barrier();
@@ -181,6 +175,7 @@
   long long *nw_size = nullptr, *nw_off = nullptr;
   unsigned int *bound = nullptr, *new_len = nullptr, *flag = nullptr;
   long long *tmp_off = nullptr, *new_idx = nullptr, *new_off = nullptr;
+  long long* glist_pos = nullptr;
   int* tmp_tok = nullptr;
   long long *plen = nullptr, *poffs = nullptr, *pos_new = nullptr;
   unsigned long long *max_bound = nullptr, *n_general = nullptr;
@@ -196,6 +191,7 @@
 struct CorrCounts {
   long long tmp_total = 0, n_gapped = 0, total_runs = 0;
   unsigned long long max_bound = 0;
+  unsigned long long alive_nodes = 0;
   bool carry = false;
   long long out_reads = 0, out_tokens = 0, big_total = 0, pos_total = 0;
   unsigned long long n_general = 0;
diff --git a/amira_amd/csrc/amg_correct.hip b/amira_amd/csrc/amg_correct.hip
--- a/amira_amd/csrc/amg_correct.hip
+++ b/amira_amd/csrc/amg_correct.hip
@@ -104,7 +104,7 @@
   AMGCHK(c->s0.ensure(per_read * (1 + 1) + 64));
   AMGCHK(c->s1.ensure(per_read * sizeof(int) * 2 + per_read * sizeof(long long) * 2 + 64));
   AMGCHK(c->s2.ensure(per_read * sizeof(unsigned int) * 3));
-  AMGCHK(c->s3.ensure(per_read * sizeof(long long) * 3));
+  AMGCHK(c->s3.ensure(per_read * sizeof(long long) * 4));
   AMGCHK(c->gm_mask.ensure(per_read * sizeof(unsigned long long)));
   AMGCHK(c->gm_ctr.ensure((16 + 256 + 256 + 16) * sizeof(unsigned long long)));
   S.per_read = per_read;
@@ -120,6 +120,7 @@
   S.tmp_off = c->s3.as<long long>();
   S.new_idx = S.tmp_off + per_read;
   S.new_off = S.new_idx + per_read;
+  S.glist_pos = S.new_off + per_read;
   S.max_bound = S.n_general = c->status.as<unsigned long long>() + ST_MISC;
   S.n_runs = c->gm_ctr.as<unsigned long long>() + 16;
   S.dead_kept = S.n_runs + 256;
@@ -186,19 +187,27 @@
   if (S.count_alive)
     hipLaunchKernelGGL(k_count_alive, dim3(128), dim3(256), 0, st, c->node_alive.as<unsigned char>(), c->n_nodes,
                        S.dead_kept + 256);
-  AMGCHK(prim_exscan_u32_pair(c, S.bound, S.tmp_off, S.flag, S.new_idx, (size_t)R));
+  AMGCHK(prim_exscan_classify(c, S.bound, S.tmp_off, S.flag, S.glist_pos, S.new_len, S.new_idx, S.new_off, (size_t)R));
   FetchList l;
   l.add(S.tmp_off + R);
   l.add(S.max_bound);
+  l.add(S.glist_pos + R);
+  for (int i = 0; i < 16; ++i) l.add(S.n_runs + 16 * i);
   l.add(S.new_idx + R);
-  for (int i = 0; i < 16; ++i) l.add(S.n_runs + 16 * i);
-  unsigned long long v[3 + 16];
+  l.add(S.new_off + R);
+  l.add(S.dead_kept + 256);
+  unsigned long long v[3 + 16 + 3];
   AMGCHK(fetch(c, l, v));
   n.tmp_total = (long long)v[0];
   n.max_bound = v[1];
   n.n_gapped = (long long)v[2];
   for (int i = 0; i < 16; ++i) n.total_runs += (long long)v[3 + i];
   n.carry = n.n_gapped > 0 && c->have_pos;
+  if (n.n_gapped == 0) {
+    n.out_reads = (long long)v[19];
+    n.out_tokens = (long long)v[20];
+  }
+  n.alive_nodes = v[21];
   return AMG_OK;
 }
 
@@ -259,14 +268,15 @@
 }
 
 static int corr_node_bound(amg_ctx* c, const CorrSwitches& sw, const CorrScratch& S, const CorrCounts& n) {
-  FetchList l;
-  for (int i = 0; i < 16; ++i) l.add(S.dead_kept + 16 * i);
-  l.add(S.dead_kept + 256);
-  unsigned long long v[17];
-  AMGCHK(fetch(c, l, v));
-  unsigned long long bound = S.count_alive ? v[16] : (unsigned long long)c->n_nodes;
   unsigned long long dead_kept = 0;
-  for (int i = 0; i < 16; ++i) dead_kept += v[i];
+  if (n.n_gapped > 0) {
+    FetchList l;
+    for (int i = 0; i < 16; ++i) l.add(S.dead_kept + 16 * i);
+    unsigned long long v[16];
+    AMGCHK(fetch(c, l, v));
+    for (int i = 0; i < 16; ++i) dead_kept += v[i];
+  }
+  unsigned long long bound = S.count_alive ? n.alive_nodes : (unsigned long long)c->n_nodes;
   bound += dead_kept;
   c->c_derivable = n.n_gapped == 0 && dead_kept == 0 && !c->edge_own_deaths;
   c->c_node_bound = (int64_t)bound;
@@ -304,7 +314,7 @@
   }
 
   stage_begin(c, "correct_pack");
-  AMGCHK(corr_shape(c, sw, S, a, n));
+  if (n.n_gapped > 0) AMGCHK(corr_shape(c, sw, S, a, n));
   stage_end(c);
   AMGCHK(ensure_outputs(c, n));
 
@@ -322,6 +332,7 @@
   AMGCHK(corr_node_bound(c, sw, S, n));
   stage_end(c);
   if (sw.routes) AMGCHK(routes_end(c, n));
+  c->c_pack_in_flight = n.n_gapped == 0;
   c->c_reads = n.out_reads;
   c->c_tokens = n.out_tokens;
   c->c_pos1_used = c->pos1_used + (n.carry ? n.pos_total : 0);
diff --git a/amira_amd/csrc/amg_correct_gapped.hip b/amira_amd/csrc/amg_correct_gapped.hip
--- a/amira_amd/csrc/amg_correct_gapped.hip
+++ b/amira_amd/csrc/amg_correct_gapped.hip
@@ -888,7 +888,7 @@
   const long long R = c->n_reads, n_gapped = n.n_gapped;
   AMGCHK(S.glist->ensure((size_t)(n_gapped + 1) * sizeof(int)));
   AMGCHK(c->gap_rec.ensure((size_t)(n_gapped + 1) * sizeof(GapRec)));
-  hipLaunchKernelGGL(k_scatter_gapped, dim3(nblk(R, 256)), dim3(256), 0, st, S.flag, S.new_idx, R,
+  hipLaunchKernelGGL(k_scatter_gapped, dim3(nblk(R, 256)), dim3(256), 0, st, S.flag, S.glist_pos, R,
                      S.glist->as<int>(), a.read_off, S.r_start, S.r_end, S.tmp_off, a.lmask, c->gap_rec.as<GapRec>());
   const int* gq = nullptr;
   if (n.total_runs > 0 && sw.gap_memo) AMGCHK(gap_memo(c, sw, a, n, &gq));
diff --git a/amira_amd/csrc/amg_corrected.hip b/amira_amd/csrc/amg_corrected.hip
--- a/amira_amd/csrc/amg_corrected.hip
+++ b/amira_amd/csrc/amg_corrected.hip
@@ -264,6 +264,11 @@
       c->pos0_own = true;
     }
   }
+  if (c->c_pack_in_flight && (c->tokens.borrowed || c->read_off.borrowed || c->read_len.borrowed)) {
+    HIPCHK(hipSetDevice(c->device));
+    AMGCHK(stream_wait(c));
+  }
+  c->c_pack_in_flight = false;
   for (DevBuf* b : {&c->tokens, &c->read_off, &c->read_len}) b->unborrow();
   std::swap(c->tokens, c->c_tokens_buf);
   std::swap(c->read_off, c->c_read_off);
diff --git a/amira_amd/csrc/amg_derive.hip b/amira_amd/csrc/amg_derive.hip
--- a/amira_amd/csrc/amg_derive.hip
+++ b/amira_amd/csrc/amg_derive.hip
@@ -196,25 +196,13 @@
     hipLaunchKernelGGL(k_dv_bounds, dim3(nblk(world + 1, 64)), dim3(64), 0, st, d_bases, world, c->node_first.as<long long>(), D,
                        new_id, c->pair_first.as<unsigned long long>(), P, ppos, d_bounds);
   }
-  unsigned long long v[2 + FETCH_MAX - 2];
-  {
-    FetchList l;
-    l.add(new_id + D);
-    l.add(ppos + P);
-    if (d_bounds) l.add_words(d_bounds, 2 * (world + 1));
-    if (l.overflow) return amg_fail(AMG_E_ARG, "derive: world too large");
-    AMGCHK(fetch(c, l, v));
-  }
-  const long long D2 = (long long)v[0], P2 = (long long)v[1];
-  if (bounds_host)
-    for (int i = 0; i < 2 * (world + 1); ++i) bounds_host[i] = (long long)v[2 + i];
-  AMGCHK(c->alt_ntok.ensure((size_t)(D2 * k + 1) * sizeof(int)));
-  AMGCHK(c->alt_ncov.ensure((size_t)(D2 + 1) * sizeof(unsigned int)));
-  AMGCHK(c->alt_nfirst.ensure((size_t)(D2 + 1) * sizeof(long long)));
-  AMGCHK(c->alt_nalive.ensure((size_t)(D2 + 1)));
-  AMGCHK(c->alt_pkey.ensure((size_t)(P2 + 2) * sizeof(unsigned long long)));
-  AMGCHK(c->alt_pfirst.ensure((size_t)(P2 + 2) * sizeof(unsigned long long)));
-  AMGCHK(c->alt_pcnt.ensure((size_t)(P2 + 2) * sizeof(unsigned int)));
+  AMGCHK(c->alt_ntok.ensure((size_t)(D * k + 1) * sizeof(int)));
+  AMGCHK(c->alt_ncov.ensure((size_t)(D + 1) * sizeof(unsigned int)));
+  AMGCHK(c->alt_nfirst.ensure((size_t)(D + 1) * sizeof(long long)));
+  AMGCHK(c->alt_nalive.ensure((size_t)(D + 1)));
+  AMGCHK(c->alt_pkey.ensure((size_t)(P + 2) * sizeof(unsigned long long)));
+  AMGCHK(c->alt_pfirst.ensure((size_t)(P + 2) * sizeof(unsigned long long)));
+  AMGCHK(c->alt_pcnt.ensure((size_t)(P + 2) * sizeof(unsigned int)));
   if (D > 0)
     hipLaunchKernelGGL(k_dv_nodes, dim3(nblk(D, 256)), dim3(256), 0, st, c->node_alive.as<unsigned char>(), new_id, D, k,
                        c->node_tokens.as<int>(), c->node_cov.as<unsigned int>(), c->node_first.as<long long>(),
@@ -229,8 +217,21 @@
                        c->alt_pcnt.as<unsigned int>(), bad);
   stage_end(c);
   AMGCHK(bs_read_stats(c, k));
-  unsigned long long hs[ST_WORDS];
-  AMGCHK(fetch_status(c, hs));
+  unsigned long long v[FETCH_MAX];
+  const int n_bounds = d_bounds ? 2 * (world + 1) : 0;
+  {
+    FetchList l;
+    l.add(new_id + D);
+    l.add(ppos + P);
+    if (d_bounds) l.add_words(d_bounds, n_bounds);
+    l.add_words(c->status.p, ST_WORDS);
+    if (l.overflow) return amg_fail(AMG_E_ARG, "derive: world too large");
+    AMGCHK(fetch(c, l, v));
+  }
+  const long long D2 = (long long)v[0], P2 = (long long)v[1];
+  if (bounds_host)
+    for (int i = 0; i < n_bounds; ++i) bounds_host[i] = (long long)v[2 + i];
+  const unsigned long long* hs = v + 2 + n_bounds;
   if (hs[ST_MISC] || hs[ST_BADINPUT]) return AMG_OK;
   c->n_windows = (int64_t)hs[ST_N_WINDOWS];
   c->n_short = (int64_t)hs[ST_N_SHORT];
diff --git a/amira_amd/csrc/amg_device.h b/amira_amd/csrc/amg_device.h
--- a/amira_amd/csrc/amg_device.h
+++ b/amira_amd/csrc/amg_device.h
@@ -12,6 +12,12 @@
 }
 __device__ __forceinline__ int ld_i32(const int* p) {
   return __hip_atomic_load(p, __ATOMIC_RELAXED, __HIP_MEMORY_SCOPE_AGENT);
+}
+
+__device__ __forceinline__ long long bcast_i64(long long v, int lane) {
+  const unsigned int lo = (unsigned int)__builtin_amdgcn_readlane((int)(unsigned int)v, lane);
+  const unsigned int hi = (unsigned int)__builtin_amdgcn_readlane((int)(unsigned int)((unsigned long long)v >> 32), lane);
+  return (long long)(((unsigned long long)hi << 32) | lo);
 }
 
 __device__ __forceinline__ unsigned long long mix64(unsigned long long x) {
diff --git a/amira_amd/csrc/amg_filter.hip b/amira_amd/csrc/amg_filter.hip
--- a/amira_amd/csrc/amg_filter.hip
+++ b/amira_amd/csrc/amg_filter.hip
@@ -15,41 +15,58 @@
   if ((min_cov > 1 && cov[e] < min_cov) || !node_alive[src[e]] || !node_alive[tgt[e]]) alive[e] = 0;
 }
 
-#define READS_PER_WAVE 8
+#define MASK_READS 64
+#define MASK_FLIGHT 8
 __global__ __launch_bounds__(256) void k_mask_reads(int* __restrict__ tok_node,
                                                     const long long* __restrict__ read_off,
                                                     long long n_reads,
                                                     const unsigned char* __restrict__ node_alive,
                                                     unsigned char* __restrict__ read_fix) {
-  const long long rbase = ((long long)blockIdx.x * 4 + (threadIdx.x >> 6)) * READS_PER_WAVE;
-  if (rbase >= n_reads) return;
   const int lane = threadIdx.x & 63;
-  const long long off_l = (lane <= READS_PER_WAVE && rbase + lane <= n_reads) ? read_off[rbase + lane] : 0;
-  long long a[READS_PER_WAVE], b[READS_PER_WAVE];
-  int v[READS_PER_WAVE];
+  const long long r0 = ((long long)blockIdx.x * 4 + (threadIdx.x >> 6)) * MASK_READS;
+  if (r0 >= n_reads) return;
+  long long o = 0;
+  int n = 0;
+  if (r0 + lane < n_reads) {
+    o = read_off[r0 + lane];
+    n = (int)(read_off[r0 + lane + 1] - o);
+  }
+  bool hit = false;
+  for (int j0 = 0; j0 < MASK_READS; j0 += MASK_FLIGHT) {
+    long long oo[MASK_FLIGHT];
+    int nn[MASK_FLIGHT], v[MASK_FLIGHT];
+    bool dead[MASK_FLIGHT];
+    int most = 0;
 #pragma unroll
-  for (int j = 0; j < READS_PER_WAVE; ++j) {
-    a[j] = __shfl(off_l, j, 64);
-    b[j] = rbase + j < n_reads ? __shfl(off_l, j + 1, 64) : a[j];
-  }
+    for (int j = 0; j < MASK_FLIGHT; ++j) {
+      nn[j] = __builtin_amdgcn_readlane(n, j0 + j);
+      oo[j] = bcast_i64(o, j0 + j);
+      most = nn[j] > most ? nn[j] : most;
+    }
+    if (most == 0) continue;
 #pragma unroll
-  for (int j = 0; j < READS_PER_WAVE; ++j) v[j] = a[j] + lane < b[j] ? tok_node[a[j] + lane] : -1;
-  bool dead[READS_PER_WAVE];
+    for (int j = 0; j < MASK_FLIGHT; ++j) v[j] = lane < nn[j] ? tok_node[oo[j] + lane] : -1;
 #pragma unroll
-  for (int j = 0; j < READS_PER_WAVE; ++j) dead[j] = v[j] >= 0 && !node_alive[v[j]];
+    for (int j = 0; j < MASK_FLIGHT; ++j) dead[j] = v[j] >= 0 && !node_alive[v[j]];
 #pragma unroll
-  for (int j = 0; j < READS_PER_WAVE; ++j) {
-    if (dead[j]) tok_node[a[j] + lane] = -2;
-    bool hit = dead[j];
-    for (long long t = a[j] + 64 + lane; t < b[j]; t += 64) {
-      const int n = tok_node[t];
-      if (n >= 0 && !node_alive[n]) {
-        tok_node[t] = -2;
-        hit = true;
+    for (int j = 0; j < MASK_FLIGHT; ++j) {
+      if (dead[j]) tok_node[oo[j] + lane] = -2;
+      bool any = __ballot(dead[j]) != 0ull;
+      if (nn[j] > 64) {
+        bool more = false;
+        for (int q = 64 + lane; q < nn[j]; q += 64) {
+          const int w = tok_node[oo[j] + q];
+          if (w >= 0 && !node_alive[w]) {
+            tok_node[oo[j] + q] = -2;
+            more = true;
+          }
+        }
+        any = any || __ballot(more) != 0ull;
       }
-    }
-    if (__any(hit) && lane == 0) read_fix[rbase + j] = 1;
-  }
+      hit = hit || (any && lane == j0 + j);
+    }
+  }
+  if (hit) read_fix[r0 + lane] = 1;
 }
 
 static int apply_removals(amg_ctx* c, unsigned int min_edge_cov) {
@@ -62,7 +79,7 @@
                        c->node_alive.as<unsigned char>(), c->edge_alive.as<unsigned char>(),
                        c->n_edges, min_edge_cov);
   if (c->n_reads > 0)
-    hipLaunchKernelGGL(k_mask_reads, dim3(nblk(c->n_reads, 4 * READS_PER_WAVE)), dim3(256), 0, st,
+    hipLaunchKernelGGL(k_mask_reads, dim3(nblk(c->n_reads, 4 * MASK_READS)), dim3(256), 0, st,
                        c->tok_node.as<int>(), c->read_off.as<long long>(), c->n_reads,
                        c->node_alive.as<unsigned char>(), c->read_fix.as<unsigned char>());
   return AMG_OK;
@@ -121,6 +138,7 @@
 #define CLIP_MAX 64
 template <class View>
 __global__ void k_clip_mark(View g, long long n_nodes, int min_length, const unsigned long long* __restrict__ acc,
+                            unsigned long long known_sum, unsigned long long known_n,
                             const unsigned int* __restrict__ comp_live,
                             const unsigned char* __restrict__ protect,
                             unsigned char* __restrict__ kill) {
@@ -146,7 +164,7 @@
     r = lin_step(g, tgt, td == 1, &tgt, &td);
   }
   if (!(len > 0 && len < min_length)) return;
-  const double thr = ((double)acc[0] / (double)acc[1]) * 1.5;
+  const double thr = ((double)(acc ? acc[0] : known_sum) / (double)(acc ? acc[1] : known_n)) * 1.5;
   bool all_high = true;
   for (int j = 0; j < len; ++j) all_high = all_high && ((double)g.n_cov[path[j]] > thr);
   if (all_high) return;
@@ -256,6 +274,27 @@
   block_add_cov(s_cov, s_n, acc);
 }
 
+extern "C" int amg_cov_acc(amg_ctx* c, uint64_t* out ) {
+  NEED_BUILT(c);
+  if (!out) return amg_fail(AMG_E_ARG, "null out");
+  unsigned long long* acc = c->status.as<unsigned long long>() + ST_COV_SUM;
+  ClearList cl;
+  cl.add(acc, 2 * sizeof(unsigned long long));
+  AMGCHK(clear_many(c, cl));
+  const long long D = c->n_nodes;
+  if (D > 0)
+    hipLaunchKernelGGL(k_cov_acc, dim3(nblk(D, 2048) < 256u ? nblk(D, 2048) : 256u), dim3(256), 0, c->stream,
+                       c->node_alive.as<unsigned char>(), c->node_cov.as<unsigned int>(), D, acc);
+  FetchList l;
+  l.add(acc);
+  l.add(acc + 1);
+  unsigned long long v[2];
+  AMGCHK(fetch(c, l, v));
+  out[0] = v[0];
+  out[1] = v[1];
+  return AMG_OK;
+}
+
 __global__ void k_scatter_ids(const unsigned char* __restrict__ killed, const long long* __restrict__ pos,
                               long long n, int* __restrict__ out) {
   long long i = (long long)blockIdx.x * blockDim.x + threadIdx.x;
@@ -300,12 +339,15 @@
   if (by_labels) AMGCHK(ensure_components(c));
   const bool light = c->live_lists == LiveLists::Absent && !getenv("AMG_CLIP_LISTS");
   stage_begin(c, "clip");
-  unsigned long long* acc = c->status.as<unsigned long long>() + ST_COV_SUM;
+  const bool known = c->pristine && !c->dist_mode && !by_labels;
+  const unsigned long long known_sum = (unsigned long long)c->n_windows, known_n = (unsigned long long)D;
+  unsigned long long* acc =
+      known ? nullptr : c->status.as<unsigned long long>() + ST_COV_SUM;
   AMGCHK(c->s0.ensure((size_t)D + 8));
   if (by_labels) AMGCHK(c->s4.ensure((size_t)(c->n_components + 2) * sizeof(unsigned int)));
   {
     ClearList cl;
-    cl.add(acc, 2 * sizeof(unsigned long long));
+    if (acc) cl.add(acc, 2 * sizeof(unsigned long long));
     cl.add(c->s0.p, (size_t)D + 8);
     if (by_labels) cl.add(c->s4.p, (size_t)(c->n_components + 2) * sizeof(unsigned int));
     if (light) AMGCHK(row_summary_reserve(c, &cl));
@@ -317,7 +359,7 @@
     hipLaunchKernelGGL(k_comp_hist, dim3(nblk(D, 256) < 256u ? nblk(D, 256) : 256u), dim3(256), 0, st, c->node_comp.as<int>(),
                        c->node_alive.as<unsigned char>(), c->node_cov.as<unsigned int>(), D, 0u,
                        c->s4.as<unsigned int>(), (unsigned int*)nullptr, acc);
-  else
+  else if (acc)
     hipLaunchKernelGGL(k_cov_acc, dim3(nblk(D, 2048) < 256u ? nblk(D, 2048) : 256u), dim3(256), 0, st,
                        c->node_alive.as<unsigned char>(), c->node_cov.as<unsigned int>(), D, acc);
   unsigned char* d_protect = nullptr;
@@ -328,12 +370,12 @@
   }
   const unsigned int* comp_live = by_labels ? c->s4.as<unsigned int>() : nullptr;
   if (light) {
-    hipLaunchKernelGGL(k_clip_mark<RView>, dim3(nblk(D, 128)), dim3(128), 0, st, summary, D, (int)min_length, acc, comp_live,
-                       d_protect, c->s0.as<unsigned char>());
+    hipLaunchKernelGGL(k_clip_mark<RView>, dim3(nblk(D, 128)), dim3(128), 0, st, summary, D, (int)min_length, acc, known_sum,
+                       known_n, comp_live, d_protect, c->s0.as<unsigned char>());
   } else {
     AMGCHK(ensure_live_adj(c));
     hipLaunchKernelGGL(k_clip_mark<GView>, dim3(nblk(D, 128)), dim3(128), 0, st, make_view(c), D, (int)min_length, acc,
-                       comp_live, d_protect, c->s0.as<unsigned char>());
+                       known_sum, known_n, comp_live, d_protect, c->s0.as<unsigned char>());
   }
   int r = finish_kill(c, n_removed, removed_ids);
   stage_end(c);
diff --git a/amira_amd/csrc/amg_internal.h b/amira_amd/csrc/amg_internal.h
--- a/amira_amd/csrc/amg_internal.h
+++ b/amira_amd/csrc/amg_internal.h
@@ -208,6 +208,7 @@
   DevBuf read_fix;
 
   bool have_corrected = false;
+  bool c_pack_in_flight = false;
   bool pos0_own = false;
   int64_t c_reads = 0, c_tokens = 0;
   DevBuf c_tokens_buf, c_read_off, c_orig, c_changed, c_gstart, c_gend, c_read_len;
@@ -300,8 +301,8 @@
 struct ClearList;
 int prim_exscan_i64(amg_ctx* c, const long long* in, long long* out, size_t n);
 int prim_exscan_u32_to_i64(amg_ctx* c, const unsigned int* in, long long* out, size_t n);
-int prim_exscan_u32_pair(amg_ctx* c, const unsigned int* in_a, long long* out_a, const unsigned int* in_b, long long* out_b,
-                         size_t n);
+int prim_exscan_classify(amg_ctx* c, const unsigned int* in_a, long long* out_a, const unsigned int* flag, long long* out_flag,
+                         const unsigned int* len, long long* out_keep, long long* out_len, size_t n);
 int prim_exscan_i64_pair(amg_ctx* c, const long long* in_a, long long* out_a, const long long* in_b, long long* out_b,
                          size_t n);
 int prim_exscan_bytes_set(amg_ctx* c, const unsigned char* in, long long* out, size_t n, const ClearList* side = nullptr);
diff --git a/amira_amd/csrc/amg_scan.hip b/amira_amd/csrc/amg_scan.hip
--- a/amira_amd/csrc/amg_scan.hip
+++ b/amira_amd/csrc/amg_scan.hip
@@ -1,4 +1,6 @@
 #include "amg_device.h"
+
+#include <type_traits>
 
 #define SC_THREADS 512
 #define SC_ROWS 16
@@ -99,6 +101,37 @@
     const unsigned int hi = (unsigned int)(key & 0xffffffffull) - 1u;
     return lo == hi ? 1ull : 2ull;
   }
+};
+
+struct LoadCorrTrio {
+  const unsigned int* flag;
+  const unsigned int* len;
+  long long n;
+  long long* out_flag;
+  long long* out_keep;
+  long long* out_len;
+  static constexpr int parts = 3;
+  struct Part {
+    const unsigned int* in;
+    long long n;
+    bool nonzero;
+    using Raw = unsigned int;
+    __device__ __forceinline__ long long lim() const { return n; }
+    __device__ __forceinline__ Raw raw(long long i) const { return in[i]; }
+    __device__ __forceinline__ unsigned long long val(long long, Raw r) const {
+      return nonzero ? (r != 0u ? 1ull : 0ull) : (unsigned long long)r;
+    }
+  };
+  __device__ __forceinline__ Part at(int p) const { return Part{p == 0 ? flag : len, n, p == 1}; }
+  __device__ __forceinline__ long long* out(int p) const { return p == 0 ? out_flag : p == 1 ? out_keep : out_len; }
+};
+template <class L, class = void>
+struct scan_parts {
+  static constexpr int value = 1;
+};
+template <class L>
+struct scan_parts<L, std::void_t<decltype(L::parts)>> {
+  static constexpr int value = L::parts;
 };
 
 struct LoadNone {
@@ -183,7 +216,7 @@
 template <class Load, class LoadB, class Emit>
 __global__ __launch_bounds__(SC_THREADS) void k_exscan(Load load, Emit emit_a, long long n_a, LoadB load_b,
                                                         long long* __restrict__ out_b, long long n_b, long long tiles_a,
-                                                        unsigned long long* counter, unsigned long long ticket_base,
+                                                        long long tiles_b , unsigned long long* counter, unsigned long long ticket_base,
                                                         unsigned long long* status, unsigned int epoch, ClearArgs side) {
   __shared__ unsigned long long s_wave[SC_THREADS / 64];
   __shared__ unsigned long long s_excl;
@@ -193,14 +226,25 @@
   __syncthreads();
   const long long tile = s_tile;
   const bool second = tile >= tiles_a;
-  const long long seg0 = second ? tiles_a : 0;
+  long long seg0 = second ? tiles_a : 0;
+  int part = 0;
+  if constexpr (scan_parts<LoadB>::value > 1) {
+    if (second) {
+      part = (int)((tile - tiles_a) / tiles_b);
+      seg0 = tiles_a + part * tiles_b;
+    }
+  }
   const long long n = second ? n_b : n_a;
   const long long w0 = (tile - seg0) * SC_TILE + (long long)wave * (64 * SC_ROWS);
   unsigned long long x[SC_ROWS], inc[SC_ROWS];
-  if (second)
-    load_rows(load_b, w0, n, lane, x);
-  else
+  if (second) {
+    if constexpr (scan_parts<LoadB>::value > 1)
+      load_rows(load_b.at(part), w0, n, lane, x);
+    else
+      load_rows(load_b, w0, n, lane, x);
+  } else {
     load_rows(load, w0, n, lane, x);
+  }
   unsigned long long row_off = 0;
 #pragma unroll
   for (int r = 0; r < SC_ROWS; ++r) {
@@ -265,6 +309,7 @@
   }
   __syncthreads();
   const unsigned long long base = s_excl + wave_excl;
+  if constexpr (scan_parts<LoadB>::value > 1) out_b = load_b.out(part);
 #pragma unroll
   for (int r = 0; r < SC_ROWS; ++r) {
     const long long i = w0 + r * 64 + lane;
@@ -284,7 +329,8 @@
   if (side && side->overflow) return amg_fail(AMG_E_ARG, "exscan: more than %d ranges in one list", CLEAR_MAX);
   if (n == 0 && n_b == 0) return side ? clear_many(c, *side) : AMG_OK;
   const unsigned long long tiles_a = (n + SC_TILE - 1) / SC_TILE;
-  const unsigned long long tiles = tiles_a + (n_b + SC_TILE - 1) / SC_TILE;
+  const unsigned long long tiles_b = (n_b + SC_TILE - 1) / SC_TILE;
+  const unsigned long long tiles = tiles_a + (n_b ? scan_parts<LoadB>::value : 1) * tiles_b;
   const size_t need = (size_t)(tiles + 8) * sizeof(unsigned long long);
   if (need > c->scan_state.cap || c->scan_epoch >= 0x3fffu) {
     if (need > c->scan_state.cap) {
@@ -303,7 +349,8 @@
   sa.n = 0;
   if (side) sa = clear_args(*side);
   hipLaunchKernelGGL((k_exscan<Load, LoadB, Emit>), dim3((unsigned int)tiles), dim3(SC_THREADS), 0, c->stream, load, emit,
-                     (long long)n, load_b, out_b, (long long)n_b, (long long)tiles_a, st, c->scan_tickets, st + 8, epoch, sa);
+                     (long long)n, load_b, out_b, (long long)n_b, (long long)tiles_a, (long long)tiles_b, st, c->scan_tickets, st + 8,
+                     epoch, sa);
   c->scan_tickets += tiles;
   return AMG_OK;
 }
@@ -322,10 +369,10 @@
   return exscan(c, LoadArr<long long>{in}, out, n);
 }
 
-int prim_exscan_u32_pair(amg_ctx* c, const unsigned int* in_a, long long* out_a, const unsigned int* in_b, long long* out_b,
-                         size_t n) {
-  return exscan(c, LoadArrN<unsigned int>{in_a, (long long)n}, out_a, n + 1, LoadArrN<unsigned int>{in_b, (long long)n}, out_b,
-                n + 1);
+int prim_exscan_classify(amg_ctx* c, const unsigned int* in_a, long long* out_a, const unsigned int* flag, long long* out_flag,
+                         const unsigned int* len, long long* out_keep, long long* out_len, size_t n) {
+  return exscan(c, LoadArrN<unsigned int>{in_a, (long long)n}, out_a, n + 1,
+                LoadCorrTrio{flag, len, (long long)n, out_flag, out_keep, out_len}, nullptr, n + 1);
 }
 
 int prim_exscan_i64_pair(amg_ctx* c, const long long* in_a, long long* out_a, const long long* in_b, long long* out_b,
diff --git a/amira_amd/engine.py b/amira_amd/engine.py
--- a/amira_amd/engine.py
+++ b/amira_amd/engine.py
@@ -204,6 +204,11 @@
 
     def remove_low_coverage_components(self, min_cov):
         check(_ffi.lib.amg_remove_low_coverage_components(self._h, int(min_cov)))
+
+    def cov_acc(self):
+        out = np.zeros(2, np.uint64)
+        check(_ffi.lib.amg_cov_acc(self._h, _ffi.ptr(out)))
+        return int(out[0]), int(out[1])
 
     def correct_reads(self):
         nr, nt = C.c_int64(0), C.c_int64(0)
diff --git a/include/amg.h b/include/amg.h
--- a/include/amg.h
+++ b/include/amg.h
@@ -199,6 +199,8 @@
 
 int amg_count_probe(amg_ctx* ctx, int kind, int form, int32_t* ids, int64_t n, int64_t n_ids, const int32_t* tab_ids,
                     int64_t n_slots, int misalign, int flags, uint32_t* counts, int64_t* state);
+
+int amg_cov_acc(amg_ctx* ctx, uint64_t* out );
 
 int amg_nw_probe(amg_ctx* ctx, int64_t n_pairs, const int32_t* x_tok, const int64_t* x_off, const int32_t* y_tok,
                  const int64_t* y_off, const int64_t* y_start, const int64_t* y_end, const int64_t* read_len,
```
